# THU-DA-6D-Pose-Group/CATRE

Hardware: AMD Instinct MI355X
Metric: pose-refine iters/sec (B=256, N=1024, K=4) (higher is better)
Workload: dtype f32; 1 GPU; B=256 objects/GPU, N=1024 observed + M=1024 prior points, K=4 refine iterations, forward-only (eval loop of catre_evaluator.py:292-311), fp32 MFMA; objects_per_gpu=256, N=1024, M=1024, K=4, parallelism=batch-sharded x1 (no data-path collective)

## Files before the change

catre_amd/csrc/catre_kernels.hip:

```cpp
#include <algorithm>
#include <cstdlib>
#include <atomic>
#include <mutex>
#include <cstring>
#include <vector>

#include "catre_device.h"

#include "../../include/catre_hip.h"

#define CATRE_VERSION_STR "catre_hip gfx950 r1"
#define PMW 1088

struct TileInfo {
  int obj;
  int cloud;
  int is_obs;
  int p0;
  int valid;
};

__device__ __forceinline__ TileInfo tile_info(int bid, int B, int N, int M) {
  const int TN = (N + TP - 1) / TP, TM = (M + TP - 1) / TP;
  TileInfo ti;
// ... 1281 lines not shown
  } else {
    const int rd = catre_rot_dim(o.rot_type);
    float r[6];
#pragma unroll
    for (int i = 0; i < 6; ++i) r[i] = i < rd ? rotp[i] : 0.f;
    rot_param_to_mat(r, o.rot_type, dR);
  }

  const float* p0 = pose0 + b * 12;
  const float t0[3] = {p0[3], p0[7], p0[11]};
  float d[3] = {dtr[b * 3] * o.delta_t_weight, dtr[b * 3 + 1] * o.delta_t_weight, dtr[b * 3 + 2] * o.delta_t_weight};
  float t[3];
  if (!o.delta_t_space_3d) {
    const float zsrc = t0[2];
    const float ztgt = o.delta_z_deepim ? zsrc / expf(d[2]) : d[2] * zsrc;
    const float fx = o.k_aware ? Ks[b * 9 + 0] : 1.f, fy = o.k_aware ? Ks[b * 9 + 4] : 1.f;
    t[0] = ztgt * (d[0] / fx + t0[0] / zsrc);
    t[1] = ztgt * (d[1] / fy + t0[1] / zsrc);
    t[2] = ztgt;
  } else {
    t[0] = t0[0] + d[0];
    t[1] = t0[1] + d[1];
    t[2] = t0[2] + d[2];
  }
  const float* sb = o.scale_base_mean ? mean_scales + b * 3 : scale0 + b * 3;
  float s[3];
#pragma unroll
  for (int i = 0; i < 3; ++i) s[i] = o.scale_mul ? sb[i] * expf(dsr[b * 3 + i]) : sb[i] + dsr[b * 3 + i];

  if (o.is_allo) {
    const float nrm = sqrtf(t[0] * t[0] + t[1] * t[1] + t[2] * t[2]) + o.allo_eps;
    const float ray[3] = {t[0] / nrm, t[1] / nrm, t[2] / nrm};
    const float angle = acosf(ray[2]);
    float ax[3] = {-ray[1], ray[0], 0.f};
    const float an = sqrtf(ax[0] * ax[0] + ax[1] * ax[1]) + o.allo_eps;
    ax[0] /= an;
    ax[1] /= an;
    const float sh = sinf(angle * 0.5f);
    float q[4] = {cosf(angle * 0.5f), ax[0] * sh, ax[1] * sh, 0.f * sh};
    const float qn = sqrtf(q[0] * q[0] + q[1] * q[1] + q[2] * q[2] + q[3] * q[3]);
#pragma unroll
    for (int i = 0; i < 4; ++i) q[i] /= qn;
    const float X = q[1] * 2.f, Y = q[2] * 2.f, Z = q[3] * 2.f;
    const float wX = q[0] * X, wY = q[0] * Y, wZ = q[0] * Z, xX = q[1] * X, xY = q[1] * Y, xZ = q[1] * Z;
    const float yY = q[2] * Y, yZ = q[2] * Z, zZ = q[3] * Z;
    const float A[9] = {1.f - (yY + zZ), xY - wZ, xZ + wY, xY + wZ, 1.f - (xX + zZ), yZ - wX,
                        xZ - wY,         yZ + wX, 1.f - (xX + yY)};
    float E[9];
#pragma unroll
    for (int i = 0; i < 3; ++i)
#pragma unroll
      for (int j = 0; j < 3; ++j) E[i * 3 + j] = A[i * 3] * dR[j] + A[i * 3 + 1] * dR[3 + j] + A[i * 3 + 2] * dR[6 + j];
#pragma unroll
    for (int i = 0; i < 9; ++i) dR[i] = E[i];
  }
  float* po = pose_out + b * 12;
#pragma unroll
  for (int i = 0; i < 3; ++i) {
#pragma unroll
    for (int j = 0; j < 3; ++j)
      po[i * 4 + j] = dR[i * 3] * p0[j] + dR[i * 3 + 1] * p0[4 + j] + dR[i * 3 + 2] * p0[8 + j];
    po[i * 4 + 3] = t[i];
  }
#pragma unroll
  for (int i = 0; i < 3; ++i) scale_out[b * 3 + i] = o.refine_scale ? s[i] : scale0[b * 3 + i];
}

__global__ void k_pose_update(const float* __restrict__ rot6d, const float* __restrict__ dtr,
                              const float* __restrict__ dsr, const float* __restrict__ pose0,
                              const float* __restrict__ scale0, const float* __restrict__ mean_scales,
                              const float* __restrict__ Ks, catre_opts o, float* __restrict__ pose_out,
                              float* __restrict__ scale_out, int B, float* __restrict__ pose_echo = nullptr,
                              float* __restrict__ scale_echo = nullptr) {
  const int b = blockIdx.x * blockDim.x + threadIdx.x;
  if (b >= B) return;
  pose_update_obj(rot6d + (size_t)b * (o.rot_input_is_matrix ? 9 : catre_rot_dim(o.rot_type)), dtr, dsr, pose0, scale0,
                  mean_scales, Ks, o, pose_out, scale_out, b, pose_echo, scale_echo);
}

__global__ __launch_bounds__(256) void k_colmax(const float* __restrict__ x, float* __restrict__ out, int rows,
                                                int N) {
  const int lane = threadIdx.x & 63;
  const int wpb = blockDim.x >> 6;
  const int nwaves = gridDim.x * wpb;
  for (int row = blockIdx.x * wpb + (threadIdx.x >> 6); row < rows; row += nwaves) {
    const float* r = x + (size_t)row * N;
    float m = -INFINITY;
    if ((N & 3) == 0) {
      const f32x4* r4 = reinterpret_cast<const f32x4*>(r);
      const int n4 = N >> 2;
#pragma unroll 4
      for (int i = lane; i < n4; i += 64) {
        const f32x4 v = __builtin_nontemporal_load(r4 + i);
        m = fmaxf(fmaxf(m, fmaxf(v[0], v[1])), fmaxf(v[2], v[3]));
      }
    } else {
      for (int i = lane; i < N; i += 64) m = fmaxf(m, r[i]);
    }
#pragma unroll
    for (int o = 32; o > 0; o >>= 1) m = fmaxf(m, __shfl_xor(m, o));
    if (lane == 0) out[row] = m;
  }
}

#include "catre_bf16.h"
#include "catre_split.h"
#include "catre_screen.h"

template <bool SPLIT, class OT = OpBf16>
__device__ __forceinline__ void pack_frag_lp_body(const PackJobs& J) {
  static_assert(!SPLIT || !is_f16_op<OT>(), "the split packs are bf16 pairs");
  const int gi = blockIdx.x * blockDim.x + threadIdx.x;
  if (gi >= J.end[J.n - 1]) return;
  int j = 0;
  while (gi >= J.end[j]) ++j;
  const int base = j ? J.end[j - 1] : 0, idx = gi - base, total = J.end[j] - base;
  const int K = J.K[j];
  const int e = idx & 7, lane = (idx >> 3) & 63, rest = idx >> 9;
  const int nkc = K / 16;
  const int kc = rest % nkc, mb = rest / nkc;
  const int row = mb * 32 + (lane & 31), col = kc * 16 + 8 * (e >> 2) + 4 * (lane >> 5) + (e & 3);
  const float w = J.src[j][(size_t)row * J.ld[j] + J.coloff[j] + col];
  unsigned short* dst = reinterpret_cast<unsigned short*>(J.dst[j]);
  const typename OT::T h = (typename OT::T)w;
  dst[idx] = __builtin_bit_cast(unsigned short, h);
  if constexpr (SPLIT) dst[(size_t)total + idx] = __builtin_bit_cast(unsigned short, (__bf16)(w - (float)h));
}
template <bool SPLIT>
__global__ void k_pack_frag_lp_multi(PackJobs J) {
  pack_frag_lp_body<SPLIT>(J);
}
__global__ void k_pack_frag_hf_multi(PackJobs J) { pack_frag_lp_body<false, OpF16>(J); }
#include "catre_gram.h"
#include "catre_small.h"
#include "catre_train.h"
#include "catre_optim.h"
#include "catre_heads.h"
#include "catre_aug.h"
#include "catre_pcl.h"
#include "catre_pclf.h"
#include "catre_loss.h"
#include "catre_eval.h"

namespace {

inline size_t align_up(size_t v, size_t a) { return (v + a - 1) / a * a; }

struct PackLayout {
  size_t stn_c2, stn_c3, fstn_c1, fstn_c2, fstn_c3, c2, c3, c4, rot_l0[2], rot_l1[2], ts_w0t, ts_w1t, sumwp, total;
  size_t bf_stn_c2, bf_stn_c3, bf_fstn_c1, bf_fstn_c2, bf_fstn_c3, bf_c2, bf_c3, bf_c4, bf_rot_l0[2], bf_rot_l1[2];
  size_t sp_stn_c2, sp_stn_c3, sp_fstn_c1, sp_fstn_c2, sp_fstn_c3, sp_c3, sp_c4, sp_rot_l0[2], sp_rot_l1[2];
  size_t f16_stn_c2, f16_stn_c3, f16_fstn_c1, f16_fstn_c2, f16_fstn_c3, f16_c2, f16_c3, f16_c4, f16_rot_l0[2], f16_rot_l1[2];
  size_t scr_c4, scr_nw4, scr_stn_c3, scr_fstn_c3, scr_nw_stn, scr_nw_fstn;
};

PackLayout pack_layout(int ts_in) {
  PackLayout L;
  size_t o = 0;
  auto take = [&](size_t n) {
    size_t r = o;
    o += align_up(n, 64);
    return r;
  };
  L.stn_c2 = take(128 * 64);
  L.stn_c3 = take(1024 * 128);
  L.fstn_c1 = take(64 * 64);
  L.fstn_c2 = take(128 * 64);
  L.fstn_c3 = take(1024 * 128);
  L.c2 = take(128 * 64);
  L.c3 = take(512 * 128);
  L.c4 = take(1024 * 512);
  for (int h = 0; h < 2; ++h) {
    L.rot_l0[h] = take(256 * 64);
    L.rot_l1[h] = take(256 * 256);
  }
  L.sumwp = take(64);
  L.bf_stn_c2 = take(128 * 64 / 2);
  L.bf_stn_c3 = take(1024 * 128 / 2);
  L.bf_fstn_c1 = take(64 * 64 / 2);
  L.bf_fstn_c2 = take(128 * 64 / 2);
  L.bf_fstn_c3 = take(1024 * 128 / 2);
  L.bf_c2 = take(128 * 64 / 2);
  L.bf_c3 = take(512 * 128 / 2);
  L.bf_c4 = take(1024 * 512 / 2);
  for (int h = 0; h < 2; ++h) {
    L.bf_rot_l0[h] = take(256 * 64 / 2);
    L.bf_rot_l1[h] = take(256 * 256 / 2);
  }
  L.sp_stn_c2 = take(128 * 64);
  L.sp_stn_c3 = take(1024 * 128);
  L.sp_fstn_c1 = take(64 * 64);
  L.sp_fstn_c2 = take(128 * 64);
  L.sp_fstn_c3 = take(1024 * 128);
  L.sp_c3 = take(512 * 128);
  L.sp_c4 = take(1024 * 512);
  for (int h = 0; h < 2; ++h) {
    L.sp_rot_l0[h] = take(256 * 64);
    L.sp_rot_l1[h] = take(256 * 256);
  }
  L.f16_stn_c2 = take(128 * 64 / 2);
  L.f16_stn_c3 = take(1024 * 128 / 2);
  L.f16_fstn_c1 = take(64 * 64 / 2);
  L.f16_fstn_c2 = take(128 * 64 / 2);
  L.f16_fstn_c3 = take(1024 * 128 / 2);
  L.f16_c2 = take(128 * 64 / 2);
  L.f16_c3 = take(512 * 128 / 2);
  L.f16_c4 = take(1024 * 512 / 2);
  for (int h = 0; h < 2; ++h) {
    L.f16_rot_l0[h] = take(256 * 64 / 2);
    L.f16_rot_l1[h] = take(256 * 256 / 2);
  }
  L.scr_c4 = take(1024 * 512);
  L.scr_nw4 = take(1024);
  L.scr_stn_c3 = take(1024 * 128);
  L.scr_fstn_c3 = take(1024 * 128);
  L.scr_nw_stn = take(1024);
  L.scr_nw_fstn = take(1024);
  L.ts_w0t = take((size_t)ts_in * 256);
  L.ts_w1t = take(256 * 256);
  L.total = o;
  return L;
}

struct WsLayout {
  size_t tspart, xbuf, kbuf, pm, pool, h1, h2, trans3, trans64, gfeat, pointfeat, dt, ds, rot6d, bias0, gn0, gn1, aff0, gn1stat, y1, rpart,
      bar, frun, total;
};

WsLayout ws_layout(int B, int N, int M) {
  const size_t TN = (N + TP - 1) / TP, TM = (M + TP - 1) / TP, T = TN + TM;
  const size_t b = B, P = (size_t)N + M;
  WsLayout L;
  size_t o = 0;
  auto take = [&](size_t n) {
    size_t r = o;
    o += align_up(n, 64);
    return r;
  };
  L.tspart = take(b * 8 * 256);
  L.xbuf = take(b * N * 3);
  L.kbuf = take(b * M * 3);
  L.pm = take((2 * b <= SMALL_ROWS ? 2 : 1) * b * T * PMW);
  L.pool = take(2 * b * 1024);
  L.h1 = take(2 * b * 512);
  L.h2 = take(2 * b * 256);
  L.trans3 = take(2 * b * 9);
  L.trans64 = take(2 * b * 4096);
  L.gfeat = take(2 * b * PMW);
  L.pointfeat = take(b * P * 64);
  L.dt = take(b * 3);
  L.ds = take(b * 3);
  L.rot6d = take(b * 6);
  L.bias0 = take(2 * 2 * b * 256);
  L.gn0 = take(b * 2 * T * 64);
  L.gn1 = take(b * 2 * T * 64);
  L.aff0 = take(b * 2 * 2 * 2 * 256);
  L.gn1stat = take(b * 2 * 64);
  {
    const size_t y1n = b * 2 * P * 256, mom = b * 2 * (4 * (4096 + 64) + 64);
    const size_t y1t = b * 2 * T * 256 * 32;
    L.y1 = take(std::max(std::max(y1n, mom), y1t));
  }
  L.rpart = take(b * 2 * T * 4);
  L.bar = take(64);
  L.frun = take(b * ((TN + 1) / 2 + (TM + 1) / 2) * 1024);
  L.total = o;
  return L;
}

inline int check_launch() { return hipGetLastError() == hipSuccess ? CATRE_OK : CATRE_ERR_LAUNCH; }

inline bool dims_ok(int B, int N, int M) { return B > 0 && N > 0 && M > 0; }
inline bool dims_ok1(int B, int N, int M) { return B > 0 && N > 0 && M >= 0; }
inline int n_clouds(int B, int M) { return M > 0 ? 2 * B : B; }
#define RS_DISPATCH(rs, L) \
  switch (rs) {            \
    case 4: L(4); break;   \
    case 2: L(2); break;   \
    default: L(1);         \
  }
inline int row_split(int tiles) { return tiles * 4 <= 256 ? 4 : tiles * 2 <= 256 ? 2 : 1; }
#define RS_DISPATCH8(rs, L) \
  switch (rs) {             \
    case 8: L(8); break;    \
    case 4: L(4); break;    \
    case 2: L(2); break;    \
    default: L(1);          \
  }
inline int row_split8(int tiles) { return tiles * 8 <= 256 ? 8 : row_split(tiles); }
inline int gn0_shares(int B) { return B * 8 <= 512 ? 8 : B * 4 <= 512 ? 4 : B * 2 <= 512 ? 2 : 1; }
inline int trunk_h_split(int tiles) { return tiles * 8 <= 256 ? 4 : tiles * 4 <= 256 ? 2 : tiles * 2 <= 256 ? 1 : 0; }

#define REQUIRE(cond) \
  do {                \
    if (!(cond)) return CATRE_ERR_BAD_ARG; \
  } while (0)

inline const f32x4* pk4(const float* packed, size_t off) { return reinterpret_cast<const f32x4*>(packed + off); }
inline const u32x4* pkb(const float* packed, size_t off) { return reinterpret_cast<const u32x4*>(packed + off); }

inline TsHeadArgs ts_head_args(const float* l0part, const float* const* prm, const float* packed, const PackLayout& L,
                               float* dt, float* ds, int B) {
  return TsHeadArgs{l0part, prm[CATRE_P_TS_L0_B], prm[CATRE_P_TS_GN0_W], prm[CATRE_P_TS_GN0_B], packed + L.ts_w1t,
                    prm[CATRE_P_TS_L1_B], prm[CATRE_P_TS_GN1_W], prm[CATRE_P_TS_GN1_B], prm[CATRE_P_TS_FCT_W],
                    prm[CATRE_P_TS_FCT_B], prm[CATRE_P_TS_FCS_W], prm[CATRE_P_TS_FCS_B], dt, ds, B};
}

int stn_fc_tail(const float* pooled, const float* const* prm, int base , float* h1, float* h2,
                float* out, int k, int R, hipStream_t st, const float* pm = nullptr, int B = 0, int N = 0, int M = 0,
                unsigned* bar = nullptr) {
  if (bar) {
    const int nb3 = (k * k + 31) / 32, grid = nb3 > 16 ? nb3 : 16;
    hipLaunchKernelGGL(k_fc_tail, dim3(grid), dim3(64 * LIN_WAVES), 0, st, pooled, pm, B, N, M, prm[base], prm[base + 1],
                       prm[base + 2], prm[base + 3], prm[base + 4], prm[base + 5], h1, h2, out, k, R, bar);
    return check_launch();
  }
  if (pm)
    hipLaunchKernelGGL(k_linear_pm, dim3(1, 512 / 32), dim3(64 * LIN_WAVES), 0, st, pm, B, N, M, prm[base], 1024,
                       prm[base + 1], h1, 512, R, 512, 1, nullptr, nullptr, nullptr);
  else
    hipLaunchKernelGGL(k_linear, dim3((R + 31) / 32, 512 / 32), dim3(64 * LIN_WAVES), 0, st, pooled, 1024, prm[base], 1024,
                       prm[base + 1], h1, 512, R, 512, 1024, 1, 0);
  hipLaunchKernelGGL(k_linear, dim3((R + 31) / 32, 256 / 32), dim3(64 * LIN_WAVES), 0, st, h1, 512, prm[base + 2], 512,
                     prm[base + 3], h2, 256, R, 256, 512, 1, 0);
  hipLaunchKernelGGL(k_linear, dim3((R + 31) / 32, (k * k + 31) / 32), dim3(64 * LIN_WAVES), 0, st, h2, 256, prm[base + 4], 256,
                     prm[base + 5], out, k * k, R, k * k, 256, 0, k);
  return check_launch();
}

struct ProfState {
  int kernel = -1;
  int cap = 0, n = 0;
  hipEvent_t* ev = nullptr;
};
ProfState g_prof;
unsigned long long* g_trunk_trace = nullptr;

static int bf_pair_min() {
  static const int v = [] {
    const char* e = getenv("CATRE_BF_PAIR_MIN");
    return e ? atoi(e) : 512;
  }();
  return v;
}

enum { FORM_TRUNK4 = 1, FORM_STN4 = 2, FORM_STN_PAIR = 4, FORM_ROTW = 8, FORM_FC_TAIL = 16, FORM_SCREEN = 32, FORM_SCREEN_STN = 64,
       FORM_SCREEN_POOL = 128, FORM_SCREEN_RUN = 256 };
#ifndef CATRE_SCREEN_DEFAULT
#define CATRE_SCREEN_DEFAULT true
#endif
#ifndef CATRE_SCREEN_STN_DEFAULT
#define CATRE_SCREEN_STN_DEFAULT true
#endif
#ifndef CATRE_SCREEN_POOL_DEFAULT
#define CATRE_SCREEN_POOL_DEFAULT true
#endif
#ifndef CATRE_SCREEN_RUN_DEFAULT
#define CATRE_SCREEN_RUN_DEFAULT true
#endif
static std::atomic<int> g_forms{-1};
static int forms() {
  int v = g_forms.load(std::memory_order_relaxed);
  if (v < 0) {
    auto on = [](const char* name, bool dflt = true) {
      const char* e = getenv(name);
      return e ? atoi(e) != 0 : dflt;
    };
    v = (on("CATRE_TRUNK4") ? FORM_TRUNK4 : 0) | (on("CATRE_STN4") ? FORM_STN4 : 0) |
        (on("CATRE_STN_PAIR") ? FORM_STN_PAIR : 0) | (on("CATRE_ROTW", false) ? FORM_ROTW : 0) |
        (on("CATRE_FC_TAIL", false) ? FORM_FC_TAIL : 0) | (on("CATRE_SCREEN", CATRE_SCREEN_DEFAULT) ? FORM_SCREEN : 0) |
        (on("CATRE_SCREEN_STN", CATRE_SCREEN_STN_DEFAULT) ? FORM_SCREEN_STN : 0) |
        (on("CATRE_SCREEN_POOL", CATRE_SCREEN_POOL_DEFAULT) ? FORM_SCREEN_POOL : 0) |
        (on("CATRE_SCREEN_RUN", CATRE_SCREEN_RUN_DEFAULT) ? FORM_SCREEN_RUN : 0);
    g_forms.store(v, std::memory_order_relaxed);
  }
  return v;
}
static bool trunk4_on() { return forms() & FORM_TRUNK4; }
inline int stn_pairs(int B, int N, int M) { return B * (((N + TP - 1) / TP + 1) / 2 + ((M + TP - 1) / TP + 1) / 2); }
static bool stn_pair_on() { return forms() & FORM_STN_PAIR; }
static bool stn4_on() { return forms() & FORM_STN4; }
static bool fc_tail_on() { return forms() & FORM_FC_TAIL; }
static bool screen_on() { return forms() & FORM_SCREEN; }
static bool screen_stn_on() { return (forms() & (FORM_SCREEN | FORM_SCREEN_STN)) == (FORM_SCREEN | FORM_SCREEN_STN); }
static bool screen_pool_on() { return forms() & FORM_SCREEN_POOL; }
static bool screen_run_on() { return (forms() & (FORM_SCREEN_POOL | FORM_SCREEN_RUN)) == (FORM_SCREEN_POOL | FORM_SCREEN_RUN); }
static std::atomic<int> g_run_len{0};
static int screen_run_rule(int B, int N, int M, int cus) {
  const int TN = (N + TP - 1) / TP, TM = (M + TP - 1) / TP;
  const long long slots1 = ((long long)B * (TN + TM) + cus - 1) / cus;
  for (int S = 16; S > 1; --S) {
    const long long R = (long long)B * ((TN + S - 1) / S + (TM + S - 1) / S);
    if ((R + cus - 1) / cus * S <= slots1) return S;
  }
  return 1;
}
static int device_cus() {
  static const int n = [] {
    int dev = 0, v = 0;
    if (hipGetDevice(&dev) != hipSuccess || hipDeviceGetAttribute(&v, hipDeviceAttributeMultiprocessorCount, dev) != hipSuccess || v <= 0)
      v = 256;
    return v;
  }();
  return n;
}
static int screen_run_len(int B, int N, int M) {
  const int f = g_run_len.load(std::memory_order_relaxed);
  return f > 0 ? f : screen_run_rule(B, N, M, device_cus());
}
#ifndef CATRE_SCREEN_POOL_STN_DEFAULT
#define CATRE_SCREEN_POOL_STN_DEFAULT true
#endif
static bool screen_pool_stn_on() {
  static const bool stn = [] { const char* e = getenv("CATRE_SCREEN_POOL_STN"); return e ? atoi(e) != 0 : CATRE_SCREEN_POOL_STN_DEFAULT; }();
  return screen_pool_on() && stn;
}
#ifndef CATRE_SCREEN_RUN_STN_DEFAULT
#define CATRE_SCREEN_RUN_STN_DEFAULT true
#endif
static bool screen_run_stn_on() {
  static const bool stn = [] { const char* e = getenv("CATRE_SCREEN_RUN_STN"); return e ? atoi(e) != 0 : CATRE_SCREEN_RUN_STN_DEFAULT; }();
  return screen_run_on() && screen_stn_on() && screen_pool_stn_on() && stn;
}
inline int stn_pair_runs(int B, int N, int M, int SP) {
  return B * ((((N + TP - 1) / TP + 1) / 2 + SP - 1) / SP + (((M + TP - 1) / TP + 1) / 2 + SP - 1) / SP);
}
static bool rotw_on() { return forms() & FORM_ROTW; }

#ifndef CATRE_NO_PROFILING
std::mutex g_prof_mu;
struct ProfScope {
  hipStream_t st;
  int slot = -1;
  ProfScope(int kernel_id, hipStream_t s) : st(s) {
    if (g_prof.kernel != kernel_id) return;
    std::lock_guard<std::mutex> lk(g_prof_mu);
    if (g_prof.kernel == kernel_id && g_prof.n < g_prof.cap) {
      slot = g_prof.n++;
      (void)hipEventRecord(g_prof.ev[2 * slot], st);
    }
  }
  ~ProfScope() {
    if (slot < 0) return;
    std::lock_guard<std::mutex> lk(g_prof_mu);
    if (slot < g_prof.cap) (void)hipEventRecord(g_prof.ev[2 * slot + 1], st);
  }
};
#else
struct ProfScope {
  ProfScope(int, hipStream_t) {}
};
#endif


static bool stn_pair_form(int tiles, int B, int N, int M) {
  return row_split8(tiles) == 1 && stn4_on() && stn_pair_on() && stn_pairs(B, N, M) >= 256;
}

void launch_stn3d(const catre_points* pts, const float* const* prm, const float* packed, float* ws, const WsLayout& W,
                  int B, int N, int M, bool split, hipStream_t st, unsigned* zero_bar = nullptr, float* probe_s = nullptr,
                  float* probe_eps = nullptr, float* probe_rows = nullptr) {
  const PackLayout L = pack_layout(1);
  const int tiles = B * ((N + TP - 1) / TP + (M + TP - 1) / TP);
  ProfScope ps(CATRE_K_STN3D, st);
  if (split) {
#define LAUNCH_(RS)                                                                                            \
  hipLaunchKernelGGL(k_stn3d_split<RS>, dim3(tiles * RS), dim3(256), 0, st, *pts, prm[CATRE_P_STN_CONV1_W],     \
                     prm[CATRE_P_STN_CONV1_B], pkb(packed, L.sp_stn_c2), prm[CATRE_P_STN_CONV2_B],              \
                     pkb(packed, L.sp_stn_c3), prm[CATRE_P_STN_CONV3_B], ws + W.pm, B, N, M)
    RS_DISPATCH(row_split(tiles), LAUNCH_)
#undef LAUNCH_
  } else if (const int S = stn_pair_form(tiles, B, N, M) && screen_run_stn_on() && !probe_s ? screen_run_len(B, N, M) : 1; S > 1) {
    const int SP = S / 2;
    hipLaunchKernelGGL(k_stn3d_pair_sr, dim3(stn_pair_runs(B, N, M, SP)), dim3(256), 0, st,
                       Stn3dRunArgs{*pts, prm[CATRE_P_STN_CONV1_W], prm[CATRE_P_STN_CONV1_B], pk4(packed, L.stn_c2),
                                    prm[CATRE_P_STN_CONV2_B], pk4(packed, L.stn_c3), prm[CATRE_P_STN_CONV3_B], ws + W.pm,
                                    pkb(packed, L.scr_stn_c3), packed + L.scr_nw_stn, B, N, M, SP});
  } else if (stn_pair_form(tiles, B, N, M) && (screen_stn_on() || probe_s)) {
    hipLaunchKernelGGL(screen_pool_stn_on() ? k_stn3d_pair_sp : k_stn3d_pair_s, dim3(stn_pairs(B, N, M)), dim3(256), 0, st, *pts, prm[CATRE_P_STN_CONV1_W],
                       prm[CATRE_P_STN_CONV1_B], pk4(packed, L.stn_c2), prm[CATRE_P_STN_CONV2_B], pk4(packed, L.stn_c3),
                       prm[CATRE_P_STN_CONV3_B], ws + W.pm, B, N, M,
                       ScreenArgs{pkb(packed, L.scr_stn_c3), packed + L.scr_nw_stn, probe_s, probe_eps}, probe_rows);
  } else if (stn_pair_form(tiles, B, N, M)) {
    const int pairs = stn_pairs(B, N, M);
    hipLaunchKernelGGL(k_stn3d_pair<false>, dim3(pairs), dim3(256), 0, st, *pts, prm[CATRE_P_STN_CONV1_W], prm[CATRE_P_STN_CONV1_B],
                       pk4(packed, L.stn_c2), prm[CATRE_P_STN_CONV2_B], pk4(packed, L.stn_c3), prm[CATRE_P_STN_CONV3_B],
                       ws + W.pm, B, N, M);
  } else if (row_split8(tiles) == 1 && stn4_on()) {
    hipLaunchKernelGGL((k_stn3d<1, false, true>), dim3(tiles), dim3(256), 0, st, *pts, prm[CATRE_P_STN_CONV1_W],
                       prm[CATRE_P_STN_CONV1_B], pk4(packed, L.stn_c2), prm[CATRE_P_STN_CONV2_B], pk4(packed, L.stn_c3),
                       prm[CATRE_P_STN_CONV3_B], ws + W.pm, B, N, M, TrainSave{}, zero_bar);
  } else {
#define LAUNCH_(RS)                                                                                      \
  hipLaunchKernelGGL(k_stn3d<RS>, dim3(tiles * RS), dim3(256), 0, st, *pts, prm[CATRE_P_STN_CONV1_W],     \
                     prm[CATRE_P_STN_CONV1_B], pk4(packed, L.stn_c2), prm[CATRE_P_STN_CONV2_B],           \
                     pk4(packed, L.stn_c3), prm[CATRE_P_STN_CONV3_B], ws + W.pm, B, N, M, TrainSave{}, zero_bar)
    RS_DISPATCH8(row_split8(tiles), LAUNCH_)
#undef LAUNCH_
  }
}

void launch_stnkd(const catre_points* pts, const float* trans3, const float* const* prm, const float* packed, float* ws,
                  const WsLayout& W, int B, int N, int M, bool split, hipStream_t st, unsigned* zero_bar = nullptr,
                  float* probe_s = nullptr, float* probe_eps = nullptr, float* probe_rows = nullptr) {
  const PackLayout L = pack_layout(1);
  const int tiles = B * ((N + TP - 1) / TP + (M + TP - 1) / TP);
  ProfScope ps(CATRE_K_STNKD, st);
  if (split) {
#define LAUNCH_(RS)                                                                                                \
  hipLaunchKernelGGL(k_stnkd_split<RS>, dim3(tiles * RS), dim3(256), 0, st, *pts, trans3, prm[CATRE_P_CONV1_W],     \
                     prm[CATRE_P_CONV1_B], pkb(packed, L.sp_fstn_c1), prm[CATRE_P_FSTN_CONV1_B],                    \
                     pkb(packed, L.sp_fstn_c2), prm[CATRE_P_FSTN_CONV2_B], pkb(packed, L.sp_fstn_c3),               \
                     prm[CATRE_P_FSTN_CONV3_B], ws + W.pm, B, N, M)
    RS_DISPATCH(row_split(tiles), LAUNCH_)
#undef LAUNCH_
  } else if (const int S = stn_pair_form(tiles, B, N, M) && screen_run_stn_on() && !probe_s ? screen_run_len(B, N, M) : 1; S > 1) {
    const int SP = S / 2;
    hipLaunchKernelGGL(k_stnkd_pair_sr, dim3(stn_pair_runs(B, N, M, SP)), dim3(256), 0, st,
                       StnkdRunArgs{*pts, trans3, prm[CATRE_P_CONV1_W], prm[CATRE_P_CONV1_B], pk4(packed, L.fstn_c1),
                                    prm[CATRE_P_FSTN_CONV1_B], pk4(packed, L.fstn_c2), prm[CATRE_P_FSTN_CONV2_B],
                                    pk4(packed, L.fstn_c3), prm[CATRE_P_FSTN_CONV3_B], ws + W.pm,
                                    pkb(packed, L.scr_fstn_c3), packed + L.scr_nw_fstn, B, N, M, SP});
  } else if (stn_pair_form(tiles, B, N, M) && (screen_stn_on() || probe_s)) {
    hipLaunchKernelGGL(screen_pool_stn_on() ? k_stnkd_pair_sp : k_stnkd_pair_s, dim3(stn_pairs(B, N, M)), dim3(256), 0, st, *pts, trans3, prm[CATRE_P_CONV1_W],
                       prm[CATRE_P_CONV1_B], pk4(packed, L.fstn_c1), prm[CATRE_P_FSTN_CONV1_B], pk4(packed, L.fstn_c2),
                       prm[CATRE_P_FSTN_CONV2_B], pk4(packed, L.fstn_c3), prm[CATRE_P_FSTN_CONV3_B], ws + W.pm, B, N, M,
                       ScreenArgs{pkb(packed, L.scr_fstn_c3), packed + L.scr_nw_fstn, probe_s, probe_eps}, probe_rows);
  } else if (stn_pair_form(tiles, B, N, M)) {
    const int pairs = stn_pairs(B, N, M);
    hipLaunchKernelGGL(k_stnkd_pair<false>, dim3(pairs), dim3(256), 0, st, *pts, trans3, prm[CATRE_P_CONV1_W], prm[CATRE_P_CONV1_B],
                       pk4(packed, L.fstn_c1), prm[CATRE_P_FSTN_CONV1_B], pk4(packed, L.fstn_c2), prm[CATRE_P_FSTN_CONV2_B],
                       pk4(packed, L.fstn_c3), prm[CATRE_P_FSTN_CONV3_B], ws + W.pm, B, N, M);
  } else if (row_split8(tiles) == 1 && stn4_on()) {
    hipLaunchKernelGGL((k_stnkd<1, false, true>), dim3(tiles), dim3(256), 0, st, *pts, trans3, prm[CATRE_P_CONV1_W],
                       prm[CATRE_P_CONV1_B], pk4(packed, L.fstn_c1), prm[CATRE_P_FSTN_CONV1_B], pk4(packed, L.fstn_c2),
                       prm[CATRE_P_FSTN_CONV2_B], pk4(packed, L.fstn_c3), prm[CATRE_P_FSTN_CONV3_B], ws + W.pm, B, N, M,
                       TrainSave{}, zero_bar);
  } else {
#define LAUNCH_(RS)                                                                                                     \
  hipLaunchKernelGGL(k_stnkd<RS>, dim3(tiles * RS), dim3(256), 0, st, *pts, trans3, prm[CATRE_P_CONV1_W],                \
                     prm[CATRE_P_CONV1_B], pk4(packed, L.fstn_c1), prm[CATRE_P_FSTN_CONV1_B], pk4(packed, L.fstn_c2),    \
                     prm[CATRE_P_FSTN_CONV2_B], pk4(packed, L.fstn_c3), prm[CATRE_P_FSTN_CONV3_B], ws + W.pm, B, N, M,   \
                     TrainSave{}, zero_bar)
    RS_DISPATCH8(row_split8(tiles), LAUNCH_)
#undef LAUNCH_
  }
}

void launch_trunk(const catre_points* pts, const float* trans3, const float* trans64, const float* const* prm,
                  const float* packed, float* pointfeat, float* ws, const WsLayout& W, int B, int N, int M, bool split,
                  hipStream_t st, float* probe_s = nullptr, float* probe_eps = nullptr) {
  const PackLayout L = pack_layout(1);
  const int tiles = B * ((N + TP - 1) / TP + (M + TP - 1) / TP);
  ProfScope ps(CATRE_K_TRUNK, st);
  if (split) {
#define LAUNCH_(RS)                                                                                           \
  hipLaunchKernelGGL(k_trunk_split<RS>, dim3(tiles * RS), dim3(512), 0, st, *pts, trans3, trans64,             \
                     prm[CATRE_P_CONV1_W], prm[CATRE_P_CONV1_B], pk4(packed, L.c2), prm[CATRE_P_CONV2_B],      \
                     pkb(packed, L.sp_c3), prm[CATRE_P_CONV3_B], pkb(packed, L.sp_c4), prm[CATRE_P_CONV4_B],   \
                     ws + W.pm, pointfeat, B, N, M, g_trunk_trace)
    RS_DISPATCH(row_split(tiles), LAUNCH_)
#undef LAUNCH_
  } else if (const int S = row_split8(tiles) == 1 && trunk4_on() && screen_on() && screen_run_on() ? screen_run_len(B, N, M) : 1;
             S > 1) {
    const int runs = B * (((N + TP - 1) / TP + S - 1) / S + ((M + TP - 1) / TP + S - 1) / S);
    hipLaunchKernelGGL(k_trunk4sr, dim3(runs), dim3(256), 0, st,
                       TrunkRunArgs{*pts, trans3, trans64, prm[CATRE_P_CONV1_W], prm[CATRE_P_CONV1_B], pk4(packed, L.c2),
                                    prm[CATRE_P_CONV2_B], pk4(packed, L.c3), prm[CATRE_P_CONV3_B], pk4(packed, L.c4),
                                    prm[CATRE_P_CONV4_B], ws + W.pm, pointfeat, g_trunk_trace,
                                    ScreenArgs{pkb(packed, L.scr_c4), packed + L.scr_nw4, probe_s, probe_eps}, ws + W.frun,
                                    B, N, M, S});
  } else if (row_split8(tiles) == 1 && trunk4_on() && (screen_on() || probe_s)) {
    hipLaunchKernelGGL(screen_pool_on() ? k_trunk4sp : k_trunk4s, dim3(tiles), dim3(256), 0, st, *pts, trans3, trans64,
                       prm[CATRE_P_CONV1_W], prm[CATRE_P_CONV1_B], pk4(packed, L.c2), prm[CATRE_P_CONV2_B], pk4(packed, L.c3),
                       prm[CATRE_P_CONV3_B], pk4(packed, L.c4), prm[CATRE_P_CONV4_B], ws + W.pm, pointfeat, B, N, M,
                       g_trunk_trace, ScreenArgs{pkb(packed, L.scr_c4), packed + L.scr_nw4, probe_s, probe_eps});
  } else if (row_split8(tiles) == 1 && trunk4_on()) {
    hipLaunchKernelGGL(k_trunk4<false>, dim3(tiles), dim3(256), 0, st, *pts, trans3, trans64, prm[CATRE_P_CONV1_W],
                       prm[CATRE_P_CONV1_B], pk4(packed, L.c2), prm[CATRE_P_CONV2_B], pk4(packed, L.c3),
                       prm[CATRE_P_CONV3_B], pk4(packed, L.c4), prm[CATRE_P_CONV4_B], ws + W.pm, pointfeat, B, N, M,
                       g_trunk_trace);
  } else {
#define LAUNCH_(RS)                                                                                             \
  hipLaunchKernelGGL(k_trunk<RS>, dim3(tiles * RS), dim3(512), 0, st, *pts, trans3, trans64, prm[CATRE_P_CONV1_W], \
                     prm[CATRE_P_CONV1_B], pk4(packed, L.c2), prm[CATRE_P_CONV2_B], pk4(packed, L.c3),            \
                     prm[CATRE_P_CONV3_B], pk4(packed, L.c4), prm[CATRE_P_CONV4_B], ws + W.pm, pointfeat, B, N, M, \
                     g_trunk_trace)
    RS_DISPATCH8(row_split8(tiles), LAUNCH_)
#undef LAUNCH_
  }
}

}

extern "C" {

const char* catre_version(void) { return CATRE_VERSION_STR; }

const char* catre_status_string(int s) {
  switch (s) {
    case CATRE_OK: return "ok";
    case CATRE_ERR_BAD_ARG: return "bad argument";
    case CATRE_ERR_WORKSPACE: return "workspace or packed-weight buffer too small";
    case CATRE_ERR_LAUNCH: return "kernel launch failed";
    case CATRE_ERR_UNSUPPORTED: return "unsupported configuration";
    default: return "unknown status";
  }
}

size_t catre_workspace_bytes(int B, int N, int M) {
  if (!dims_ok1(B, N, M)) return 0;
  return ws_layout(B, N, M).total * sizeof(float);
}

size_t catre_packed_floats(int N, int M, int ts_in_dim) {
  if (N <= 0 || M <= 0 || ts_in_dim <= 0) return 0;
  return pack_layout(ts_in_dim).total;
}

int catre_pack_weights(const float* const* prm, int N, int M, int ts_in, float* packed, size_t packed_floats,
                       void* stream) {
  return catre_pack_weights_sel(prm, N, M, ts_in, packed, packed_floats, CATRE_PACK_ALL, stream);
}

int catre_pack_weights_sel(const float* const* prm, int N, int M, int ts_in, float* packed, size_t packed_floats, int sel,
                           void* stream) {
  REQUIRE(prm && packed && N > 0 && M > 0 && ts_in > 0);
  const PackLayout L = pack_layout(ts_in);
  if (packed_floats < L.total) return CATRE_ERR_WORKSPACE;
  hipStream_t st = (hipStream_t)stream;
  const bool enc32 = sel & CATRE_PACK_F32_ENCODER, head32 = sel & CATRE_PACK_F32_HEADS, bf = sel & CATRE_PACK_BF16,
             sp = sel & CATRE_PACK_SPLIT, tails = sel & CATRE_PACK_F32_TAILS, hf = sel & CATRE_PACK_F16;
  PackJobs jobs;
  jobs.n = 0;
  auto flush = [&]() {
    if (jobs.n) hipLaunchKernelGGL(k_pack_frag_multi, dim3((jobs.end[jobs.n - 1] + 255) / 256), dim3(256), 0, st, jobs);
    jobs.n = 0;
  };
  auto frag = [&](const float* src, int ld, int coloff, int rows, int K, size_t off) {
    if (!src) return;
    if (jobs.n == PACK_MAX_JOBS) flush();
    const int j = jobs.n++;
    jobs.src[j] = src;
    jobs.dst[j] = packed + off;
    jobs.ld[j] = ld;
    jobs.coloff[j] = coloff;
    jobs.K[j] = K;
    jobs.end[j] = (j ? jobs.end[j - 1] : 0) + rows * K;
  };
  PackJobs lpjobs;
  lpjobs.n = 0;
  enum { LP_BF16, LP_SPLIT, LP_F16 };
  auto flush_lp = [&](int kind) {
    if (lpjobs.n) {
      const dim3 grid((lpjobs.end[lpjobs.n - 1] + 255) / 256);
      if (kind == LP_SPLIT)
        hipLaunchKernelGGL(k_pack_frag_lp_multi<true>, grid, dim3(256), 0, st, lpjobs);
      else if (kind == LP_F16)
        hipLaunchKernelGGL(k_pack_frag_hf_multi, grid, dim3(256), 0, st, lpjobs);
      else
        hipLaunchKernelGGL(k_pack_frag_lp_multi<false>, grid, dim3(256), 0, st, lpjobs);
    }
    lpjobs.n = 0;
  };
  auto frag_lp = [&](int kind, const float* src, int ld, int coloff, int rows, int K, size_t off) {
    if (!src) return;
    if (lpjobs.n == PACK_MAX_JOBS) flush_lp(kind);
    const int j = lpjobs.n++;
    lpjobs.src[j] = src;
    lpjobs.dst[j] = packed + off;
    lpjobs.ld[j] = ld;
    lpjobs.coloff[j] = coloff;
    lpjobs.K[j] = K;
    lpjobs.end[j] = (j ? lpjobs.end[j - 1] : 0) + rows * K;
  };
  auto frag_bf = [&](const float* src, int ld, int coloff, int rows, int K, size_t off) {
    frag_lp(LP_BF16, src, ld, coloff, rows, K, off);
  };
  if (bf) {
  frag_bf(prm[CATRE_P_STN_CONV2_W], 64, 0, 128, 64, L.bf_stn_c2);
  frag_bf(prm[CATRE_P_STN_CONV3_W], 128, 0, 1024, 128, L.bf_stn_c3);
  frag_bf(prm[CATRE_P_FSTN_CONV1_W], 64, 0, 64, 64, L.bf_fstn_c1);
  frag_bf(prm[CATRE_P_FSTN_CONV2_W], 64, 0, 128, 64, L.bf_fstn_c2);
  frag_bf(prm[CATRE_P_FSTN_CONV3_W], 128, 0, 1024, 128, L.bf_fstn_c3);
  frag_bf(prm[CATRE_P_CONV2_W], 64, 0, 128, 64, L.bf_c2);
  frag_bf(prm[CATRE_P_CONV3_W], 128, 0, 512, 128, L.bf_c3);
  frag_bf(prm[CATRE_P_CONV4_W], 512, 0, 1024, 512, L.bf_c4);
  for (int h = 0; h < 2; ++h) {
    const int base = h ? CATRE_P_ROTY_L0_W : CATRE_P_ROTX_L0_W;
    frag_bf(prm[base], PMW, 1024, 256, 64, L.bf_rot_l0[h]);
    frag_bf(prm[base + 4], 256, 0, 256, 256, L.bf_rot_l1[h]);
  }
  flush_lp(LP_BF16);
  }
  if (hf) {
    auto frag_hf = [&](const float* src, int ld, int coloff, int rows, int K, size_t off) {
      frag_lp(LP_F16, src, ld, coloff, rows, K, off);
    };
    frag_hf(prm[CATRE_P_STN_CONV2_W], 64, 0, 128, 64, L.f16_stn_c2);
    frag_hf(prm[CATRE_P_STN_CONV3_W], 128, 0, 1024, 128, L.f16_stn_c3);
    frag_hf(prm[CATRE_P_FSTN_CONV1_W], 64, 0, 64, 64, L.f16_fstn_c1);
    frag_hf(prm[CATRE_P_FSTN_CONV2_W], 64, 0, 128, 64, L.f16_fstn_c2);
    frag_hf(prm[CATRE_P_FSTN_CONV3_W], 128, 0, 1024, 128, L.f16_fstn_c3);
    frag_hf(prm[CATRE_P_CONV2_W], 64, 0, 128, 64, L.f16_c2);
    frag_hf(prm[CATRE_P_CONV3_W], 128, 0, 512, 128, L.f16_c3);
    frag_hf(prm[CATRE_P_CONV4_W], 512, 0, 1024, 512, L.f16_c4);
    for (int h = 0; h < 2; ++h) {
      const int base = h ? CATRE_P_ROTY_L0_W : CATRE_P_ROTX_L0_W;
      frag_hf(prm[base], PMW, 1024, 256, 64, L.f16_rot_l0[h]);
      frag_hf(prm[base + 4], 256, 0, 256, 256, L.f16_rot_l1[h]);
    }
    flush_lp(LP_F16);
  }
  auto frag_sp = [&](const float* src, int ld, int rows, int K, size_t off, int coloff = 0) {
    frag_lp(LP_SPLIT, src, ld, coloff, rows, K, off);
  };
  if (sp) {
  frag_sp(prm[CATRE_P_STN_CONV2_W], 64, 128, 64, L.sp_stn_c2);
  frag_sp(prm[CATRE_P_STN_CONV3_W], 128, 1024, 128, L.sp_stn_c3);
  frag_sp(prm[CATRE_P_FSTN_CONV1_W], 64, 64, 64, L.sp_fstn_c1);
  frag_sp(prm[CATRE_P_FSTN_CONV2_W], 64, 128, 64, L.sp_fstn_c2);
  frag_sp(prm[CATRE_P_FSTN_CONV3_W], 128, 1024, 128, L.sp_fstn_c3);
  frag_sp(prm[CATRE_P_CONV3_W], 128, 512, 128, L.sp_c3);
  frag_sp(prm[CATRE_P_CONV4_W], 512, 1024, 512, L.sp_c4);
  frag_sp(prm[CATRE_P_ROTX_L0_W], PMW, 256, 64, L.sp_rot_l0[0], 1024);
  frag_sp(prm[CATRE_P_ROTY_L0_W], PMW, 256, 64, L.sp_rot_l0[1], 1024);
  frag_sp(prm[CATRE_P_ROTX_L0_W + 4], 256, 256, 256, L.sp_rot_l1[0]);
  frag_sp(prm[CATRE_P_ROTY_L0_W + 4], 256, 256, 256, L.sp_rot_l1[1]);
  flush_lp(LP_SPLIT);
  }
  if (enc32) {
  frag(prm[CATRE_P_STN_CONV2_W], 64, 0, 128, 64, L.stn_c2);
  frag(prm[CATRE_P_STN_CONV3_W], 128, 0, 1024, 128, L.stn_c3);
  frag(prm[CATRE_P_FSTN_CONV1_W], 64, 0, 64, 64, L.fstn_c1);
  frag(prm[CATRE_P_FSTN_CONV2_W], 64, 0, 128, 64, L.fstn_c2);
  frag(prm[CATRE_P_FSTN_CONV3_W], 128, 0, 1024, 128, L.fstn_c3);
  frag(prm[CATRE_P_CONV2_W], 64, 0, 128, 64, L.c2);
  frag(prm[CATRE_P_CONV3_W], 128, 0, 512, 128, L.c3);
  frag(prm[CATRE_P_CONV4_W], 512, 0, 1024, 512, L.c4);
  if (prm[CATRE_P_CONV4_W]) {
    frag_sp(prm[CATRE_P_CONV4_W], 512, 1024, 512, L.scr_c4);
    flush_lp(LP_SPLIT);
    hipLaunchKernelGGL(k_screen_wnorm, dim3(1024 / 4), dim3(256), 0, st, prm[CATRE_P_CONV4_W], 512, 1024, 512,
                       packed + L.scr_nw4);
  }
  frag_sp(prm[CATRE_P_STN_CONV3_W], 128, 1024, 128, L.scr_stn_c3);
  frag_sp(prm[CATRE_P_FSTN_CONV3_W], 128, 1024, 128, L.scr_fstn_c3);
  flush_lp(LP_SPLIT);
  if (prm[CATRE_P_STN_CONV3_W])
    hipLaunchKernelGGL(k_screen_wnorm, dim3(1024 / 4), dim3(256), 0, st, prm[CATRE_P_STN_CONV3_W], 128, 1024, 128,
                       packed + L.scr_nw_stn);
  if (prm[CATRE_P_FSTN_CONV3_W])
    hipLaunchKernelGGL(k_screen_wnorm, dim3(1024 / 4), dim3(256), 0, st, prm[CATRE_P_FSTN_CONV3_W], 128, 1024, 128,
                       packed + L.scr_nw_fstn);
  }
  for (int h = 0; h < 2 && head32; ++h) {
    const int base = h ? CATRE_P_ROTY_L0_W : CATRE_P_ROTX_L0_W;
    frag(prm[base], PMW, 1024, 256, 64, L.rot_l0[h]);
    frag(prm[base + 4], 256, 0, 256, 256, L.rot_l1[h]);
    if (prm[base + 10] && tails)
      hipLaunchKernelGGL(k_sum, dim3(1), dim3(256), 0, st, prm[base + 10], N + M, packed + L.sumwp + h);
  }
  flush();
  if (head32 && tails && prm[CATRE_P_TS_L0_W] && prm[CATRE_P_TS_L1_W]) {
    int n = ts_in * 256;
    hipLaunchKernelGGL(k_pack_transpose, dim3((n + 255) / 256), dim3(256), 0, st, prm[CATRE_P_TS_L0_W], 256, ts_in,
                       packed + L.ts_w0t);
    n = 256 * 256;
    hipLaunchKernelGGL(k_pack_transpose, dim3((n + 255) / 256), dim3(256), 0, st, prm[CATRE_P_TS_L1_W], 256, 256,
                       packed + L.ts_w1t);
  }
  return check_launch();
}

int catre_pose_apply(const float* pcl, const float* kps, const float* pose, const float* scale, float* x_out,
                     float* kps_out, int B, int N, int M, int zero_center, void* stream) {
  REQUIRE(pcl && kps && pose && scale && x_out && kps_out && dims_ok(B, N, M));
  const int total = B * (N + M);
  hipLaunchKernelGGL(k_pose_apply, dim3((total + 255) / 256), dim3(256), 0, (hipStream_t)stream, pcl, kps, pose, scale,
                     x_out, kps_out, B, N, M, zero_center);
  return check_launch();
}

int catre_stn3d_pool(const catre_points* pts, const float* const* prm, const float* packed, float* pooled,
                     void* workspace, size_t ws_bytes, int B, int N, int M, void* stream) {
  REQUIRE(pts && prm && packed && pooled && workspace && dims_ok1(B, N, M));
  const WsLayout W = ws_layout(B, N, M);
  if (ws_bytes < W.total * sizeof(float)) return CATRE_ERR_WORKSPACE;
  float* ws = (float*)workspace;
  hipStream_t st = (hipStream_t)stream;
  launch_stn3d(pts, prm, packed, ws, W, B, N, M, false, st);
  hipLaunchKernelGGL(k_reduce_pm, dim3(n_clouds(B, M), (1024 + 255) / 256), dim3(256), 0, st, ws + W.pm, pooled, 1024, 1024, B, N, M);
  return check_launch();
}

int catre_linear(const float* x, int ldx, const float* Wt, int ldw, const float* bias, float* y, int ldy, int R, int J,
                 int K, int relu, int add_identity_k, void* stream) {
  REQUIRE(x && Wt && y && R > 0 && J > 0 && K > 0 && (K % 8) == 0 && (ldx % 4) == 0 && (ldw % 4) == 0);
  hipLaunchKernelGGL(k_linear, dim3((R + 31) / 32, (J + 31) / 32), dim3(64 * LIN_WAVES), 0, (hipStream_t)stream, x, ldx, Wt, ldw,
                     bias, y, ldy, R, J, K, relu, add_identity_k);
  return check_launch();
}

int catre_linear_t(const float* x, int ldx, const float* xmask, const float* W, int ldw, float* y, int ldy, int R, int J,
                   int K, void* stream) {
  REQUIRE(x && W && y && R > 0 && J > 0 && K > 0 && (K % 8) == 0 && (ldx % 4) == 0 && ldw >= J);
  hipLaunchKernelGGL(k_linear_t, dim3((R + 31) / 32, (J + 31) / 32), dim3(64 * LIN_WAVES), 0, (hipStream_t)stream, x, ldx, W,
                     ldw, y, ldy, R, J, K, xmask);
  return check_launch();
}

int catre_stnkd_pool(const catre_points* pts, const float* trans3, const float* const* prm, const float* packed,
                     float* pooled, void* workspace, size_t ws_bytes, int B, int N, int M, void* stream) {
  REQUIRE(pts && trans3 && prm && packed && pooled && workspace && dims_ok1(B, N, M));
  const WsLayout W = ws_layout(B, N, M);
  if (ws_bytes < W.total * sizeof(float)) return CATRE_ERR_WORKSPACE;
  float* ws = (float*)workspace;
  hipStream_t st = (hipStream_t)stream;
  launch_stnkd(pts, trans3, prm, packed, ws, W, B, N, M, false, st);
  hipLaunchKernelGGL(k_reduce_pm, dim3(n_clouds(B, M), (1024 + 255) / 256), dim3(256), 0, st, ws + W.pm, pooled, 1024, 1024, B, N, M);
  return check_launch();
}

int catre_trunk(const catre_points* pts, const float* trans3, const float* trans64, const float* const* prm,
                const float* packed, float* gfeat, float* pointfeat, void* workspace, size_t ws_bytes, int B, int N,
                int M, void* stream) {
  REQUIRE(pts && trans3 && prm && packed && gfeat && pointfeat && workspace && dims_ok1(B, N, M));
  const WsLayout W = ws_layout(B, N, M);
  if (ws_bytes < W.total * sizeof(float)) return CATRE_ERR_WORKSPACE;
  float* ws = (float*)workspace;
  hipStream_t st = (hipStream_t)stream;
  launch_trunk(pts, trans3, trans64, prm, packed, pointfeat, ws, W, B, N, M, false, st);
  hipLaunchKernelGGL(k_reduce_pm, dim3(n_clouds(B, M), (PMW + 255) / 256), dim3(256), 0, st, ws + W.pm, gfeat, PMW, PMW, B, N, M);
  return check_launch();
}

static bool out_dim_ok(int d) { return d == 64 || d == 128 || d == 256 || d == 512 || d == 1024; }

size_t catre_packed_floats_w(int out_dim) {
  if (!out_dim_ok(out_dim)) return 0;
  return pack_layout(1).total + (size_t)out_dim * 512;
}

int catre_pack_encoder_w(const float* const* prm, int out_dim, float* packed, size_t packed_floats, void* stream) {
  REQUIRE(prm && packed);
  if (!out_dim_ok(out_dim)) return CATRE_ERR_UNSUPPORTED;
  REQUIRE(prm[CATRE_P_CONV4_W]);
  const size_t base = pack_layout(1).total;
  if (packed_floats < base + (size_t)out_dim * 512) return CATRE_ERR_WORKSPACE;
  const float* enc[CATRE_P_COUNT];
  for (int i = 0; i < CATRE_P_COUNT; ++i) enc[i] = prm[i];
  enc[CATRE_P_CONV4_W] = nullptr;
  const int s = catre_pack_weights_sel(enc, 1, 1, 1, packed, packed_floats, CATRE_PACK_F32_ENCODER, stream);
  if (s != CATRE_OK) return s;
  const int n = out_dim * 512;
  hipLaunchKernelGGL(k_pack_frag, dim3((n + 255) / 256), dim3(256), 0, (hipStream_t)stream, prm[CATRE_P_CONV4_W], 512, 0,
                     out_dim, 512, packed + base);
  return check_launch();
}

int catre_trunk_w(const catre_points* pts, const float* trans3, const float* trans64, const float* const* prm,
                  const float* packed, int out_dim, float* gfeat, float* pointfeat, void* workspace, size_t ws_bytes, int B,
                  int N, int M, void* stream) {
  REQUIRE(pts && trans3 && prm && packed && gfeat && pointfeat && workspace && dims_ok1(B, N, M));
  if (!out_dim_ok(out_dim)) return CATRE_ERR_UNSUPPORTED;
  const WsLayout W = ws_layout(B, N, M);
  if (ws_bytes < W.total * sizeof(float)) return CATRE_ERR_WORKSPACE;
  float* ws = (float*)workspace;
  hipStream_t st = (hipStream_t)stream;
  const PackLayout L = pack_layout(1);
  const int tiles = B * ((N + TP - 1) / TP + (M + TP - 1) / TP);
#define LAUNCH_(MB, NB)                                                                                                \
  hipLaunchKernelGGL((k_trunkw<MB, NB>), dim3(tiles), dim3(512), 0, st, *pts, trans3, trans64, prm[CATRE_P_CONV1_W],   \
                     prm[CATRE_P_CONV1_B], pk4(packed, L.c2), prm[CATRE_P_CONV2_B], pk4(packed, L.c3),                 \
                     prm[CATRE_P_CONV3_B], pk4(packed, L.total), prm[CATRE_P_CONV4_B], out_dim / 32, ws + W.pm,        \
                     pointfeat, B, N, M)
  switch (out_dim) {
    case 1024: LAUNCH_(4, 2); break;
    case 512: LAUNCH_(2, 2); break;
    case 256: LAUNCH_(1, 2); break;
    default: LAUNCH_(1, 1);
  }
#undef LAUNCH_
  hipLaunchKernelGGL(k_reduce_pm_w, dim3(n_clouds(B, M), (out_dim + 64 + 255) / 256), dim3(256), 0, st, ws + W.pm, gfeat,
                     out_dim, B, N, M);
  return check_launch();
}

int catre_trunk_screen_probe(const catre_points* pts, const float* trans3, const float* trans64, const float* const* prm,
                             const float* packed, float* screen, float* eps, float* gfeat, float* pointfeat, void* workspace,
                             size_t ws_bytes, int B, int N, int M, void* stream) {
  REQUIRE(pts && trans3 && prm && packed && screen && eps && gfeat && pointfeat && workspace && dims_ok1(B, N, M));
  const WsLayout W = ws_layout(B, N, M);
  if (ws_bytes < W.total * sizeof(float)) return CATRE_ERR_WORKSPACE;
  const int tiles = B * ((N + TP - 1) / TP + (M + TP - 1) / TP);
  if (row_split8(tiles) != 1 || !trunk4_on()) return CATRE_ERR_UNSUPPORTED;
  float* ws = (float*)workspace;
  hipStream_t st = (hipStream_t)stream;
  launch_trunk(pts, trans3, trans64, prm, packed, pointfeat, ws, W, B, N, M, false, st, screen, eps);
  hipLaunchKernelGGL(k_reduce_pm, dim3(n_clouds(B, M), (PMW + 255) / 256), dim3(256), 0, st, ws + W.pm, gfeat, PMW, PMW, B, N, M);
  return check_launch();
}

int catre_stn_screen_probe(int which, const catre_points* pts, const float* trans3, const float* const* prm,
                           const float* packed, float* screen, float* eps, float* rows, float* pooled, void* workspace,
                           size_t ws_bytes, int B, int N, int M, void* stream) {
  REQUIRE((which == 0 || which == 1) && pts && (which == 0 || trans3) && prm && packed && screen && eps && rows && pooled &&
// ... 346 lines not shown
    A.s1c = s1c;
    A.shc = shc;
    A.pose = init_pose;
    A.scale = init_scale;
    A.W0T = packed + L.ts_w0t;
    A.tspart = ws + W.tspart;
    A.in_dim = o->ts_in_dim;
    A.with_kps = o->with_kps_feature;
    A.with_scale = o->with_init_scale;
    A.with_trans = o->with_init_trans;
    A.w0x = prm[CATRE_P_ROTX_L0_W];
    A.b0x = prm[CATRE_P_ROTX_L0_W + 1];
    A.w0y = prm[CATRE_P_ROTY_L0_W];
    A.b0y = prm[CATRE_P_ROTY_L0_W + 1];
    A.bias0 = bias0;
    A.pm = fold ? ws + W.pm : nullptr;
    A.gfeat = ws + W.gfeat;
    A.B = B;
    A.N = N;
    A.M = M;
    A.rpt = rsh ? 2 : 1;
    A.n_mom = R * PF_NG;
    A.n_ts = groups * TS_KS;
    ProfScope ps(CATRE_K_ROT_L0_STATS, st);
    hipLaunchKernelGGL(k_heads_a, dim3(A.n_mom + A.n_ts + 2 * 8), dim3(64 * LIN_WAVES), 0, st, A);
    hipLaunchKernelGGL(k_gn0_from_moments, dim3(B, gn0_shares(B)), dim3(256), 0, st, Gc, s1c, shc, prm[CATRE_P_ROTX_L0_W],
                       prm[CATRE_P_ROTY_L0_W], PMW, 1024, bias0, prm[CATRE_P_ROTX_GN0_W], prm[CATRE_P_ROTX_GN0_B],
                       prm[CATRE_P_ROTY_GN0_W], prm[CATRE_P_ROTY_GN0_B], ws + W.aff0, B, N, M);
  }
  {
    ProfScope ps(CATRE_K_ROT_L1, st);
    if (split)
      hipLaunchKernelGGL(k_rot_l1_split<false>, dim3(B * T), dim3(256), 0, st, ws + W.pointfeat, pkb(packed, L.sp_rot_l0[0]),
                         pkb(packed, L.sp_rot_l0[1]), ws + W.aff0, pkb(packed, L.sp_rot_l1[0]), pkb(packed, L.sp_rot_l1[1]),
                         prm[CATRE_P_ROTX_L1_B], prm[CATRE_P_ROTY_L1_B], ws + W.y1, ws + W.gn1, B, N, M,
                         g_trunk_trace ? g_trunk_trace + ((size_t)1 << 24) : nullptr);
    else {
#define LAUNCH_ROT_L1(RS)                                                                                               \
  hipLaunchKernelGGL(k_rot_l1<RS>, dim3(B * T * RS), dim3(256), 0, st, ws + W.pointfeat, pk4(packed, L.rot_l0[0]),        \
                     pk4(packed, L.rot_l0[1]), ws + W.aff0, pk4(packed, L.rot_l1[0]), pk4(packed, L.rot_l1[1]),         \
                     prm[CATRE_P_ROTX_L1_B], prm[CATRE_P_ROTY_L1_B], ws + W.y1, ws + W.gn1, B, N, M,                     \
                     g_trunk_trace ? g_trunk_trace + ((size_t)1 << 24) : nullptr)
      RS_DISPATCH(row_split(B * T), LAUNCH_ROT_L1)
#undef LAUNCH_ROT_L1
    }
  }
  {
    HeadsDArgs D;
    D.y1 = ws + W.y1;
    D.gn1 = ws + W.gn1;
    D.gam1x = prm[CATRE_P_ROTX_GN1_W];
    D.bet1x = prm[CATRE_P_ROTX_GN1_B];
    D.gam1y = prm[CATRE_P_ROTY_GN1_W];
    D.bet1y = prm[CATRE_P_ROTY_GN1_B];
    D.neckx = prm[CATRE_P_ROTX_NECK_W];
    D.necky = prm[CATRE_P_ROTY_NECK_W];
    D.wpx = prm[CATRE_P_ROTX_CONVP_W];
    D.wpy = prm[CATRE_P_ROTY_CONVP_W];
    D.rpart = ws + W.rpart;
    D.B = B;
    D.N = N;
    D.M = M;
    D.rd = rd;
    D.n_rot = B * T * 2;
    D.ts = ts_head_args(ws + W.tspart, prm, packed, L, ws + W.dt, ws + W.ds, B);
    ProfScope ps(CATRE_K_ROT_OUT, st);
    hipLaunchKernelGGL(k_heads_d, dim3(D.n_rot + groups), dim3(1024), smem_d, st, D);
  }
  hipLaunchKernelGGL(k_finish_update, dim3((B + 7) / 8), dim3(64), 0, st, ws + W.rpart, prm[CATRE_P_ROTX_NECK_B],
                     prm[CATRE_P_ROTY_NECK_B], packed + L.sumwp, prm[CATRE_P_ROTX_CONVP_B], prm[CATRE_P_ROTY_CONVP_B], T, rd,
                     ws + W.dt, ws + W.ds, init_pose, init_scale, mean_scales, Ks, *o, pose_out, scale_out, B, pose_echo,
                     scale_echo);
  return check_launch();
}

int catre_refine_iter(const catre_points* pts, const float* init_pose, const float* init_scale,
                      const float* mean_scales, const float* Ks, const float* const* prm, const float* packed,
                      const catre_opts* o, float* pose_out, float* scale_out, void* workspace, size_t ws_bytes, int B,
                      int N, int M, void* stream) {
  return refine_iter_impl(pts, init_pose, init_scale, mean_scales, Ks, prm, packed, o, pose_out, scale_out, workspace,
                          ws_bytes, B, N, M, stream, nullptr, nullptr);
}

static int refine_k_impl(const float* pcl, const float* kps, const float* init_pose, const float* init_scale,
                         const float* mean_scales, const float* Ks, const float* const* prm, const float* packed,
                         const catre_opts* o, float* poses, float* scales, void* workspace, size_t ws_bytes, int B, int N,
                         int M, int n_iter, void* stream) {
  REQUIRE(pcl && kps && prm && packed && o && poses && scales && workspace && dims_ok(B, N, M) && n_iter >= 0);
  REQUIRE((init_pose == nullptr) == (init_scale == nullptr));
  const WsLayout W = ws_layout(B, N, M);
  if (ws_bytes < W.total * sizeof(float)) return CATRE_ERR_WORKSPACE;
  float* ws = (float*)workspace;
#ifndef CATRE_OTF_POINTS
#define CATRE_OTF_POINTS (64 * 1024)
#endif
  const bool on_the_fly = (size_t)B * (N + M) <= (size_t)CATRE_OTF_POINTS;
  catre_points pts;
  pts.obs = on_the_fly ? pcl : ws + W.xbuf;
  pts.obs_sb = (int64_t)N * 3;
  pts.obs_sn = 3;
  pts.obs_sc = 1;
  pts.kps = on_the_fly ? kps : ws + W.kbuf;
  pts.kps_sb = (int64_t)M * 3;
  pts.kps_sn = 3;
  pts.kps_sc = 1;
  pts.apply_pose = on_the_fly ? 1 : 0;
  pts.zero_center = o->zero_center;
  pts.pose = pts.scale = nullptr;
  if (init_pose && n_iter == 0) {
    if (hipMemcpyAsync(poses, init_pose, (size_t)B * 12 * sizeof(float), hipMemcpyDeviceToDevice, (hipStream_t)stream) !=
            hipSuccess ||
        hipMemcpyAsync(scales, init_scale, (size_t)B * 3 * sizeof(float), hipMemcpyDeviceToDevice, (hipStream_t)stream) !=
            hipSuccess)
      return CATRE_ERR_LAUNCH;
  }
  for (int i = 1; i <= n_iter; ++i) {
    const bool first = init_pose && i == 1;
    const float* pose_in = first ? init_pose : poses + (size_t)(i - 1) * B * 12;
    const float* scale_in = first ? init_scale : scales + (size_t)(o->refine_scale ? i - 1 : 0) * B * 3;
    if (on_the_fly) {
      pts.pose = pose_in;
      pts.scale = scale_in;
    } else {
      const int rc0 =
          catre_pose_apply(pcl, kps, pose_in, scale_in, ws + W.xbuf, ws + W.kbuf, B, N, M, o->zero_center, stream);
      if (rc0) return rc0;
    }
    const int rc = refine_iter_impl(&pts, pose_in, scale_in, mean_scales, Ks, prm, packed, o, poses + (size_t)i * B * 12,
                                    scales + (size_t)i * B * 3, workspace, ws_bytes, B, N, M, stream,
                                    first ? poses : nullptr, first ? scales : nullptr);
    if (rc) return rc;
  }
  return CATRE_OK;
}

int catre_refine_k(const float* pcl, const float* kps, const float* mean_scales, const float* Ks,
                   const float* const* prm, const float* packed, const catre_opts* o, float* poses, float* scales,
                   void* workspace, size_t ws_bytes, int B, int N, int M, int n_iter, void* stream) {
  return refine_k_impl(pcl, kps, nullptr, nullptr, mean_scales, Ks, prm, packed, o, poses, scales, workspace, ws_bytes, B, N,
                       M, n_iter, stream);
}

int catre_refine_k_from(const float* pcl, const float* kps, const float* init_pose, const float* init_scale,
                        const float* mean_scales, const float* Ks, const float* const* prm, const float* packed,
                        const catre_opts* o, float* poses, float* scales, void* workspace, size_t ws_bytes, int B, int N,
                        int M, int n_iter, void* stream) {
  REQUIRE(init_pose && init_scale);
  return refine_k_impl(pcl, kps, init_pose, init_scale, mean_scales, Ks, prm, packed, o, poses, scales, workspace, ws_bytes,
                       B, N, M, n_iter, stream);
}


int catre_form_switch(int id, int value) {
  if (id < 0 || id > 8) return -1;
  const int bit = 1 << id;
  const int cur = forms();
  if (value >= 0) g_forms.store(value ? (cur | bit) : (cur & ~bit), std::memory_order_relaxed);
  return (cur & bit) ? 1 : 0;
}

int catre_screen_run_len(int value) {
  const int prev = g_run_len.load(std::memory_order_relaxed);
  if (value >= 0) g_run_len.store(value > 16 ? 16 : value, std::memory_order_relaxed);
  return prev;
}

int catre_screen_run_rule(int B, int N, int M, int cus) {
  if (B <= 0 || N <= 0 || M < 0 || cus <= 0) return -1;
  return screen_run_rule(B, N, M, cus);
}

int catre_debug_knob(int id, int value) {
#ifdef CATRE_DEBUG_TRACE
  if (id == 0) return hipMemcpyToSymbol(HIP_SYMBOL(g_dephase_cycles), &value, sizeof(int)) == hipSuccess ? CATRE_OK : CATRE_ERR_LAUNCH;
  if (id == 1) return hipMemcpyToSymbol(HIP_SYMBOL(g_ablate), &value, sizeof(int)) == hipSuccess ? CATRE_OK : CATRE_ERR_LAUNCH;
  if (id == 2) return hipMemcpyToSymbol(HIP_SYMBOL(g_screen_count_on), &value, sizeof(int)) == hipSuccess ? CATRE_OK : CATRE_ERR_LAUNCH;
  return CATRE_ERR_BAD_ARG;
#else
  (void)id;
  (void)value;
  return CATRE_ERR_UNSUPPORTED;
#endif
}

int catre_stream_capture_id(void* stream, unsigned long long* id_out) {
  REQUIRE(id_out);
  hipStreamCaptureStatus status = hipStreamCaptureStatusNone;
  unsigned long long id = 0;
  if (hipStreamGetCaptureInfo((hipStream_t)stream, &status, &id) != hipSuccess) return CATRE_ERR_LAUNCH;
  *id_out = status == hipStreamCaptureStatusActive ? id : 0ull;
  return CATRE_OK;
}

int catre_debug_screen_counts(unsigned long long* out192, int reset) {
#ifdef CATRE_DEBUG_TRACE
  REQUIRE(out192);
  if (hipMemcpyFromSymbol(out192, HIP_SYMBOL(g_screen_cnt), 3 * 64 * sizeof(unsigned long long)) != hipSuccess) return CATRE_ERR_LAUNCH;
  if (reset) {
    const unsigned long long z[3 * 64] = {};
    if (hipMemcpyToSymbol(HIP_SYMBOL(g_screen_cnt), z, sizeof(z)) != hipSuccess) return CATRE_ERR_LAUNCH;
  }
  return CATRE_OK;
#else
  (void)out192;
  (void)reset;
  return CATRE_ERR_UNSUPPORTED;
#endif
}

int catre_debug_trunk_trace(void* device_buffer) {
#ifdef CATRE_DEBUG_TRACE
  g_trunk_trace = (unsigned long long*)device_buffer;
  return CATRE_OK;
#else
  (void)device_buffer;
  return CATRE_ERR_UNSUPPORTED;
#endif
}

#ifdef CATRE_NO_PROFILING
int catre_profile_enable(int, int) { return CATRE_ERR_UNSUPPORTED; }
int catre_profile_collect(float*, int, int*) { return CATRE_ERR_UNSUPPORTED; }
#else
int catre_profile_enable(int kernel_id, int max_records) {
  std::lock_guard<std::mutex> lk(g_prof_mu);
  for (int i = 0; i < 2 * g_prof.cap; ++i) (void)hipEventDestroy(g_prof.ev[i]);
  delete[] g_prof.ev;
  g_prof = ProfState();
  if (kernel_id < 0 || max_records <= 0) return CATRE_OK;
  if (kernel_id >= CATRE_K_COUNT) return CATRE_ERR_BAD_ARG;
  g_prof.ev = new hipEvent_t[2 * max_records];
  for (int i = 0; i < 2 * max_records; ++i)
    if (hipEventCreate(&g_prof.ev[i]) != hipSuccess) return CATRE_ERR_LAUNCH;
  g_prof.kernel = kernel_id;
  g_prof.cap = max_records;
  return CATRE_OK;
}

int catre_profile_collect(float* ms_out, int max_out, int* n_out) {
  REQUIRE(n_out && (ms_out || max_out == 0));
  std::lock_guard<std::mutex> lk(g_prof_mu);
  int n = g_prof.n < max_out ? g_prof.n : max_out;
  for (int i = 0; i < n; ++i) {
    if (hipEventSynchronize(g_prof.ev[2 * i + 1]) != hipSuccess) return CATRE_ERR_LAUNCH;
    if (hipEventElapsedTime(&ms_out[i], g_prof.ev[2 * i], g_prof.ev[2 * i + 1]) != hipSuccess) return CATRE_ERR_LAUNCH;
  }
  *n_out = n;
  g_prof.n = 0;
  return CATRE_OK;
}
#endif

int catre_colmax(const float* x, float* out, int B, int C, int N, void* stream) {
  REQUIRE(x && out && B > 0 && C > 0 && N > 0);
  const int rows = B * C;
  const int grid = rows / 4 < 8192 ? (rows + 3) / 4 : 8192;
  {
    ProfScope ps(CATRE_K_COLMAX, (hipStream_t)stream);
    hipLaunchKernelGGL(k_colmax, dim3(grid), dim3(256), 0, (hipStream_t)stream, x, out, rows, N);
  }
  return check_launch();
}

#include "catre_train_api.inc"
#include "catre_heads_api.inc"

int catre_aug_points(const float* pcl, const float* pose, const float* scale, const int32_t* sym_flags,
                     const float* bbox_ratios, const float* delta_r, const float* delta_t, float* pcl_out,
                     float* pose_out, float* scale_out, int B, int N, void* stream) {
  REQUIRE(pcl && pose && scale && pcl_out && pose_out && scale_out && B > 0 && N > 0);
  REQUIRE((delta_r == nullptr) == (delta_t == nullptr));
  AugParams prm;
  prm.do_bbox = bbox_ratios != nullptr;
  prm.do_rt = delta_r != nullptr;
  for (int i = 0; i < 3; ++i) prm.ratios[i] = prm.do_bbox ? bbox_ratios[i] : 1.f;
  for (int i = 0; i < 9; ++i) prm.delta_r[i] = prm.do_rt ? delta_r[i] : (i % 4 == 0 ? 1.f : 0.f);
  for (int i = 0; i < 3; ++i) prm.delta_t[i] = prm.do_rt ? delta_t[i] : 0.f;
  const int total = B * N;
  hipLaunchKernelGGL(k_aug_points, dim3((total + 255) / 256), dim3(256), 0, (hipStream_t)stream, pcl, pose, scale,
                     sym_flags, prm, pcl_out, pose_out, scale_out, B, N);
  return check_launch();
}

namespace {
struct PclWs {
  size_t bins, choose, offsets, total, cand, total_ints;
  int nchunks;
};
inline bool pcl_frame_ok(int H, int W) { return H > 0 && W > 0 && (size_t)H * (size_t)W < ((size_t)1 << 30); }
PclWs pcl_ws(int I, int H, int W) {
  PclWs L;
  const size_t HW = (size_t)H * (size_t)W;
  L.nchunks = (int)((HW + PCL_CHUNK - 1) / PCL_CHUNK);
  size_t o = 0;
  auto take = [&](size_t n) {
    size_t r = o;
    o += align_up(n, 64);
    return r;
  };
  L.bins = take((size_t)I * L.nchunks * 12);
  L.choose = take(I);
  L.offsets = take((size_t)I * L.nchunks);
  L.total = take(I);
  L.cand = take((size_t)I * HW);
  L.total_ints = o;
  return L;
}
// ... 254 lines not shown
```

catre_amd/csrc/catre_screen.h:

```cpp
#pragma once

template <int K>
struct ScreenBound {
  static constexpr float gamma = 3.f * 0x1p-18f + 4.f * K * 0x1p-23f;
  static constexpr float delta = K * 0x1p-122f;
  static constexpr float infl = 1.f + 0x1p-22f / gamma + 0x1p-20f;
};
template <int K>
__device__ __forceinline__ void screen_eps_coef(float nw, float& e1, float& e0) {
  e1 = fmaf(ScreenBound<K>::gamma, nw, ScreenBound<K>::delta) * ScreenBound<K>::infl;
  e0 = ScreenBound<K>::delta * (nw + 1.f) * ScreenBound<K>::infl;
}

__global__ __launch_bounds__(256) void k_screen_wnorm(const float* __restrict__ W, int ld, int rows, int K,
                                                      float* __restrict__ nw) {
  const int row = blockIdx.x * 4 + (threadIdx.x >> 6), lane = threadIdx.x & 63;
  if (row >= rows) return;
  double s = 0.0;
  for (int k = lane; k < K; k += 64) {
    const double w = W[(size_t)row * ld + k];
    s += w * w;
  }
#pragma unroll
  for (int o = 32; o > 0; o >>= 1) s += __shfl_xor(s, o);
  if (lane == 0) nw[row] = (float)sqrt(s) * (1.f + 0x1p-21f);
}

struct ScreenArgs {
  const u32x4* wps;
  const float* nw;
  float* probe_s;
  float* probe_eps;
};

#ifdef CATRE_DEBUG_TRACE
__device__ unsigned long long g_screen_cnt[3][64];
__device__ int g_screen_count_on = 1;
#define SCREEN_COUNT(layer, bin, v)                                        \
  do {                                                                     \
    if (g_screen_count_on) atomicAdd(&g_screen_cnt[layer][bin], (unsigned long long)(v)); \
  } while (0)
#endif

#define SCREEN_CMAX 4

template <class T>
__device__ __forceinline__ T lane_get(T v, int src_lane) {
  return __builtin_bit_cast(T, __builtin_amdgcn_ds_bpermute(src_lane << 2, __builtin_bit_cast(int, v)));
}

template <int C, int NT, int ROWS = 64, bool SWZ = true>
__device__ __forceinline__ void screen_row_norms(const float* __restrict__ img, float* __restrict__ na, int tid, int ld = C) {
  constexpr int PER = NT / ROWS, CH = C / 4 / PER;
  static_assert(CH % 16 == 0, "a thread's chunks are whole swizzle groups");
  const int row = tid / PER, part = tid % PER;
  const float* r = img + row * ld + part * CH * 4;
  const int key = SWZ ? row & 15 : 0;
  float s = 0.f;
#pragma unroll 8
  for (int j = 0; j < CH; ++j) {
    const f32x4 v = *reinterpret_cast<const f32x4*>(r + ((j ^ key) << 2));
    s = fmaf(v[0], v[0], s);
    s = fmaf(v[1], v[1], s);
    s = fmaf(v[2], v[2], s);
    s = fmaf(v[3], v[3], s);
  }
#pragma unroll
  for (int o = 1; o < PER; o <<= 1) s += lane_get(s, tid ^ o);
  if (part == 0) na[row] = fmaf(sqrtf(s), 1.f + 0x1p-12f, 0x1p-58f);
}

template <int PFD, int NKC_ = 32, bool SWZ = true, int LD = 512>
struct ScreenPipe8 {
  static constexpr int NKC = NKC_, NT = 2 * NKC, RA = PFD + 1, LO = 1024 * (16 * NKC) / 8;
  u32x4 ah[RA][4], al[RA][4];
  const u32x4* wp;

  __device__ __forceinline__ void issue_a(int t) {
    const int kc = t >> 1, half = t & 1;
#pragma unroll
    for (int m = 0; m < 4; ++m) {
      ah[t % RA][m] = wp[((half * 4 + m) * NKC + kc) * 64];
      al[t % RA][m] = wp[LO + ((half * 4 + m) * NKC + kc) * 64];
    }
  }
  __device__ __forceinline__ void prefetch(const u32x4* __restrict__ wp_) {
    wp = wp_;
#pragma unroll
    for (int d = 0; d < PFD - 1; ++d) issue_a(d);
    __builtin_amdgcn_sched_barrier(0);
  }
  __device__ __forceinline__ void run(f32x16 (&acc)[8][2], const float* x, int lane) {
    const int n = lane & 31, h = lane >> 5, sw = lane & 15;
    const float* xrow = x + n * LD;
    const float* xlow[4][2];
#pragma unroll
    for (int q = 0; q < 4; ++q)
#pragma unroll
      for (int j = 0; j < 2; ++j) xlow[q][j] = SWZ ? xrow + (((4 * q + 2 * j + h) ^ sw) << 2) : xrow + ((2 * j + h) << 2);
    f32x4 braw[2][2];
    u32x4 bh[2][2], bl[2][2];
    auto issue_b = [&](int kc) {
#pragma unroll
      for (int nb = 0; nb < 2; ++nb)
#pragma unroll
        for (int j = 0; j < 2; ++j)
          braw[nb][j] = *reinterpret_cast<const f32x4*>((SWZ ? xlow[kc & 3][j] + (kc >> 2) * 64 : xlow[0][j] + kc * 16) +
                                                        nb * 32 * LD);
    };
    auto split_b = [&](int kc) {
#pragma unroll
      for (int nb = 0; nb < 2; ++nb) {
        const float v[8] = {braw[nb][0][0], braw[nb][0][1], braw[nb][0][2], braw[nb][0][3],
                            braw[nb][1][0], braw[nb][1][1], braw[nb][1][2], braw[nb][1][3]};
        split_bf8(v, bh[kc & 1][nb], bl[kc & 1][nb]);
      }
    };
    issue_a(PFD - 1);
    issue_b(0);
    split_b(0);
    issue_b(1);
#pragma unroll
    for (int kc = 0; kc < NKC; ++kc) {
#pragma unroll
      for (int half = 0; half < 2; ++half) {
        const int t = 2 * kc + half;
        if (t + PFD < NT) issue_a(t + PFD);
        __builtin_amdgcn_sched_barrier(0);
        if (half == 1 && kc + 1 < NKC) split_b(kc + 1);
#pragma unroll
        for (int m = 0; m < 4; ++m)
#pragma unroll
          for (int nb = 0; nb < 2; ++nb) {
            f32x16& c = acc[half * 4 + m][nb];
            c = mfma_bf(bh[kc & 1][nb], al[t % RA][m], c);
            c = mfma_bf(bl[kc & 1][nb], ah[t % RA][m], c);
            c = mfma_bf(bh[kc & 1][nb], ah[t % RA][m], c);
          }
        if (half == 1 && kc + 1 < NKC) {
#pragma unroll
          for (int g = 0; g < 24; ++g) {
            __builtin_amdgcn_sched_group_barrier(0x008, 1, 0);
            __builtin_amdgcn_sched_group_barrier(0x002, 3, 0);
          }
        }
        __builtin_amdgcn_sched_barrier(0);
        if (half == 1 && kc + 2 < NKC) issue_b(kc + 2);
      }
    }
  }
};

__device__ __forceinline__ void screen_load_w(f32x4 (&wb)[16], const f32x4* __restrict__ w) {
#pragma unroll
  for (int kc = 0; kc < 8; ++kc) {
    wb[2 * kc] = w[kc * 64];
    wb[2 * kc + 1] = w[kc * 64 + 32];
  }
}

template <int T, int NKC8, bool SWZ = true>
__device__ __forceinline__ float screen_replay(const f32x4* __restrict__ w, const f32x4* __restrict__ wnext,
                                               f32x4 (&wb)[2][16], const float* x, int ld, const int (&p)[SCREEN_CMAX]) {
  static_assert(NKC8 % 2 == 0 && (T == 1 || T == 2 || T == 4), "two blocks of 8 chunks per trip");
  constexpr int SB = 4 / T, NS = 8 / SB;
  float y[T];
  const float* row[T];
  int key[T];
#pragma unroll
  for (int j = 0; j < T; ++j) {
    y[j] = 0.f;
    row[j] = x + p[j] * ld;
    key[j] = SWZ ? p[j] & 15 : 0;
  }
  f32x4 ab[2][SB][T][2];
  auto load_stage = [&](int buf, int b8, int st) {
#pragma unroll
    for (int i = 0; i < SB; ++i)
#pragma unroll
      for (int j = 0; j < T; ++j)
#pragma unroll
        for (int e = 0; e < 2; ++e)
          ab[buf][i][j][e] =
              *reinterpret_cast<const f32x4*>(row[j] + b8 * 64 + (((2 * (SB * st + i) + e) ^ key[j]) << 2));
  };
  auto block = [&](const f32x4 (&wv)[16], int b8, int b8next) {
#pragma unroll
    for (int st = 0; st < NS; ++st) {
      if (st + 1 < NS)
        load_stage((st + 1) & 1, b8, st + 1);
      else
        load_stage(0, b8next, 0);
      __builtin_amdgcn_sched_barrier(0);
#pragma unroll
      for (int i = 0; i < SB; ++i)
#pragma unroll
        for (int j = 0; j < T; ++j)
#pragma unroll
          for (int s = 0; s < 4; ++s) {
            y[j] = fmaf(wv[2 * (SB * st + i)][s], ab[st & 1][i][j][0][s], y[j]);
            y[j] = fmaf(wv[2 * (SB * st + i) + 1][s], ab[st & 1][i][j][1][s], y[j]);
          }
      __builtin_amdgcn_sched_barrier(0);
    }
  };
  load_stage(0, 0, 0);
#pragma unroll 1
  for (int it = 0; it < NKC8 / 2; ++it) {
    screen_load_w(wb[1], w + (2 * it + 1) * 8 * 64);
    __builtin_amdgcn_sched_barrier(0);
    block(wb[0], 2 * it, 2 * it + 1);
    screen_load_w(wb[0], it + 1 < NKC8 / 2 ? w + (2 * it + 2) * 8 * 64 : wnext);
    __builtin_amdgcn_sched_barrier(0);
    block(wb[1], 2 * it + 1, (2 * it + 2) % NKC8);
  }
  float m = y[0];
#pragma unroll
  for (int j = 1; j < T; ++j) m = fmaxf(m, y[j]);
  return m;
}

#define SCREEN_POOL_CAP 512
static_assert(SCREEN_POOL_CAP >= 64 && SCREEN_POOL_CAP * 4 + 256 * 8 <= 8 * 64 * 8, "a channel's 64 candidates fit; list + sets fit the wave's 4 KiB");

template <int T, int K, bool SWZ>
__device__ __forceinline__ void screen_replay_pool(const f32x4* __restrict__ wbase, const float* x, int ld, unsigned* list,
                                                   int e0, int total, int lane) {
  constexpr int WB = 2, RING = 4, WL = K >= 512 ? 3 : 2, AL = K >= 512 ? 2 : 1, NKC8 = K / 64;
  static_assert(WB * RING == 8, "one trip of the loop is one group of 8 chunks (64 floats of a row)");
  float y[T];
  const f32x4* w[T];
  const float* row[T];
  int key[T];
  bool live[T];
#pragma unroll
  for (int j = 0; j < T; ++j) {
    const int idx = e0 + 64 * j + lane;
    live[j] = idx < total;
    const unsigned ent = list[live[j] ? idx : e0];
    const int cw = ent >> 8, p = ent & 63;
    y[j] = 0.f;
    w[j] = wbase + (size_t)(cw >> 5) * (K / 8) * 64 + (cw & 31);
    row[j] = x + p * ld;
    key[j] = SWZ ? p & 15 : 0;
  }
  f32x4 wv[RING][WB][T][2], ab[RING][WB][T][2];
  auto load_w = [&](int slot, int g8, int b) {
#pragma unroll
    for (int i = 0; i < WB; ++i)
#pragma unroll
      for (int j = 0; j < T; ++j)
#pragma unroll
        for (int e = 0; e < 2; ++e) wv[slot][i][j][e] = w[j][(g8 * 8 + WB * b + i) * 64 + 32 * e];
  };
  auto load_a = [&](int slot, int g8, int b) {
#pragma unroll
    for (int i = 0; i < WB; ++i)
#pragma unroll
      for (int j = 0; j < T; ++j)
#pragma unroll
        for (int e = 0; e < 2; ++e)
          ab[slot][i][j][e] = *reinterpret_cast<const f32x4*>(row[j] + g8 * 64 + (((2 * (WB * b + i) + e) ^ key[j]) << 2));
  };
#pragma unroll
  for (int b = 0; b < WL; ++b) load_w(b, 0, b);
#pragma unroll
  for (int b = 0; b < AL; ++b) load_a(b, 0, b);
  __builtin_amdgcn_sched_barrier(0);
#pragma unroll 1
  for (int g8 = 0; g8 < NKC8; ++g8) {
    const int gn = g8 + 1 < NKC8 ? g8 + 1 : 0;
#pragma unroll
    for (int b = 0; b < RING; ++b) {
      load_w((b + WL) % RING, b + WL < RING ? g8 : gn, (b + WL) % RING);
      load_a((b + AL) % RING, b + AL < RING ? g8 : gn, (b + AL) % RING);
      __builtin_amdgcn_sched_barrier(0);
#pragma unroll
      for (int i = 0; i < WB; ++i)
#pragma unroll
        for (int j = 0; j < T; ++j)
#pragma unroll
          for (int s = 0; s < 4; ++s) {
            y[j] = fmaf(wv[b][i][j][0][s], ab[b][i][j][0][s], y[j]);
            y[j] = fmaf(wv[b][i][j][1][s], ab[b][i][j][1][s], y[j]);
          }
      __builtin_amdgcn_sched_barrier(0);
    }
  }
#pragma unroll
  for (int j = 0; j < T; ++j)
    if (live[j]) list[e0 + 64 * j + lane] = __float_as_uint(y[j]);
}

template <int K, bool SWZ, int LAYER, bool RUN = false>
__device__ __forceinline__ void screen_pool_store(const f32x4* __restrict__ wbase, const float* x, int ld,
                                                  unsigned long long* sets, float* __restrict__ out,
                                                  const float* __restrict__ bias, int ch0, bool relu, int lane,
                                                  float* frun = nullptr, bool first = true) {
  unsigned* list = reinterpret_cast<unsigned*>(sets + 256);
  float best[4] = {-INFINITY, -INFINITY, -INFINITY, -INFINITY};
  if constexpr (RUN) {
    if (!first) {
      const f32x4 f = *reinterpret_cast<const f32x4*>(frun + ch0 + 4 * lane);
#pragma unroll
      for (int j = 0; j < 4; ++j) best[j] = f[j];
    }
  }
#ifdef CATRE_DEBUG_TRACE
  int entries = 0, rounds = 0, batches = 0;
#endif
  int start = 0;
#pragma unroll 1
  while (start < 256) {
    int c[4], off[4], s = 0;
#pragma unroll
    for (int j = 0; j < 4; ++j) {
      c[j] = 4 * lane + j >= start ? __popcll(sets[4 * lane + j]) : 0;
      s += c[j];
    }
    int incl = s;
#pragma unroll
    for (int o = 1; o < 64; o <<= 1) {
      const int t = lane_get(incl, lane - o);
      if (lane >= o) incl += t;
    }
    int run = incl - s, end = 0, last[4];
#pragma unroll
    for (int j = 0; j < 4; ++j) {
      off[j] = run;
      run += c[j];
      last[j] = run;
      end += __popcll(__ballot(run <= SCREEN_POOL_CAP));
    }
    const int sel = (end - 1) & 3;
    const int total = lane_get(sel == 0 ? last[0] : sel == 1 ? last[1] : sel == 2 ? last[2] : last[3], (end - 1) >> 2);
#pragma unroll
    for (int j = 0; j < 4; ++j) {
      const int cw = 4 * lane + j;
      if (cw >= start && cw < end) {
        unsigned long long m = sets[cw];
        int o = off[j];
        while (m) {
          const int bit = __builtin_ctzll(m);
          m &= m - 1;
          const int p = ((bit >> 4) & 1) * 32 + (bit & 3) + 8 * ((bit & 15) >> 2) + 4 * (bit >> 5);
          list[o++] = (unsigned)(cw << 8 | p);
        }
      }
    }
    __builtin_amdgcn_fence(__ATOMIC_ACQ_REL, "wavefront");
    __builtin_amdgcn_wave_barrier();
#pragma unroll 1
    for (int e0 = 0; e0 < total; e0 += 128) {
      if (total - e0 > 64)
        screen_replay_pool<2, K, SWZ>(wbase, x, ld, list, e0, total, lane);
      else
        screen_replay_pool<1, K, SWZ>(wbase, x, ld, list, e0, total, lane);
    }
    __builtin_amdgcn_fence(__ATOMIC_ACQ_REL, "wavefront");
    __builtin_amdgcn_wave_barrier();
#pragma unroll
    for (int j = 0; j < 4; ++j) {
      const int cw = 4 * lane + j;
      if (cw >= start && cw < end)
        for (int i = 0; i < c[j]; ++i) best[j] = fmaxf(best[j], __uint_as_float(list[off[j] + i]));
    }
    __builtin_amdgcn_fence(__ATOMIC_ACQ_REL, "wavefront");
    __builtin_amdgcn_wave_barrier();
#ifdef CATRE_DEBUG_TRACE
    entries += total;
    rounds += (total + 63) >> 6;
    ++batches;
#endif
    start = end;
  }
  if constexpr (RUN) {
    *reinterpret_cast<f32x4*>(frun + ch0 + 4 * lane) = f32x4{best[0], best[1], best[2], best[3]};
    __builtin_amdgcn_fence(__ATOMIC_RELEASE, "workgroup");
  }
  const f32x4 b = *reinterpret_cast<const f32x4*>(bias + ch0 + 4 * lane);
  f32x4 v;
#pragma unroll
  for (int j = 0; j < 4; ++j) {
    v[j] = best[j] + b[j];
    if (relu) v[j] = fmaxf(v[j], 0.f);
  }
  *reinterpret_cast<f32x4*>(out + ch0 + 4 * lane) = v;
#ifdef CATRE_DEBUG_TRACE
  if (lane == 0) {
    SCREEN_COUNT(LAYER, 32 + (rounds < 15 ? rounds : 15), 1ull);
    if (batches > 1) SCREEN_COUNT(LAYER, 48, 1ull);
    SCREEN_COUNT(LAYER, 49, 1ull);
    SCREEN_COUNT(LAYER, 50, entries);
    SCREEN_COUNT(LAYER, 51, rounds);
    if (entries == 0) SCREEN_COUNT(LAYER, 52, 1ull);
  }
#endif
}

template <int MB, int K, bool SWZ = true, int LAYER = 0, bool POOL = false, bool RUN = false>
__device__ __forceinline__ void screen_select_store(const f32x16 (&acc)[MB][2], const f32x4* __restrict__ wf,
                                                    const float* __restrict__ nw, const float* na, const float* x,
                                                    unsigned long long* sets, float* __restrict__ out,
                                                    const float* __restrict__ bias, int ch0, bool relu, int valid, int tile,
                                                    const ScreenArgs& sc, int lane, int ld = K, float* frun = nullptr,
                                                    bool first = true) {
  static_assert(POOL || !RUN, "the run form refines the pooled replay");
  constexpr int NKC8 = K / 64;
  const int n = lane & 31, h = lane >> 5;
  const int partner = (lane ^ 32) << 2;
  auto swap32 = [&](auto v) { return __builtin_bit_cast(decltype(v), __builtin_amdgcn_ds_bpermute(partner, __builtin_bit_cast(int, v))); };
  f32x4 wb[2][16];
  if constexpr (!POOL) screen_load_w(wb[0], wf);
  {
    f32x4 na4[2][4];
#pragma unroll
    for (int nb = 0; nb < 2; ++nb)
#pragma unroll
      for (int g = 0; g < 4; ++g) na4[nb][g] = *reinterpret_cast<const f32x4*>(na + nb * 32 + 8 * g + 4 * h);
    unsigned vmask = 0xffffffffu;
    if (valid < TP) {
      vmask = 0;
#pragma unroll
      for (int i = 0; i < 32; ++i)
        if ((i >> 4) * 32 + (i & 3) + 8 * ((i & 15) >> 2) + 4 * h < valid) vmask |= 1u << i;
    }
    float fc[RUN ? MB : 1];
    if constexpr (RUN) {
      __builtin_amdgcn_fence(__ATOMIC_ACQUIRE, "workgroup");
#pragma unroll
      for (int mb = 0; mb < MB; ++mb) fc[mb] = -INFINITY;
      if (!first) {
#pragma unroll
        for (int mb = 0; mb < MB; ++mb) fc[mb] = frun[ch0 + mb * 32 + n];
      }
    }
#pragma unroll
    for (int mb = 0; mb < MB; ++mb) {
      float e1, e0;
      screen_eps_coef<K>(nw[ch0 + mb * 32 + n], e1, e0);
      float L = -INFINITY;
      if constexpr (RUN) L = fc[mb];
#pragma unroll
      for (int nb = 0; nb < 2; ++nb)
#pragma unroll
        for (int r = 0; r < 16; ++r) L = fmaxf(L, acc[mb][nb][r] - fmaf(e1, na4[nb][r >> 2][r & 3], e0));
      L = fmaxf(L, swap32(L));
      unsigned own = 0;
#pragma unroll
      for (int nb = 0; nb < 2; ++nb)
#pragma unroll
        for (int r = 0; r < 16; ++r)
          own |= (acc[mb][nb][r] + fmaf(e1, na4[nb][r >> 2][r & 3], e0) >= L) ? 1u << (nb * 16 + r) : 0u;
      own &= vmask;
      if (sc.probe_s) {
#pragma unroll
        for (int nb = 0; nb < 2; ++nb)
#pragma unroll
          for (int r = 0; r < 16; ++r) {
            const size_t o = ((size_t)tile * 1024 + ch0 + mb * 32 + n) * TP + nb * 32 + (r & 3) + 8 * (r >> 2) + 4 * h;
            sc.probe_s[o] = acc[mb][nb][r];
            sc.probe_eps[o] = fmaf(e1, na4[nb][r >> 2][r & 3], e0);
          }
      }
      const unsigned other = swap32(own);
      unsigned long long m64 = h ? ((unsigned long long)own << 32) | other : ((unsigned long long)other << 32) | own;
      if (m64 == 0 && (!RUN || L == -INFINITY)) m64 = 1;
      if constexpr (POOL) {
#ifdef CATRE_DEBUG_TRACE
        const int c = __popcll(m64);
        if (h == 0) SCREEN_COUNT(LAYER, c < 31 ? c : 31, 1ull);
#endif
        sets[mb * 32 + n] = m64;
      } else {
        sets[mb * 64 + lane] = m64;
      }
    }
  }
  if constexpr (POOL) {
    static_assert(MB == 8, "lane l owns channels 4 l .. 4 l + 3 of the wave's 256");
    __builtin_amdgcn_fence(__ATOMIC_ACQ_REL, "wavefront");
    __builtin_amdgcn_wave_barrier();
    screen_pool_store<K, SWZ, LAYER, RUN>(wf - n, x, ld, sets, out, bias, ch0, relu, lane, frun, first);
    return;
  }
#ifdef CATRE_DEBUG_TRACE
  int tmax = 0;
#endif
#pragma unroll 1
  for (int mb = 0; mb < MB; ++mb) {
    const unsigned long long m64 = sets[mb * 64 + lane];
    const float b = bias[ch0 + mb * 32 + n];
    int c = __popcll(m64);
#ifdef CATRE_DEBUG_TRACE
    if (h == 0) SCREEN_COUNT(LAYER, c < 31 ? c : 31, 1ull);
#endif
    int trips = 1;
    while (trips < TP / 2 && __ballot(c > 2 * trips)) ++trips;
#ifdef CATRE_DEBUG_TRACE
    if (lane == 0) SCREEN_COUNT(LAYER, 32 + (trips < 15 ? trips : 15), 1ull);
    tmax = trips > tmax ? trips : tmax;
#endif
    const int pad = __builtin_ctzll(m64);
    unsigned long long m = m64;
    if (h) m &= m - 1;
    const f32x4* w = wf + (size_t)mb * (K / 8) * 64;
    const f32x4* wn = mb + 1 < MB ? w + (K / 8) * 64 : w;
    float best = -INFINITY;
#pragma unroll 1
    for (int done = 0; done < trips; done += SCREEN_CMAX) {
      int p[SCREEN_CMAX];
#pragma unroll
      for (int j = 0; j < SCREEN_CMAX; ++j) {
        const int bit = m ? __builtin_ctzll(m) : pad;
        m &= m - 1;
        m &= m - 1;
        p[j] = ((bit >> 4) & 1) * 32 + (bit & 3) + 8 * ((bit & 15) >> 2) + 4 * (bit >> 5);
      }
      const int rem = trips - done;
      const f32x4* nxt = rem > SCREEN_CMAX ? w : wn;
      float v;
      if (rem == 1)
        v = screen_replay<1, NKC8, SWZ>(w, nxt, wb, x, ld, p);
      else if (rem == 2)
        v = screen_replay<2, NKC8, SWZ>(w, nxt, wb, x, ld, p);
      else
        v = screen_replay<SCREEN_CMAX, NKC8, SWZ>(w, nxt, wb, x, ld, p);
      best = fmaxf(best, v);
    }
    best = fmaxf(best, swap32(best));
    if (lane < 32) {
      const float v = best + b;
      out[ch0 + mb * 32 + lane] = relu ? fmaxf(v, 0.f) : v;
    }
  }
#ifdef CATRE_DEBUG_TRACE
  if (lane == 0) {
    if (tmax > SCREEN_CMAX) SCREEN_COUNT(LAYER, 48, 1ull);
    SCREEN_COUNT(LAYER, 49, 1ull);
  }
#endif
}

template <bool POOL, bool RUN = false>
struct Trunk4ScreenT {
  ScreenArgs sc;
  float* frun;
  bool first;
  const f32x4* wf;
  const float* b4;
  ScreenPipe8<2> g4;
  f32x16 acc4[8][2];
  __device__ __forceinline__ void prefetch(const f32x4* __restrict__ wp4, const float* __restrict__ b4_, int mb0, int lane) {
    wf = wp4 + ((size_t)mb0 * 64) * 64 + (lane & 31);
    b4 = b4_;
    g4.prefetch(sc.wps + ((size_t)mb0 * 32) * 64 + lane);
  }
  __device__ __forceinline__ void sweep(const float* a3, float* a2, int tid, int lane) {
    screen_row_norms<512, 256>(a3, a2, tid);
    __syncthreads();
#pragma unroll
    for (int mb = 0; mb < 8; ++mb) acc4[mb][0] = acc4[mb][1] = zero16();
    g4.run(acc4, a3, lane);
  }
  __device__ __forceinline__ void store(const float* a3, float* a2, float* __restrict__ pm, int tile, int mb0, int valid, int,
                                        const TrainSave&, int lane) {
    unsigned long long* sets = reinterpret_cast<unsigned long long*>(a2 + 64) + (mb0 >> 3) * 8 * 64;
    asm volatile("v_mbcnt_lo_u32_b32 %0, -1, 0\n\tv_mbcnt_hi_u32_b32 %0, -1, %0" : "=v"(lane));
    screen_select_store<8, 512, true, 0, POOL, RUN>(acc4, wf, sc.nw, a2, a3, sets, pm + (size_t)tile * PMW, b4, mb0 * 32,
                                                    false, valid, tile, sc, lane, 512, frun, first);
  }
};
typedef Trunk4ScreenT<false> Trunk4Screen;

__global__ __launch_bounds__(256) void k_trunk4s(catre_points P, const float* __restrict__ trans3,
                                                 const float* __restrict__ trans64, const float* __restrict__ Wc1,
                                                 const float* __restrict__ bc1, const f32x4* __restrict__ wp2,
                                                 const float* __restrict__ b2, const f32x4* __restrict__ wp3,
                                                 const float* __restrict__ b3, const f32x4* __restrict__ wp4,
                                                 const float* __restrict__ b4, float* __restrict__ pm,
                                                 float* __restrict__ pointfeat, int B, int N, int M,
                                                 unsigned long long* __restrict__ trace, ScreenArgs sc) {
  __shared__ __attribute__((aligned(16))) float smem[TRUNK_SMEM];
  Trunk4Screen tl;
  tl.sc = sc;
  trunk4_body<false>(smem, P, trans3, trans64, Wc1, bc1, wp2, b2, wp3, b3, wp4, b4, pm, pointfeat, B, N, M, trace,
                     TrainSave{}, tl, blockIdx.x, threadIdx.x);
}

__global__ __launch_bounds__(256) void k_trunk4sp(catre_points P, const float* __restrict__ trans3,
                                                  const float* __restrict__ trans64, const float* __restrict__ Wc1,
                                                  const float* __restrict__ bc1, const f32x4* __restrict__ wp2,
                                                  const float* __restrict__ b2, const f32x4* __restrict__ wp3,
                                                  const float* __restrict__ b3, const f32x4* __restrict__ wp4,
                                                  const float* __restrict__ b4, float* __restrict__ pm,
                                                  float* __restrict__ pointfeat, int B, int N, int M,
                                                  unsigned long long* __restrict__ trace, ScreenArgs sc) {
  __shared__ __attribute__((aligned(16))) float smem[TRUNK_SMEM];
  Trunk4ScreenT<true> tl;
  tl.sc = sc;
  trunk4_body<false>(smem, P, trans3, trans64, Wc1, bc1, wp2, b2, wp3, b3, wp4, b4, pm, pointfeat, B, N, M, trace,
                     TrainSave{}, tl, blockIdx.x, threadIdx.x);
}

__device__ __forceinline__ void run_info(int rid, int B, int N, int M, int S, int& tile0, int& nt) {
  const int TN = (N + TP - 1) / TP, TM = (M + TP - 1) / TP;
  const int RN = (TN + S - 1) / S, RM = (TM + S - 1) / S;
  if (rid < B * RN) {
    const int k = rid % RN;
    tile0 = (rid / RN) * TN + k * S;
    nt = min(S, TN - k * S);
  } else {
    const int r = rid - B * RN, k = r % RM;
    tile0 = B * TN + (r / RM) * TM + k * S;
    nt = min(S, TM - k * S);
  }
}

struct TrunkRunArgs {
  catre_points P;
  const float *trans3, *trans64, *Wc1, *bc1;
  const f32x4* wp2;
  const float* b2;
  const f32x4* wp3;
  const float* b3;
  const f32x4* wp4;
  const float* b4;
  float *pm, *pointfeat;
  unsigned long long* trace;
  ScreenArgs sc;
  float* frun;
  int B, N, M, S;
};

__global__ __launch_bounds__(256) void k_trunk4sr(TrunkRunArgs args) {
  __shared__ __attribute__((aligned(16))) float smem[TRUNK_SMEM];
  typedef const __attribute__((address_space(4))) TrunkRunArgs* ArgPtr;
  ArgPtr ap = (ArgPtr)__builtin_amdgcn_kernarg_segment_ptr();
  (void)args;
  const int wave = __builtin_amdgcn_readfirstlane(threadIdx.x >> 6);
  int tile0, nt;
  run_info(blockIdx.x, ap->B, ap->N, ap->M, ap->S, tile0, nt);
#pragma unroll 1
  for (int t = 0; t < nt; ++t) {
    int lane;
    asm volatile("v_mbcnt_lo_u32_b32 %0, -1, 0\n\tv_mbcnt_hi_u32_b32 %0, -1, %0" : "=v"(lane));
    asm volatile("" : "+s"(ap));
    const TrunkRunArgs a = *(const TrunkRunArgs*)ap;
    Trunk4ScreenT<true, true> tl;
    tl.sc = a.sc;
    tl.frun = a.frun + (size_t)blockIdx.x * 1024;
    tl.first = t == 0;
    trunk4_body<false>(smem, a.P, a.trans3, a.trans64, a.Wc1, a.bc1, a.wp2, a.b2, a.wp3, a.b3, a.wp4, a.b4, a.pm, a.pointfeat,
                       a.B, a.N, a.M, a.trace, TrainSave{}, tl, tile0 + t, wave * 64 + lane);
    __syncthreads();
  }
}

typedef ScreenPipe8<2, 8, false, LD128> StnScreenPipe;

template <int LAYER, bool POOL, bool RUN = false>
__device__ __forceinline__ void stn_conv3_screened(const float* img, float* scratch, StnScreenPipe& g,
                                                   const f32x4* __restrict__ wp3, const float* __restrict__ b3,
                                                   float* __restrict__ pm, int tile0, int valid2, const ScreenArgs& sc,
                                                   float* __restrict__ probe_rows, int wave, int tid, int lane,
                                                   float* frun = nullptr, bool first_pair = true) {
  const int nt = valid2 > TP ? 2 : 1, mb0 = wave * 8;
  screen_row_norms<128, 256, 2 * TP, false>(img, scratch, tid, LD128);
  if (probe_rows) {
    for (int i = tid; i < nt * TP * 32; i += 256)
      *reinterpret_cast<f32x4*>(probe_rows + ((size_t)tile0 * TP + (i >> 5)) * 128 + (i & 31) * 4) =
          *reinterpret_cast<const f32x4*>(img + (i >> 5) * LD128 + (i & 31) * 4);
  }
  __syncthreads();
  unsigned long long* sets = reinterpret_cast<unsigned long long*>(scratch + 2 * TP) + wave * 8 * 64;
  auto tile = [&](int t, int ln) {
    f32x16 acc[8][2];
#pragma unroll
    for (int mb = 0; mb < 8; ++mb) acc[mb][0] = acc[mb][1] = zero16();
    const float* x = img + t * TP * LD128;
    g.run(acc, x, ln);
    asm volatile("v_mbcnt_lo_u32_b32 %0, -1, 0\n\tv_mbcnt_hi_u32_b32 %0, -1, %0" : "=v"(ln));
    const f32x4* wf = wp3 + ((size_t)mb0 * 16) * 64 + (ln & 31);
    screen_select_store<8, 128, false, LAYER, POOL, RUN>(acc, wf, sc.nw, scratch + t * TP, x, sets,
                                                         pm + (size_t)(tile0 + t) * PMW, b3, mb0 * 32, true,
                                                         min(valid2 - t * TP, TP), tile0 + t, sc, ln, LD128, frun,
                                                         first_pair && t == 0);
  };
  tile(0, lane);
  if (nt == 2) {
    asm volatile("v_mbcnt_lo_u32_b32 %0, -1, 0\n\tv_mbcnt_hi_u32_b32 %0, -1, %0" : "=v"(lane));
    g.prefetch(sc.wps + ((size_t)mb0 * 8) * 64 + lane);
    tile(1, lane);
  }
}

template <bool POOL, bool RUN = false>
__device__ __forceinline__ void stn3d_pair_s_body(catre_points P, const float* __restrict__ W1,
                                                  const float* __restrict__ b1, const f32x4* __restrict__ wp2,
                                                  const float* __restrict__ b2, const f32x4* __restrict__ wp3,
                                                  const float* __restrict__ b3, float* __restrict__ pm, int B, int N,
                                                  int M, const ScreenArgs& sc, float* __restrict__ probe_rows,
                                                  const int bid, const int tid, float* frun = nullptr,
                                                  bool first_pair = true) {
  __shared__ __attribute__((aligned(16))) float smem[2 * TP * LD64 + 2 * TP * LD128];
  float* a1 = smem;
  float* a2 = smem + 2 * TP * LD64;
  const int lane = tid & 63;
  const int wave = __builtin_amdgcn_readfirstlane(tid >> 6);
  TileInfo ti;
  int tile0;
  pair_info32(bid, B, N, M, ti, tile0);

  GemmPipe<1, 4, false, false, 8, 3> g2;
  g2.prefetch(wp2 + (wave * 8) * 64 + lane, 0);
  f32x4 bv2[1][4];
  load_bias_quads<1>(bv2, b2, wave * 32, lane);
  {
    const int p = (wave & 1) * TP + lane;
    float x, y, z;
    load_point(P, ti, p, x, y, z);
    conv3_relu_row<32>(x, y, z, W1, b1, (wave >> 1) * 32, a1 + p * LD64);
  }
  __syncthreads();
  StnScreenPipe g3;
  g3.prefetch(sc.wps + ((size_t)wave * 8 * 8) * 64 + lane);
  {
    f32x16 acc[1][4] = {{zero16(), zero16(), zero16(), zero16()}};
    g2.run(acc, a1, LD64, lane);
    store_tile_lds_pre<1, 4, true, false>(acc, a2, LD128, wave * 32, bv2, lane);
  }
  __syncthreads();
  stn_conv3_screened<1, POOL, RUN>(a2, a1, g3, wp3, b3, pm, tile0, ti.valid, sc, probe_rows, wave, tid, lane, frun, first_pair);
}
#define STN3D_PAIR_S_(NAME, POOL)                                                                                          \
  __global__ __launch_bounds__(256) void NAME(catre_points P, const float* __restrict__ W1, const float* __restrict__ b1, \
                                              const f32x4* __restrict__ wp2, const float* __restrict__ b2,                \
                                              const f32x4* __restrict__ wp3, const float* __restrict__ b3,                \
                                              float* __restrict__ pm, int B, int N, int M, ScreenArgs sc,                 \
                                              float* __restrict__ probe_rows) {                                           \
    stn3d_pair_s_body<POOL>(P, W1, b1, wp2, b2, wp3, b3, pm, B, N, M, sc, probe_rows, blockIdx.x, threadIdx.x);          \
  }
STN3D_PAIR_S_(k_stn3d_pair_s, false)
STN3D_PAIR_S_(k_stn3d_pair_sp, true)
#undef STN3D_PAIR_S_

template <bool POOL, bool RUN = false>
__device__ __forceinline__ void stnkd_pair_s_body(catre_points P, const float* __restrict__ trans3,
                                                  const float* __restrict__ Wc1, const float* __restrict__ bc1,
                                                  const f32x4* __restrict__ wpf1, const float* __restrict__ bf1,
                                                  const f32x4* __restrict__ wpf2, const float* __restrict__ bf2,
                                                  const f32x4* __restrict__ wpf3, const float* __restrict__ bf3,
                                                  float* __restrict__ pm, int B, int N, int M, const ScreenArgs& sc,
                                                  float* __restrict__ probe_rows, const int bid, const int tid,
                                                  float* frun = nullptr, bool first_pair = true) {
  __shared__ __attribute__((aligned(16))) float smem[4 * TP * LD64 + 2 * TP * LD128];
  float* h1 = smem;
  float* f1 = smem + 2 * TP * LD64;
  float* f2 = smem + 4 * TP * LD64;
  const int lane = tid & 63;
  const int wave = __builtin_amdgcn_readfirstlane(tid >> 6);
  TileInfo ti;
  int tile0;
  pair_info32(bid, B, N, M, ti, tile0);

  const int mblk1 = wave >> 1, half1 = wave & 1;
  GemmPipe<1, 2, false, false, 8, 4> g1;
  g1.prefetch(wpf1 + (mblk1 * 8) * 64 + lane, 0);
  f32x4 bv1[1][4];
  load_bias_quads<1>(bv1, bf1, mblk1 * 32, lane);
  {
    const int p = (wave & 1) * TP + lane;
    float x, y, z;
    load_point(P, ti, p, x, y, z);
    apply_t3(trans3 + ti.cloud * 9, x, y, z);
    conv3_relu_row<32>(x, y, z, Wc1, bc1, (wave >> 1) * 32, h1 + p * LD64);
  }
  __syncthreads();
  GemmPipe<1, 4, false, false, 8, 3> g2;
  g2.prefetch(wpf2 + (wave * 8) * 64 + lane, 0);
  f32x4 bv2[1][4];
  load_bias_quads<1>(bv2, bf2, wave * 32, lane);
  __builtin_amdgcn_sched_barrier(0);
  {
    f32x16 acc[1][2] = {{zero16(), zero16()}};
    g1.run(acc, h1 + half1 * TP * LD64, LD64, lane);
    store_tile_lds_pre<1, 2, true, false>(acc, f1 + half1 * TP * LD64, LD64, mblk1 * 32, bv1, lane);
  }
  __syncthreads();
  StnScreenPipe g3;
  g3.prefetch(sc.wps + ((size_t)wave * 8 * 8) * 64 + lane);
  {
    f32x16 acc[1][4] = {{zero16(), zero16(), zero16(), zero16()}};
    g2.run(acc, f1, LD64, lane);
    store_tile_lds_pre<1, 4, true, false>(acc, f2, LD128, wave * 32, bv2, lane);
  }
  __syncthreads();
  stn_conv3_screened<2, POOL, RUN>(f2, h1, g3, wpf3, bf3, pm, tile0, ti.valid, sc, probe_rows, wave, tid, lane, frun, first_pair);
}
#define STNKD_PAIR_S_(NAME, POOL)                                                                                      \
  __global__ __launch_bounds__(256) void NAME(                                                                        \
      catre_points P, const float* __restrict__ trans3, const float* __restrict__ Wc1, const float* __restrict__ bc1, \
      const f32x4* __restrict__ wpf1, const float* __restrict__ bf1, const f32x4* __restrict__ wpf2,                  \
      const float* __restrict__ bf2, const f32x4* __restrict__ wpf3, const float* __restrict__ bf3,                   \
      float* __restrict__ pm, int B, int N, int M, ScreenArgs sc, float* __restrict__ probe_rows) {                   \
    stnkd_pair_s_body<POOL>(P, trans3, Wc1, bc1, wpf1, bf1, wpf2, bf2, wpf3, bf3, pm, B, N, M, sc, probe_rows,       \
                            blockIdx.x, threadIdx.x);                                                                  \
  }
STNKD_PAIR_S_(k_stnkd_pair_s, false)
STNKD_PAIR_S_(k_stnkd_pair_sp, true)
#undef STNKD_PAIR_S_

__device__ __forceinline__ void pair_run_info(int rid, int B, int N, int M, int SP, int& pair0, int& np) {
  const int PN = ((N + TP - 1) / TP + 1) / 2, PM_ = ((M + TP - 1) / TP + 1) / 2;
  const int RN = (PN + SP - 1) / SP, RM = (PM_ + SP - 1) / SP;
  if (rid < B * RN) {
    const int k = rid % RN;
    pair0 = (rid / RN) * PN + k * SP;
    np = min(SP, PN - k * SP);
  } else {
    const int r = rid - B * RN, k = r % RM;
    pair0 = B * PN + (r / RM) * PM_ + k * SP;
    np = min(SP, PM_ - k * SP);
  }
}

struct Stn3dRunArgs {
  catre_points P;
  const float *W1, *b1;
  const f32x4* wp2;
  const float* b2;
  const f32x4* wp3;
  const float* b3;
  float* pm;
  const u32x4* wps;
  const float* nw;
  int B, N, M, SP;
};

__global__ __launch_bounds__(256) void k_stn3d_pair_sr(Stn3dRunArgs args) {
  __shared__ __attribute__((aligned(16))) float frun[1024];
  typedef const __attribute__((address_space(4))) Stn3dRunArgs* ArgPtr;
  ArgPtr ap = (ArgPtr)__builtin_amdgcn_kernarg_segment_ptr();
  (void)args;
  const int wave = __builtin_amdgcn_readfirstlane(threadIdx.x >> 6);
  int pair0, np;
  pair_run_info(blockIdx.x, ap->B, ap->N, ap->M, ap->SP, pair0, np);
  *reinterpret_cast<f32x4*>(frun + 4 * threadIdx.x) = f32x4{-INFINITY, -INFINITY, -INFINITY, -INFINITY};
  __syncthreads();
#pragma unroll 1
  for (int bid = pair0, end = pair0 + np; bid < end; ++bid) {
    int lane;
    asm volatile("v_mbcnt_lo_u32_b32 %0, -1, 0\n\tv_mbcnt_hi_u32_b32 %0, -1, %0" : "=v"(lane));
    asm volatile("" : "+s"(ap));
    const Stn3dRunArgs a = *(const Stn3dRunArgs*)ap;
    stn3d_pair_s_body<true, true>(a.P, a.W1, a.b1, a.wp2, a.b2, a.wp3, a.b3, a.pm, a.B, a.N, a.M,
                                  ScreenArgs{a.wps, a.nw, nullptr, nullptr}, nullptr, bid, wave * 64 + lane, frun, false);
    __syncthreads();
  }
}

struct StnkdRunArgs {
  catre_points P;
  const float *trans3, *Wc1, *bc1;
  const f32x4* wpf1;
  const float* bf1;
  const f32x4* wpf2;
  const float* bf2;
  const f32x4* wpf3;
  const float* bf3;
  float* pm;
  const u32x4* wps;
  const float* nw;
  int B, N, M, SP;
};

__global__ __launch_bounds__(256) void k_stnkd_pair_sr(StnkdRunArgs args) {
  __shared__ __attribute__((aligned(16))) float frun[1024];
  typedef const __attribute__((address_space(4))) StnkdRunArgs* ArgPtr;
  ArgPtr ap = (ArgPtr)__builtin_amdgcn_kernarg_segment_ptr();
  (void)args;
  const int wave = __builtin_amdgcn_readfirstlane(threadIdx.x >> 6);
  int pair0, np;
  pair_run_info(blockIdx.x, ap->B, ap->N, ap->M, ap->SP, pair0, np);
  *reinterpret_cast<f32x4*>(frun + 4 * threadIdx.x) = f32x4{-INFINITY, -INFINITY, -INFINITY, -INFINITY};
  __syncthreads();
#pragma unroll 1
  for (int bid = pair0, end = pair0 + np; bid < end; ++bid) {
    int lane;
    asm volatile("v_mbcnt_lo_u32_b32 %0, -1, 0\n\tv_mbcnt_hi_u32_b32 %0, -1, %0" : "=v"(lane));
    asm volatile("" : "+s"(ap));
    const StnkdRunArgs a = *(const StnkdRunArgs*)ap;
    stnkd_pair_s_body<true, true>(a.P, a.trans3, a.Wc1, a.bc1, a.wpf1, a.bf1, a.wpf2, a.bf2, a.wpf3, a.bf3, a.pm, a.B, a.N, a.M,
                                  ScreenArgs{a.wps, a.nw, nullptr, nullptr}, nullptr, bid, wave * 64 + lane, frun, false);
    __syncthreads();
  }
}
```

catre_amd/hip.py:

```python
import ctypes
import os

import torch

_HERE = os.path.dirname(os.path.abspath(__file__))
LIB_PATH = os.environ.get("CATRE_HIP_LIB") or os.path.join(_HERE, "csrc", "libcatre_hip.so")

PARAM_KEYS = (
    [f"pcl_net.stn.{l}.{p}" for l in ("conv1", "conv2", "conv3", "fc1", "fc2", "fc3") for p in ("weight", "bias")]
    + [f"pcl_net.{l}.{p}" for l in ("conv1", "conv2", "conv3", "conv4") for p in ("weight", "bias")]
    + [f"pcl_net.fstn.{l}.{p}" for l in ("conv1", "conv2", "conv3", "fc1", "fc2", "fc3") for p in ("weight", "bias")]
    + [
        f"rot_head.rot_head_{a}.{l}.{p}"
        for a in ("x", "y")
        for l in ("layers.0", "layers.1", "layers.3", "layers.4", "neck.0", "conv_p")
        for p in ("weight", "bias")
    ]
    + [
        f"ts_head.{l}.{p}"
        for l in ("linears.0", "linears.1", "linears.3", "linears.4", "fc_t", "fc_s")
        for p in ("weight", "bias")
    ]
)
CATRE_P_COUNT = len(PARAM_KEYS)
# ... 87 lines not shown
    "catre_op_gemm_rows_nr": (_I, [_P, _I, _P, _I, _P, _P, _P, _I, _P, _P, _I, _I, _I, _I, _I, _P, _I, _P]),
    "catre_op_gemm_tn_bias_nr": (_I, [_P, _I, _P, _I, _P, _I, _P, _P, _P, _I, _I, _I, _I, _P, _SZ, _P, _I, _P]),
    "catre_train_stn3d_fwd": (_I, [_P, _P, _P, _P, _P, _P, _P, _P, _SZ, _I, _I, _I, _I, _P]),
    "catre_train_stnkd_fwd": (_I, [_P, _P, _P, _P, _P, _P, _P, _P, _P, _SZ, _I, _I, _I, _I, _P]),
    "catre_train_trunk_fwd": (_I, [_P] * 12 + [_P, _SZ, _I, _I, _I, _I, _P]),
    "catre_pose_apply": (_I, [_P, _P, _P, _P, _P, _P, _I, _I, _I, _I, _P]),
    "catre_stn3d_pool": (_I, [_P, _P, _P, _P, _P, _SZ, _I, _I, _I, _P]),
    "catre_linear": (_I, [_P, _I, _P, _I, _P, _P, _I, _I, _I, _I, _I, _I, _P]),
    "catre_linear_t": (_I, [_P, _I, _P, _P, _I, _P, _I, _I, _I, _I, _P]),
    "catre_stnkd_pool": (_I, [_P, _P, _P, _P, _P, _P, _SZ, _I, _I, _I, _P]),
    "catre_trunk": (_I, [_P, _P, _P, _P, _P, _P, _P, _P, _SZ, _I, _I, _I, _P]),
    "catre_packed_floats_w": (_SZ, [_I]),
    "catre_pack_encoder_w": (_I, [_P, _I, _P, _SZ, _P]),
    "catre_trunk_w": (_I, [_P, _P, _P, _P, _P, _I, _P, _P, _P, _SZ, _I, _I, _I, _P]),
    "catre_trunk_screen_probe": (_I, [_P, _P, _P, _P, _P, _P, _P, _P, _P, _P, _SZ, _I, _I, _I, _P]),
    "catre_ts_head": (_I, [_P, _P, _P, _P, _P, _P, _P, _P, _P, _SZ, _I, _P]),
    "catre_rot_head": (_I, [_P, _P, _P, _P, _P, _P, _SZ, _I, _I, _I, _P]),
    "catre_rot_head_dim": (_I, [_P, _P, _P, _P, _P, _P, _SZ, _I, _I, _I, _I, _P]),
    "catre_rot_to_mat": (_I, [_P, _I, _P, _I, _P]),
    "catre_rot_to_mat_bwd": (_I, [_P, _I, _P, _P, _I, _P]),
    "catre_pose_update": (_I, [_P, _P, _P, _P, _P, _P, _P, _P, _P, _P, _I, _P]),
    "catre_refine_iter": (_I, [_P, _P, _P, _P, _P, _P, _P, _P, _P, _P, _P, _SZ, _I, _I, _I, _P]),
    "catre_refine_k": (_I, [_P, _P, _P, _P, _P, _P, _P, _P, _P, _P, _SZ, _I, _I, _I, _I, _P]),
    "catre_stn_screen_probe": (_I, [_I, _P, _P, _P, _P, _P, _P, _P, _P, _P, _SZ, _I, _I, _I, _P]),
    "catre_form_switch": (_I, [_I, _I]),
    "catre_screen_run_len": (_I, [_I]),
    "catre_screen_run_rule": (_I, [_I, _I, _I, _I]),
    "catre_refine_k_from": (_I, [_P, _P, _P, _P, _P, _P, _P, _P, _P, _P, _P, _P, _SZ, _I, _I, _I, _I, _P]),
    "catre_colmax": (_I, [_P, _P, _I, _I, _I, _P]),
    "catre_op_pack": (_I, [_P, _I, _I, _I, _I, _P, _P]),
    "catre_op_gemm_rows": (_I, [_P, _I, _P, _P, _P, _I, _P, _I, _I, _I, _I, _I, _P]),
    "catre_op_linear_maxpool_ws_bytes": (_SZ, [_I, _I]),
    "catre_op_linear_maxpool": (_I, [_P, _I, _P, _P, _P, _P, _I, _I, _I, _I, _I, _P, _SZ, _P]),
    "catre_op_pack_bf16": (_I, [_P, _I, _I, _I, _I, _P, _P]),
    "catre_op_gemm_rows_bf16": (_I, [_P, _I, _P, _I, _P, _P, _P, _I, _P, _I, _I, _I, _I, _I, _P]),
    "catre_op_linear_maxpool_bf16": (_I, [_P, _I, _P, _P, _P, _P, _I, _I, _I, _I, _I, _P, _SZ, _P]),
    "catre_op_gemm_rows_cloudbias": (_I, [_P, _I, _P, _P, _P, _I, _I, _I, _I, _I, _I, _I, _P]),
    "catre_op_gemm_rows_gn": (_I, [_P, _I, _P, _P, _I, _P, _I, _I, _I, _I, _I, _I, _P, _I, _P]),
    "catre_op_gnp_gelu_fwd_pre": (_I, [_P, _P, _P, _P, _P, _P, _I, _I, _P]),
    "catre_op_pack_split": (_I, [_P, _I, _I, _I, _I, _P, _P]),
    "catre_op_gemm_rows_split": (_I, [_P, _I, _P, _I, _P, _P, _P, _I, _P, _I, _I, _I, _I, _I, _P]),
    "catre_op_linear_maxpool_split": (_I, [_P, _I, _P, _P, _P, _P, _I, _I, _I, _I, _I, _P, _SZ, _P]),
    "catre_op_gemm_tn_ws_bytes": (_SZ, [_I, _I, _I]),
    "catre_op_gemm_tn": (_I, [_P, _I, _P, _I, _P, _I, _I, _I, _I, _P, _SZ, _P]),
    "catre_op_gemm_rows_m": (_I, [_P, _I, _P, _I, _P, _P, _P, _I, _P, _I, _I, _I, _I, _I, _P]),
    "catre_op_gemm_tn_bias_m": (_I, [_P, _I, _P, _I, _P, _I, _P, _P, _I, _I, _I, _I, _P, _SZ, _P]),
    "catre_op_gemm_tn_bias_lp": (_I, [_P, _I, _P, _I, _P, _I, _P, _P, _I, _I, _I, _I, _P, _SZ, _I, _P]),
    "catre_op_gemm_tn_bias_ws_bytes": (_SZ, [_I, _I, _I]),
    "catre_op_fc_bwd": (_I, [_P, _I, _P, _P, _I, _P, _I, _P, _P, _P, _I, _I, _I, _I, _I, _P]),
    "catre_op_skinny_bwd": (_I, [_P, _I, _P, _I, _P, _I, _P, _I, _P, _I, _I, _P, _P, _P, _I, _I, _I, _P, _SZ, _P]),
    "catre_op_gemm_tn_bias": (_I, [_P, _I, _P, _I, _P, _P, _I, _I, _I, _I, _P, _SZ, _P]),
    "catre_op_colsum": (_I, [_P, _I, _I, _I, _P, _I, _P, _SZ, _P]),
    "catre_op_reduce_splits": (_I, [_P, _P, _I, _I, _I, _P]),
    "catre_op_rowbias_add": (_I, [_P, _I, _P, _I, _I, _I, _I, _P]),
    "catre_op_rowbias_bwd": (_I, [_P, _I, _P, _I, _I, _I, _I, _P]),
    "catre_op_maxpool_fwd": (_I, [_P, _I, _P, _P, _I, _I, _I, _I, _P]),
    "catre_op_maxpool_scatter": (_I, [_P, _P, _P, _I, _I, _I, _P]),
    "catre_op_maxlin_bwd_w": (_I, [_P, _P, _P, _I, _P, _P, _I, _I, _I, _P]),
    "catre_op_maxlin_bwd_w_h": (_I, [_P, _P, _P, _I, _P, _P, _I, _I, _I, _P]),
    "catre_op_maxlin_bwd_x": (_I, [_P, _P, _P, _I, _P, _I, _I, _I, _I, _P]),
    "catre_op_maxlin_bwd_x_rows": (_I, [_P, _P, _P, _I, _P, _I, _I, _I, _I, _I, _I, _P]),
    "catre_op_cloud_matmul": (_I, [_P, _I, _P, _P, _I, _I, _I, _I, _I, _I, _P]),
    "catre_op_cloud_matmul_bwd_t": (_I, [_P, _I, _P, _I, _P, _I, _I, _I, _I, _P]),
    "catre_op_relu_bwd": (_I, [_P, _P, _P, _SZ, _P]),
    "catre_op_sum_rows": (_I, [_P, _P, _P, _I, _P, _I, _I, _I, _P]),
    "catre_op_gnp_gelu_fwd": (_I, [_P, _P, _P, _P, _P, _I, _I, _P]),
    "catre_op_gnp_gelu_neck_fwd": (_I, [_P, _P, _P, _P, _P, _P, _P, _P, _I, _I, _P]),
    "catre_op_gnp_gelu_neck_bwd_ws_bytes": (_SZ, [_I, _I]),
    "catre_op_gnp_gelu_neck_bwd": (_I, [_P, _P, _P, _P, _P, _P, _P, _P, _I, _P, _SZ, _I, _I, _P]),
    "catre_op_rot_l0_bwd_ws_bytes": (_SZ, [_I, _I, _I]),
    "catre_op_rot_l0_bwd": (_I, [_P, _P, _P, _P, _P, _P, _I, _P, _P, _I, _P, _P, _P, _P, _I, _P, _SZ, _I, _I, _I, _P]),
    "catre_op_rot_l0_bwd_lp": (_I, [_P, _P, _P, _P, _P, _P, _I, _P, _P, _I, _P, _P, _P, _P, _I, _P, _SZ, _I, _I, _I, _P]),
    "catre_op_rot_l0_bwd_sp": (_I, [_P, _P, _P, _P, _P, _P, _I, _P, _P, _I, _P, _P, _P, _P, _I, _P, _SZ, _I, _I, _I, _P]),
    "catre_op_gnp_gelu_neck_fwd_s": (_I, [_P] * 10 + [_I, _I, _P]),
    "catre_op_rot_l1_bwd_s": (_I, [_P] * 14 + [_SZ, _I, _I, _P]),
    "catre_op_rot_l1_bwd_lp": (_I, [_P] * 14 + [_SZ, _I, _I, _P]),
    "catre_op_rot_l1_bwd_sp": (_I, [_P] * 14 + [_SZ, _I, _I, _P]),
    "catre_op_rot_l1_bwd_h": (_I, [_P] * 14 + [_SZ, _I, _I, _P]),
    "catre_op_rot_l0_bwd_h": (_I, [_P, _P, _P, _P, _P, _P, _I, _P, _P, _I, _P, _P, _P, _P, _I, _P, _SZ, _I, _I, _I, _P]),
    "catre_op_gemm_rows_gn_h": (_I, [_P, _I, _P, _P, _I, _P, _I, _I, _I, _I, _I, _I, _P, _I, _P]),
    "catre_op_gnp_gelu_fwd_pre_h": (_I, [_P, _P, _P, _P, _P, _P, _I, _I, _P]),
    "catre_op_gnp_gelu_neck_fwd_s_h": (_I, [_P] * 10 + [_I, _I, _P]),
    "catre_op_gn_gelu_gemm_rows_h": (_I, [_P] * 10 + [_I, _I, _I, _P]),
    "catre_op_gnp_gelu_neck_bwd_s": (_I, [_P] * 11 + [_SZ, _I, _I, _P]),
    "catre_op_pad_cols": (_I, [_P, ctypes.c_long, ctypes.c_long, _I, _I, _P, _I, _P]),
    "catre_op_rot_l1_bwd_ws_bytes": (_SZ, [_I, _I]),
    "catre_op_rot_l1_bwd": (_I, [_P, _P, _P, _P, _P, _P, _P, _P, _P, _P, _P, _P, _SZ, _I, _I, _P]),
    "catre_op_gnp_gelu_bwd": (_I, [_P, _P, _P, _P, _P, _P, _P, _P, _I, _P, _SZ, _I, _I, _P]),
    "catre_op_gnr_gelu_fwd": (_I, [_P, _P, _P, _P, _I, _P]),
    "catre_op_gnr_gelu_bwd": (_I, [_P, _P, _P, _P, _P, _P, _P, _I, _P, _SZ, _I, _P]),
    "catre_op_gnp_act_fwd": (_I, [_P] * 5 + [_I] * 6 + [_P]),
    "catre_op_gnp_act_bwd_ws_bytes": (_SZ, [_I, _I, _I, _I]),
    "catre_op_gnp_act_bwd": (_I, [_P] * 8 + [_I, _P, _SZ] + [_I] * 6 + [_P]),
    "catre_op_gnr_act_fwd": (_I, [_P] * 4 + [_I] * 5 + [_P]),
    "catre_op_gnr_act_bwd_ws_bytes": (_SZ, [_I, _I]),
    "catre_op_gnr_act_bwd": (_I, [_P] * 7 + [_I, _P, _SZ] + [_I] * 5 + [_P]),
    "catre_op_gnp_act_neck_wsum_ws_bytes": (_SZ, [_I, _I, _I]),
    "catre_op_gnp_act_neck_wsum": (_I, [_P] * 9 + [_SZ] + [_I] * 7 + [_P]),
    "catre_op_wsum_fwd": (_I, [_P, _P, _P, _P, _I, _I, _P]),
    "catre_op_wsum_bwd": (_I, [_P, _P, _P, _P, _P, _P, _I, _P, _SZ, _I, _I, _P]),
    "catre_op_wsum_bwd_n": (_I, [_P, _P, _P, _P, _P, _P, _P, _I, _P, _SZ, _I, _I, _P]),
    "catre_op_pose_update_bwd": (_I, [_P] * 13 + [_I, _P]),
    "catre_train_rot_fwd_ws_bytes": (_SZ, [_I]),
    "catre_train_rot_fwd": (_I, [_P] * 10 + [_SZ, _I, _I, _I, _I, _P]),
    "catre_op_ranger_step": (_I, [_P, _I, _P, _I, _P, _I, _P, ctypes.c_double, ctypes.c_double, ctypes.c_float,
                                  ctypes.c_float, _I, ctypes.c_float, _P]),
    "catre_op_optim_step": (_I, [_I, _P, _I, _P, _I, _P, _I, _I, _P, _SZ, _I, ctypes.c_float, _P]),
    "catre_aug_points": (_I, [_P] * 10 + [_I, _I, _P]),
    "catre_init_noise": (_I, [_P, _P, _P, ctypes.c_float, ctypes.c_float, _P, _P, _P, ctypes.c_float, ctypes.c_float, _P, _I,
                              _P]),
    "catre_pcl_workspace_bytes": (_SZ, [_I, _I, _I]),
    "catre_pcl_candidates": (_I, [_P, _P, _P, _P, _P, ctypes.c_float, _I, _I, _I, _I, _P, _SZ, _P, _P]),
    "catre_pcl_sample": (_I, [_P, _P, _P, _SZ, _P, ctypes.c_uint64, _I, _I, _I, _I, _P, _P, _P]),
    "catre_pcl_fps": (_I, [_P, _P, _P, _SZ, _I, _I, _I, _I, _P, _I, _P, _P]),
    "catre_pclf_workspace_bytes": (_SZ, [_I, _I, _I, _I]),
    "catre_pclf_candidates": (_I, [_P, _P, _P, _P, _P, _I, _P, _P, _P, ctypes.c_float, _I, _I, _I, _I, _I, _P, _SZ, _P, _P]),
    "catre_pclf_sample": (_I, [_P, _P, _P, _P, _P, _SZ, _P, _P, _I, _I, _I, _I, _I, _P, _P, _P]),
    "catre_pclf_fps": (_I, [_P, _P, _P, _P, _SZ, _I, _I, _I, _I, _I, _P, _I, _P, _P]),
    "catre_depth_augment": (_I, [_P, _I, ctypes.c_float, _P, _I, _P, _P, _P, ctypes.c_uint64, _P, _I, _I, _I, _P]),
    "catre_loss_fwd": (_I, [_P] * 15 + [_I, _I, _I, _P]),
    "catre_loss_bwd": (_I, [_P] * 14 + [_I, _I, _I, _P]),
    "catre_loss_fwd_sums": (_I, [_P] * 16 + [_I, _P, _I, _I, _I, _P]),
    "catre_loss_bwd_sums": (_I, [_P] * 13 + [_I, _P, _P, _P, _I, _I, _I, _P]),
    "catre_loss_fwd2": (_I, [_P] * 16 + [_I, _P, _I, _I, _I, _P]),
    "catre_loss_bwd2": (_I, [_P] * 13 + [_I, _P, _P, _P, _I, _I, _I, _P]),
    "catre_loss_fwd3": (_I, [_P] * 16 + [_I, _P, _I, _I, _I, _P, _P]),
    "catre_loss_bwd3": (_I, [_P] * 13 + [_I, _P, _P, _P, _I, _I, _I, _P, _P]),
    "catre_eval_overlaps": (_I, [_P] * 14 + [_I] * 6 + [_P]),
    "catre_eval_match_iou": (_I, [_P] * 7 + [_I] * 6 + [_P]),
    "catre_eval_match_pose": (_I, [_P] * 6 + [_I, _I] + [_P] * 4 + [_I] * 7 + [_P]),
    "catre_profile_enable": (_I, [_I, _I]),
    "catre_profile_collect": (_I, [_P, _I, _P]),
    "catre_debug_trunk_trace": (_I, [_P]),
    "catre_debug_knob": (_I, [_I, _I]),
    "catre_debug_screen_counts": (_I, [_P, _I]),
    "catre_stream_capture_id": (_I, [_P, _P]),
    "catre_status_string": (ctypes.c_char_p, [_I]),
    "catre_version": (ctypes.c_char_p, []),
}
EXPORTED_SYMBOLS = tuple(_SIGS)

KERNEL_IDS = {"stn3d": 0, "stnkd": 1, "trunk": 2, "ts_head": 3, "rot_l0_stats": 4, "rot_l1": 5, "rot_out": 6, "colmax": 7}

_lib = None

_param_epoch = [0]


def bump_param_epoch():
    _param_epoch[0] += 1


FORM_IDS = {"trunk4": 0, "stn4": 1, "stn_pair": 2, "rotw": 3, "fc_tail": 4, "screen": 5, "screen_stn": 6, "screen_pool": 7,
            "screen_run": 8}


def form_switch(name, value=None):
    r = load().catre_form_switch(FORM_IDS[name], -1 if value is None else int(bool(value)))
    if r < 0:
        raise CatreHipError(f"unknown kernel-form switch {name!r}")
    return bool(r)


def screen_run_len(value=None):
    return load().catre_screen_run_len(-1 if value is None else int(value))


def screen_run_rule(B, N, M, cus=256):
    return load().catre_screen_run_rule(B, N, M, cus)


def capture_id(device):
    out = ctypes.c_ulonglong(0)
    check(load().catre_stream_capture_id(stream_ptr(device), ctypes.byref(out)), "catre_stream_capture_id")
    return int(out.value)


def param_epoch():
    return _param_epoch[0]


class CatreHipError(RuntimeError):
    pass


def load():
    global _lib
    if _lib is not None:
        return _lib
    if not os.path.exists(LIB_PATH):
        raise CatreHipError(
            f"{LIB_PATH} not found - build it with `make -C catre_amd/csrc` (or `python -c "
            "'import __graft_entry__ as g; g.build()'`).  catre_amd has no CPU or PyTorch fallback."
        )
    lib = ctypes.CDLL(LIB_PATH)
    for name, (res, args) in _SIGS.items():
        fn = getattr(lib, name)
        fn.restype = res
        fn.argtypes = args
    _lib = lib
    return lib


def check(status, what):
    if status != 0:
        msg = load().catre_status_string(status).decode()
        raise CatreHipError(f"{what} failed: {msg} (status {status})")


_raw_stream = getattr(torch._C, "_cuda_getCurrentRawStream", None)


def stream_ptr(device=None):
    if _raw_stream is not None:
        if device is None:
            idx = torch.cuda.current_device()
        elif isinstance(device, int):
            idx = device
        else:
            if isinstance(device, str):
                device = torch.device(device)
            idx = device.index if device.index is not None else torch.cuda.current_device()
        return ctypes.c_void_p(_raw_stream(idx))
    return ctypes.c_void_p(torch.cuda.current_stream(device).cuda_stream)


def ptr(t):
    return ctypes.c_void_p(t.data_ptr()) if t is not None else ctypes.c_void_p(0)


def require_dev_f32(t, name, shape=None, contiguous=True):
    if not isinstance(t, torch.Tensor):
        raise TypeError(f"{name}: expected a torch.Tensor, got {type(t).__name__}")
    if not t.is_cuda:
        raise CatreHipError(
            f"{name} is on {t.device}; catre_amd runs on HIP devices only (no CPU fallback - the CPU "
            "restatement lives in oracle/ and is test infrastructure)"
        )
    if t.dtype != torch.float32:
        raise TypeError(f"{name}: expected float32, got {t.dtype}")
    if shape is not None:
        if t.dim() != len(shape) or any(e is not None and int(a) != int(e) for a, e in zip(t.shape, shape)):
            raise ValueError(f"{name}: expected shape {tuple(shape)}, got {tuple(t.shape)}")
    if contiguous and not t.is_contiguous():
        raise ValueError(f"{name}: must be contiguous")
    return t


def points_desc(x, tfd_kps):
    require_dev_f32(x, "x", (None, 3, None), contiguous=False)
    require_dev_f32(tfd_kps, "tfd_kps", (x.shape[0], 3, None), contiguous=False)
    d = CatrePoints()
    d.obs, d.obs_sb, d.obs_sc, d.obs_sn = x.data_ptr(), x.stride(0), x.stride(1), x.stride(2)
    d.kps, d.kps_sb, d.kps_sc, d.kps_sn = tfd_kps.data_ptr(), tfd_kps.stride(0), tfd_kps.stride(1), tfd_kps.stride(2)
    return d


def param_array(tensors):
    arr = (ctypes.c_void_p * CATRE_P_COUNT)()
    for i, t in enumerate(tensors):
        if t is None:
            arr[i] = None
        else:
            require_dev_f32(t, PARAM_KEYS[i])
            arr[i] = t.data_ptr()
    return arr


def profile_kernel(name, max_records):
    check(load().catre_profile_enable(-1 if name is None else KERNEL_IDS[name], int(max_records)), "catre_profile_enable")


def profile_collect(max_records):
    buf = (ctypes.c_float * max_records)()
    n = ctypes.c_int(0)
    check(load().catre_profile_collect(buf, max_records, ctypes.byref(n)), "catre_profile_collect")
    return [buf[i] for i in range(n.value)]
```

profiles/screen_candidates.py:

```python
import ctypes
import os
import sys

import torch

sys.path.insert(0, os.path.dirname(os.path.dirname(os.path.abspath(__file__))))
from catre_amd import hip, synth
from catre_amd.CATRE_disR_shared import build_model_optimizer, expected_state_shapes
from catre_amd.config import default_cfg

B, N, M, K = 256, 1024, 1024, 4
cfg = default_cfg(num_pcl=N, num_kps=M, n_iter=K, device="cuda:0")
model, _ = build_model_optimizer(cfg, is_test=True)
sd = synth.recipe_state_dict(expected_state_shapes(cfg))
model.load_state_dict({k: v.cuda() for k, v in sd.items()}, strict=True)
model.eval()
batch = {k: v.cuda() for k, v in synth.make_inputs(B, N, M, seed=1000).items()}
lib = hip.load()
hip.form_switch("screen", True)
hip.form_switch("screen_stn", True)
model.refine(batch, n_iter=K)
torch.cuda.synchronize()
cnt = (ctypes.c_ulonglong * (3 * 64))()
hip.check(lib.catre_debug_screen_counts(cnt, 1), "catre_debug_screen_counts (needs the TRACE=1 library)")
model.refine(batch, n_iter=K)
torch.cuda.synchronize()
hip.check(lib.catre_debug_screen_counts(cnt, 1), "catre_debug_screen_counts")
pool = hip.form_switch("screen_pool")
run = pool and hip.form_switch("screen_run")
run_stn = run and os.environ.get("CATRE_SCREEN_RUN_STN", "1") != "0"
S = (hip.screen_run_len() or hip.screen_run_rule(B, N, M, torch.cuda.get_device_properties(0).multi_processor_count)) if run else 1
lines = [f"B={B} N=M={N} K={K} refine, make_inputs(seed=1000), recipe weights; screen_pool {'on' if pool else 'off'}; "
         f"screen_run {'on, run length ' + str(S) + (' (STN kernels: ' + ('on' if run_stn else 'off') + ')') if run and S > 1 else 'off'}; "
         "per-channel replay: chains a lane carries at once: 4"]
for row, name in enumerate(("trunk conv4 (k_trunk4s)", "stn.conv3 (k_stn3d_pair_s)", "fstn.conv3 (k_stnkd_pair_s)")):
    c = list(cnt)[64 * row:64 * row + 64]
    pooled = c[51] > 0
    if pooled:
        name = name.replace("_s)", "_sp)").replace("k_trunk4s", "k_trunk4sp")
        if run and S > 1 and (row == 0 or run_stn):
            name = name.replace("sp)", "sr)")
    lines.append(f"screened {name}")
    tot = sum(c[:32])
    mean = sum(i * v for i, v in enumerate(c[:32])) / max(tot, 1)
    lines.append(f"candidates per (tile, channel): {tot} pairs, mean {mean:.4f} (bin 31 = 31 and more)")
    for i, v in enumerate(c[:32]):
        if v:
            lines.append(f"  {i:2d}: {v:10d}  {v / tot:.6f}")
    if pooled:
        lines.append(f"list entries per (wave, tile): mean {c[50] / max(c[49], 1):.2f}; rounds of 64 entries: mean "
                     f"{c[51] / max(c[49], 1):.4f} over {c[49]} units (bin 15 = 15 and more)")
        for i, v in enumerate(c[32:48]):
            if v:
                lines.append(f"  {i:2d}: {v:10d}  {v / max(c[49], 1):.6f}")
        lines.append(f"(wave, tile) units whose list filled up (replayed in more than one batch): {c[48]} of {c[49]}")
        lines.append(f"(wave, tile) units with an empty list: {c[52]} of {c[49]}")
        continue
    tt = sum(c[32:48])
    tmean = sum(i * v for i, v in enumerate(c[32:48])) / max(tt, 1)
    lines.append(f"replay trips per (wave, tile, 32-channel block): {tt} blocks, mean {tmean:.4f} (bin 15 = 15 and more)")
    for i, v in enumerate(c[32:48]):
        if v:
            lines.append(f"  {i:2d}: {v:10d}  {v / tt:.6f}")
    lines.append(f"(wave, tile) units with a block of more than 4 trips (a further replay round): {c[48]} of {c[49]} = "
                 f"{c[48] / max(c[49], 1):.5f}")
text = "\n".join(lines) + "\n"
print(text, end="")
if len(sys.argv) > 1:
    open(sys.argv[1], "w").write(text)
```

Baseline: 47250 object-iterations/s.

## Run max-pool screening pass in fp16 MFMA with rigorous per-row error bounds

Adds an fp16 variant of the screening GEMM for trunk conv4 and the STN conv3 layers. Weights are pre-scaled per row by a power of two and packed to fp16, and each row's residual norm is computed so the screen's error bound stays valid. Activation tiles are scaled the same way at runtime. Doing the candidate-screening matmul at half precision is meant to cut its MFMA and bandwidth cost, in exchange for looser bounds that may let more candidates through to exact fp32 replay, plus extra packing kernels and workspace.

```diff
diff --git a/catre_amd/csrc/catre_kernels.hip b/catre_amd/csrc/catre_kernels.hip
--- a/catre_amd/csrc/catre_kernels.hip
+++ b/catre_amd/csrc/catre_kernels.hip
@@ -1457,6 +1457,7 @@
   size_t sp_stn_c2, sp_stn_c3, sp_fstn_c1, sp_fstn_c2, sp_fstn_c3, sp_c3, sp_c4, sp_rot_l0[2], sp_rot_l1[2];
   size_t f16_stn_c2, f16_stn_c3, f16_fstn_c1, f16_fstn_c2, f16_fstn_c3, f16_c2, f16_c3, f16_c4, f16_rot_l0[2], f16_rot_l1[2];
   size_t scr_c4, scr_nw4, scr_stn_c3, scr_fstn_c3, scr_nw_stn, scr_nw_fstn;
+  size_t s16_c4, s16_stn_c3, s16_fstn_c3, s16_uw4, s16_uw_stn, s16_uw_fstn;
 };
 
 PackLayout pack_layout(int ts_in) {
@@ -1521,6 +1522,12 @@
   L.scr_fstn_c3 = take(1024 * 128);
   L.scr_nw_stn = take(1024);
   L.scr_nw_fstn = take(1024);
+  L.s16_c4 = take(1024 * 512 / 2);
+  L.s16_stn_c3 = take(1024 * 128 / 2);
+  L.s16_fstn_c3 = take(1024 * 128 / 2);
+  L.s16_uw4 = take(2 * 1024);
+  L.s16_uw_stn = take(2 * 1024);
+  L.s16_uw_fstn = take(2 * 1024);
   L.ts_w0t = take((size_t)ts_in * 256);
   L.ts_w1t = take(256 * 256);
   L.total = o;
@@ -1650,7 +1657,7 @@
 }
 
 enum { FORM_TRUNK4 = 1, FORM_STN4 = 2, FORM_STN_PAIR = 4, FORM_ROTW = 8, FORM_FC_TAIL = 16, FORM_SCREEN = 32, FORM_SCREEN_STN = 64,
-       FORM_SCREEN_POOL = 128, FORM_SCREEN_RUN = 256 };
+       FORM_SCREEN_POOL = 128, FORM_SCREEN_RUN = 256, FORM_SCREEN_F16 = 512 };
 #ifndef CATRE_SCREEN_DEFAULT
 #define CATRE_SCREEN_DEFAULT true
 #endif
@@ -1662,6 +1669,9 @@
 #endif
 #ifndef CATRE_SCREEN_RUN_DEFAULT
 #define CATRE_SCREEN_RUN_DEFAULT true
+#endif
+#ifndef CATRE_SCREEN_F16_DEFAULT
+#define CATRE_SCREEN_F16_DEFAULT true
 #endif
 static std::atomic<int> g_forms{-1};
 static int forms() {
@@ -1676,7 +1686,8 @@
         (on("CATRE_FC_TAIL", false) ? FORM_FC_TAIL : 0) | (on("CATRE_SCREEN", CATRE_SCREEN_DEFAULT) ? FORM_SCREEN : 0) |
         (on("CATRE_SCREEN_STN", CATRE_SCREEN_STN_DEFAULT) ? FORM_SCREEN_STN : 0) |
         (on("CATRE_SCREEN_POOL", CATRE_SCREEN_POOL_DEFAULT) ? FORM_SCREEN_POOL : 0) |
-        (on("CATRE_SCREEN_RUN", CATRE_SCREEN_RUN_DEFAULT) ? FORM_SCREEN_RUN : 0);
+        (on("CATRE_SCREEN_RUN", CATRE_SCREEN_RUN_DEFAULT) ? FORM_SCREEN_RUN : 0) |
+        (on("CATRE_SCREEN_F16", CATRE_SCREEN_F16_DEFAULT) ? FORM_SCREEN_F16 : 0);
     g_forms.store(v, std::memory_order_relaxed);
   }
   return v;
@@ -1727,6 +1738,14 @@
   static const bool stn = [] { const char* e = getenv("CATRE_SCREEN_RUN_STN"); return e ? atoi(e) != 0 : CATRE_SCREEN_RUN_STN_DEFAULT; }();
   return screen_run_on() && screen_stn_on() && screen_pool_stn_on() && stn;
 }
+static bool screen_f16_on() { return (forms() & (FORM_SCREEN_POOL | FORM_SCREEN_F16)) == (FORM_SCREEN_POOL | FORM_SCREEN_F16); }
+#ifndef CATRE_SCREEN_F16_STN_DEFAULT
+#define CATRE_SCREEN_F16_STN_DEFAULT true
+#endif
+static bool screen_f16_stn_on() {
+  static const bool stn = [] { const char* e = getenv("CATRE_SCREEN_F16_STN"); return e ? atoi(e) != 0 : CATRE_SCREEN_F16_STN_DEFAULT; }();
+  return screen_f16_on() && screen_pool_stn_on() && stn;
+}
 inline int stn_pair_runs(int B, int N, int M, int SP) {
   return B * ((((N + TP - 1) / TP + 1) / 2 + SP - 1) / SP + (((M + TP - 1) / TP + 1) / 2 + SP - 1) / SP);
 }
@@ -1777,15 +1796,20 @@
 #undef LAUNCH_
   } else if (const int S = stn_pair_form(tiles, B, N, M) && screen_run_stn_on() && !probe_s ? screen_run_len(B, N, M) : 1; S > 1) {
     const int SP = S / 2;
-    hipLaunchKernelGGL(k_stn3d_pair_sr, dim3(stn_pair_runs(B, N, M, SP)), dim3(256), 0, st,
+    const bool f16 = screen_f16_stn_on();
+    hipLaunchKernelGGL(f16 ? k_stn3d_pair_sr16 : k_stn3d_pair_sr, dim3(stn_pair_runs(B, N, M, SP)), dim3(256), 0, st,
                        Stn3dRunArgs{*pts, prm[CATRE_P_STN_CONV1_W], prm[CATRE_P_STN_CONV1_B], pk4(packed, L.stn_c2),
                                     prm[CATRE_P_STN_CONV2_B], pk4(packed, L.stn_c3), prm[CATRE_P_STN_CONV3_B], ws + W.pm,
-                                    pkb(packed, L.scr_stn_c3), packed + L.scr_nw_stn, B, N, M, SP});
+                                    pkb(packed, f16 ? L.s16_stn_c3 : L.scr_stn_c3), packed + L.scr_nw_stn, B, N, M, SP,
+                                    packed + L.s16_uw_stn});
   } else if (stn_pair_form(tiles, B, N, M) && (screen_stn_on() || probe_s)) {
-    hipLaunchKernelGGL(screen_pool_stn_on() ? k_stn3d_pair_sp : k_stn3d_pair_s, dim3(stn_pairs(B, N, M)), dim3(256), 0, st, *pts, prm[CATRE_P_STN_CONV1_W],
+    const bool f16 = screen_f16_stn_on();
+    hipLaunchKernelGGL(f16 ? k_stn3d_pair_sp16 : screen_pool_stn_on() ? k_stn3d_pair_sp : k_stn3d_pair_s, dim3(stn_pairs(B, N, M)), dim3(256), 0, st, *pts, prm[CATRE_P_STN_CONV1_W],
                        prm[CATRE_P_STN_CONV1_B], pk4(packed, L.stn_c2), prm[CATRE_P_STN_CONV2_B], pk4(packed, L.stn_c3),
                        prm[CATRE_P_STN_CONV3_B], ws + W.pm, B, N, M,
-                       ScreenArgs{pkb(packed, L.scr_stn_c3), packed + L.scr_nw_stn, probe_s, probe_eps}, probe_rows);
+                       ScreenArgs{pkb(packed, f16 ? L.s16_stn_c3 : L.scr_stn_c3), packed + L.scr_nw_stn, probe_s, probe_eps,
+                                  packed + L.s16_uw_stn},
+                       probe_rows);
   } else if (stn_pair_form(tiles, B, N, M)) {
     const int pairs = stn_pairs(B, N, M);
     hipLaunchKernelGGL(k_stn3d_pair<false>, dim3(pairs), dim3(256), 0, st, *pts, prm[CATRE_P_STN_CONV1_W], prm[CATRE_P_STN_CONV1_B],
@@ -1821,16 +1845,21 @@
 #undef LAUNCH_
   } else if (const int S = stn_pair_form(tiles, B, N, M) && screen_run_stn_on() && !probe_s ? screen_run_len(B, N, M) : 1; S > 1) {
     const int SP = S / 2;
-    hipLaunchKernelGGL(k_stnkd_pair_sr, dim3(stn_pair_runs(B, N, M, SP)), dim3(256), 0, st,
+    const bool f16 = screen_f16_stn_on();
+    hipLaunchKernelGGL(f16 ? k_stnkd_pair_sr16 : k_stnkd_pair_sr, dim3(stn_pair_runs(B, N, M, SP)), dim3(256), 0, st,
                        StnkdRunArgs{*pts, trans3, prm[CATRE_P_CONV1_W], prm[CATRE_P_CONV1_B], pk4(packed, L.fstn_c1),
                                     prm[CATRE_P_FSTN_CONV1_B], pk4(packed, L.fstn_c2), prm[CATRE_P_FSTN_CONV2_B],
                                     pk4(packed, L.fstn_c3), prm[CATRE_P_FSTN_CONV3_B], ws + W.pm,
-                                    pkb(packed, L.scr_fstn_c3), packed + L.scr_nw_fstn, B, N, M, SP});
+                                    pkb(packed, f16 ? L.s16_fstn_c3 : L.scr_fstn_c3), packed + L.scr_nw_fstn, B, N, M, SP,
+                                    packed + L.s16_uw_fstn});
   } else if (stn_pair_form(tiles, B, N, M) && (screen_stn_on() || probe_s)) {
-    hipLaunchKernelGGL(screen_pool_stn_on() ? k_stnkd_pair_sp : k_stnkd_pair_s, dim3(stn_pairs(B, N, M)), dim3(256), 0, st, *pts, trans3, prm[CATRE_P_CONV1_W],
+    const bool f16 = screen_f16_stn_on();
+    hipLaunchKernelGGL(f16 ? k_stnkd_pair_sp16 : screen_pool_stn_on() ? k_stnkd_pair_sp : k_stnkd_pair_s, dim3(stn_pairs(B, N, M)), dim3(256), 0, st, *pts, trans3, prm[CATRE_P_CONV1_W],
                        prm[CATRE_P_CONV1_B], pk4(packed, L.fstn_c1), prm[CATRE_P_FSTN_CONV1_B], pk4(packed, L.fstn_c2),
                        prm[CATRE_P_FSTN_CONV2_B], pk4(packed, L.fstn_c3), prm[CATRE_P_FSTN_CONV3_B], ws + W.pm, B, N, M,
-                       ScreenArgs{pkb(packed, L.scr_fstn_c3), packed + L.scr_nw_fstn, probe_s, probe_eps}, probe_rows);
+                       ScreenArgs{pkb(packed, f16 ? L.s16_fstn_c3 : L.scr_fstn_c3), packed + L.scr_nw_fstn, probe_s, probe_eps,
+                                  packed + L.s16_uw_fstn},
+                       probe_rows);
   } else if (stn_pair_form(tiles, B, N, M)) {
     const int pairs = stn_pairs(B, N, M);
     hipLaunchKernelGGL(k_stnkd_pair<false>, dim3(pairs), dim3(256), 0, st, *pts, trans3, prm[CATRE_P_CONV1_W], prm[CATRE_P_CONV1_B],
@@ -1869,17 +1898,21 @@
   } else if (const int S = row_split8(tiles) == 1 && trunk4_on() && screen_on() && screen_run_on() ? screen_run_len(B, N, M) : 1;
              S > 1) {
     const int runs = B * (((N + TP - 1) / TP + S - 1) / S + ((M + TP - 1) / TP + S - 1) / S);
-    hipLaunchKernelGGL(k_trunk4sr, dim3(runs), dim3(256), 0, st,
+    const bool f16 = screen_f16_on();
+    hipLaunchKernelGGL(f16 ? k_trunk4sr16 : k_trunk4sr, dim3(runs), dim3(256), 0, st,
                        TrunkRunArgs{*pts, trans3, trans64, prm[CATRE_P_CONV1_W], prm[CATRE_P_CONV1_B], pk4(packed, L.c2),
                                     prm[CATRE_P_CONV2_B], pk4(packed, L.c3), prm[CATRE_P_CONV3_B], pk4(packed, L.c4),
                                     prm[CATRE_P_CONV4_B], ws + W.pm, pointfeat, g_trunk_trace,
-                                    ScreenArgs{pkb(packed, L.scr_c4), packed + L.scr_nw4, probe_s, probe_eps}, ws + W.frun,
-                                    B, N, M, S});
+                                    ScreenArgs{pkb(packed, f16 ? L.s16_c4 : L.scr_c4), packed + L.scr_nw4, probe_s, probe_eps,
+                                               packed + L.s16_uw4},
+                                    ws + W.frun, B, N, M, S});
   } else if (row_split8(tiles) == 1 && trunk4_on() && (screen_on() || probe_s)) {
-    hipLaunchKernelGGL(screen_pool_on() ? k_trunk4sp : k_trunk4s, dim3(tiles), dim3(256), 0, st, *pts, trans3, trans64,
+    const bool f16 = screen_f16_on();
+    hipLaunchKernelGGL(f16 ? k_trunk4sp16 : screen_pool_on() ? k_trunk4sp : k_trunk4s, dim3(tiles), dim3(256), 0, st, *pts, trans3, trans64,
                        prm[CATRE_P_CONV1_W], prm[CATRE_P_CONV1_B], pk4(packed, L.c2), prm[CATRE_P_CONV2_B], pk4(packed, L.c3),
                        prm[CATRE_P_CONV3_B], pk4(packed, L.c4), prm[CATRE_P_CONV4_B], ws + W.pm, pointfeat, B, N, M,
-                       g_trunk_trace, ScreenArgs{pkb(packed, L.scr_c4), packed + L.scr_nw4, probe_s, probe_eps});
+                       g_trunk_trace,
+                       ScreenArgs{pkb(packed, f16 ? L.s16_c4 : L.scr_c4), packed + L.scr_nw4, probe_s, probe_eps, packed + L.s16_uw4});
   } else if (row_split8(tiles) == 1 && trunk4_on()) {
     hipLaunchKernelGGL(k_trunk4<false>, dim3(tiles), dim3(256), 0, st, *pts, trans3, trans64, prm[CATRE_P_CONV1_W],
                        prm[CATRE_P_CONV1_B], pk4(packed, L.c2), prm[CATRE_P_CONV2_B], pk4(packed, L.c3),
@@ -2048,16 +2081,31 @@
     flush_lp(LP_SPLIT);
     hipLaunchKernelGGL(k_screen_wnorm, dim3(1024 / 4), dim3(256), 0, st, prm[CATRE_P_CONV4_W], 512, 1024, 512,
                        packed + L.scr_nw4);
+    hipLaunchKernelGGL(k_pack_screen_f16, dim3(1024 * 512 / 256), dim3(256), 0, st, prm[CATRE_P_CONV4_W], 512, 1024, 512,
+                       packed + L.scr_nw4, reinterpret_cast<unsigned short*>(packed + L.s16_c4), packed + L.s16_uw4);
+    hipLaunchKernelGGL(k_screen_f16_dw, dim3(1024 / 4), dim3(256), 0, st, prm[CATRE_P_CONV4_W], 512, 1024, 512,
+                       packed + L.scr_nw4, packed + L.s16_uw4 + 1024);
   }
   frag_sp(prm[CATRE_P_STN_CONV3_W], 128, 1024, 128, L.scr_stn_c3);
   frag_sp(prm[CATRE_P_FSTN_CONV3_W], 128, 1024, 128, L.scr_fstn_c3);
   flush_lp(LP_SPLIT);
-  if (prm[CATRE_P_STN_CONV3_W])
+  if (prm[CATRE_P_STN_CONV3_W]) {
     hipLaunchKernelGGL(k_screen_wnorm, dim3(1024 / 4), dim3(256), 0, st, prm[CATRE_P_STN_CONV3_W], 128, 1024, 128,
                        packed + L.scr_nw_stn);
-  if (prm[CATRE_P_FSTN_CONV3_W])
+    hipLaunchKernelGGL(k_pack_screen_f16, dim3(1024 * 128 / 256), dim3(256), 0, st, prm[CATRE_P_STN_CONV3_W], 128, 1024, 128,
+                       packed + L.scr_nw_stn, reinterpret_cast<unsigned short*>(packed + L.s16_stn_c3), packed + L.s16_uw_stn);
+    hipLaunchKernelGGL(k_screen_f16_dw, dim3(1024 / 4), dim3(256), 0, st, prm[CATRE_P_STN_CONV3_W], 128, 1024, 128,
+                       packed + L.scr_nw_stn, packed + L.s16_uw_stn + 1024);
+  }
+  if (prm[CATRE_P_FSTN_CONV3_W]) {
     hipLaunchKernelGGL(k_screen_wnorm, dim3(1024 / 4), dim3(256), 0, st, prm[CATRE_P_FSTN_CONV3_W], 128, 1024, 128,
                        packed + L.scr_nw_fstn);
+    hipLaunchKernelGGL(k_pack_screen_f16, dim3(1024 * 128 / 256), dim3(256), 0, st, prm[CATRE_P_FSTN_CONV3_W], 128, 1024, 128,
+                       packed + L.scr_nw_fstn, reinterpret_cast<unsigned short*>(packed + L.s16_fstn_c3),
+                       packed + L.s16_uw_fstn);
+    hipLaunchKernelGGL(k_screen_f16_dw, dim3(1024 / 4), dim3(256), 0, st, prm[CATRE_P_FSTN_CONV3_W], 128, 1024, 128,
+                       packed + L.scr_nw_fstn, packed + L.s16_uw_fstn + 1024);
+  }
   }
   for (int h = 0; h < 2 && head32; ++h) {
     const int base = h ? CATRE_P_ROTY_L0_W : CATRE_P_ROTX_L0_W;
@@ -2710,7 +2758,7 @@
 
 
 int catre_form_switch(int id, int value) {
-  if (id < 0 || id > 8) return -1;
+  if (id < 0 || id > 9) return -1;
   const int bit = 1 << id;
   const int cur = forms();
   if (value >= 0) g_forms.store(value ? (cur | bit) : (cur & ~bit), std::memory_order_relaxed);
diff --git a/catre_amd/csrc/catre_screen.h b/catre_amd/csrc/catre_screen.h
--- a/catre_amd/csrc/catre_screen.h
+++ b/catre_amd/csrc/catre_screen.h
@@ -12,6 +12,25 @@
   e0 = ScreenBound<K>::delta * (nw + 1.f) * ScreenBound<K>::infl;
 }
 
+template <int K>
+struct ScreenBoundF16 {
+  static_assert(K == 128 || K == 512, "rk is tabulated");
+  static constexpr float gamma = 0x1p-11f + 0x1p-21f + 2.f * K * 0x1p-23f;
+  static constexpr float rk = (K == 128 ? 11.32f : 22.63f) * 0x1p-12f;
+  static constexpr float infl = 1.f + 0x1p-22f / gamma + 0x1p-19f;
+};
+template <int K>
+__device__ __forceinline__ void screen_eps_coef_f16(float nw, float uw, float dw, float ua, float& e1, float& e0) {
+  typedef ScreenBoundF16<K> SB;
+  e1 = fmaf(SB::gamma, nw, fmaf(1.f + 0x1p-10f, dw, SB::rk * uw)) * SB::infl;
+  e0 = fmaf(SB::rk * nw, ua, fmaf(K * 0x1p-24f * uw, ua, K * 0x1p-122f)) * SB::infl;
+}
+__device__ __forceinline__ int screen_f16_exp(float n) {
+  const int s = 14 - ((int)((__float_as_uint(n) >> 23) & 0xff) - 127);
+  return s > 60 ? 60 : s;
+}
+__device__ __forceinline__ float screen_pow2(int e) { return __uint_as_float((unsigned)(127 + e) << 23); }
+
 __global__ __launch_bounds__(256) void k_screen_wnorm(const float* __restrict__ W, int ld, int rows, int K,
                                                       float* __restrict__ nw) {
   const int row = blockIdx.x * 4 + (threadIdx.x >> 6), lane = threadIdx.x & 63;
@@ -26,11 +45,47 @@
   if (lane == 0) nw[row] = (float)sqrt(s) * (1.f + 0x1p-21f);
 }
 
+__global__ __launch_bounds__(256) void k_pack_screen_f16(const float* __restrict__ W, int ld, int rows, int K,
+                                                         const float* __restrict__ nw, unsigned short* __restrict__ dst,
+                                                         float* __restrict__ uw) {
+  const int idx = blockIdx.x * blockDim.x + threadIdx.x;
+  if (idx >= rows * K) return;
+  const int e = idx & 7, lane = (idx >> 3) & 63, rest = idx >> 9;
+  const int nkc = K / 16;
+  const int kc = rest % nkc, mb = rest / nkc;
+  const int row = mb * 32 + (lane & 31), col = kc * 16 + 8 * (e >> 2) + 4 * (lane >> 5) + (e & 3);
+  const int sw = screen_f16_exp(nw[row]);
+  const bool bad = sw < -60;
+  const float w = bad ? 0.f : W[(size_t)row * ld + col] * screen_pow2(sw);
+  dst[idx] = __builtin_bit_cast(unsigned short, (_Float16)w);
+  if (col == 0) uw[row] = bad ? INFINITY : screen_pow2(-sw);
+}
+
+__global__ __launch_bounds__(256) void k_screen_f16_dw(const float* __restrict__ W, int ld, int rows, int K,
+                                                       const float* __restrict__ nw, float* __restrict__ dw) {
+  const int row = blockIdx.x * 4 + (threadIdx.x >> 6), lane = threadIdx.x & 63;
+  if (row >= rows) return;
+  const int sw = screen_f16_exp(nw[row]);
+  double s = 0.0;
+  if (sw >= -60) {
+    const float f = screen_pow2(sw);
+    for (int k = lane; k < K; k += 64) {
+      const float w = W[(size_t)row * ld + k] * f;
+      const double r = (double)w - (double)(float)(_Float16)w;
+      s += r * r;
+    }
+  }
+#pragma unroll
+  for (int o = 32; o > 0; o >>= 1) s += __shfl_xor(s, o);
+  if (lane == 0) dw[row] = sw >= -60 ? (float)(sqrt(s) * (double)screen_pow2(-sw)) * (1.f + 0x1p-21f) : 0.f;
+}
+
 struct ScreenArgs {
   const u32x4* wps;
   const float* nw;
   float* probe_s;
   float* probe_eps;
+  const float* uw;
 };
 
 #ifdef CATRE_DEBUG_TRACE
@@ -151,6 +206,93 @@
   }
 };
 
+__device__ __forceinline__ int screen_tile_scale(const float* na, int lane) {
+  float m = na[lane & 63];
+#pragma unroll
+  for (int o = 1; o < 64; o <<= 1) m = fmaxf(m, lane_get(m, lane ^ o));
+  const int s = screen_f16_exp(m);
+  return __builtin_amdgcn_readfirstlane(s < -61 ? -61 : s);
+}
+
+template <int PFD, int PRE, int NKC_ = 32, bool SWZ = true, int LD = 512>
+struct ScreenPipeF16 {
+  static constexpr int NKC = NKC_, NT = 2 * NKC, RA = PFD + 1;
+  static_assert(PRE <= PFD && PFD < NT, "ring");
+  u32x4 ah[RA][4];
+  const u32x4* wp;
+
+  __device__ __forceinline__ void issue_a(int t) {
+    const int kc = t >> 1, half = t & 1;
+#pragma unroll
+    for (int m = 0; m < 4; ++m) ah[t % RA][m] = wp[((half * 4 + m) * NKC + kc) * 64];
+  }
+  __device__ __forceinline__ void prefetch(const u32x4* __restrict__ wp_) {
+    wp = wp_;
+#pragma unroll
+    for (int d = 0; d < PRE; ++d) issue_a(d);
+    __builtin_amdgcn_sched_barrier(0);
+  }
+  __device__ __forceinline__ void run(f32x16 (&acc)[8][2], const float* x, int lane, int sa) {
+    const int n = lane & 31, h = lane >> 5, sw = lane & 15;
+    const float fs = screen_pow2(sa < -60 ? -60 : sa);
+    const float* xrow = x + n * LD;
+    const float* xlow[4][2];
+#pragma unroll
+    for (int q = 0; q < 4; ++q)
+#pragma unroll
+      for (int j = 0; j < 2; ++j) xlow[q][j] = SWZ ? xrow + (((4 * q + 2 * j + h) ^ sw) << 2) : xrow + ((2 * j + h) << 2);
+    f32x4 braw[2][2];
+    u32x4 bh[2][2];
+    auto issue_b = [&](int kc) {
+#pragma unroll
+      for (int nb = 0; nb < 2; ++nb)
+#pragma unroll
+        for (int j = 0; j < 2; ++j)
+          braw[nb][j] = *reinterpret_cast<const f32x4*>((SWZ ? xlow[kc & 3][j] + (kc >> 2) * 64 : xlow[0][j] + kc * 16) +
+                                                        nb * 32 * LD);
+    };
+    auto cvt_b = [&](int kc) {
+#pragma unroll
+      for (int nb = 0; nb < 2; ++nb) {
+        const float v[8] = {braw[nb][0][0] * fs, braw[nb][0][1] * fs, braw[nb][0][2] * fs, braw[nb][0][3] * fs,
+                            braw[nb][1][0] * fs, braw[nb][1][1] * fs, braw[nb][1][2] * fs, braw[nb][1][3] * fs};
+        bh[kc & 1][nb] = pack8<OpF16>(v);
+      }
+    };
+#pragma unroll
+    for (int d = PRE; d < PFD; ++d) issue_a(d);
+    issue_b(0);
+    cvt_b(0);
+    issue_b(1);
+#pragma unroll
+    for (int kc = 0; kc < NKC; ++kc) {
+#pragma unroll
+      for (int half = 0; half < 2; ++half) {
+        const int t = 2 * kc + half;
+        if (t + PFD < NT) issue_a(t + PFD);
+        __builtin_amdgcn_sched_barrier(0);
+        if (half == 1 && kc + 1 < NKC) cvt_b(kc + 1);
+#pragma unroll
+        for (int m = 0; m < 4; ++m)
+#pragma unroll
+          for (int nb = 0; nb < 2; ++nb) {
+            f32x16& c = acc[half * 4 + m][nb];
+            c = OpF16::mfma(bh[kc & 1][nb], ah[t % RA][m], c);
+          }
+        if (half == 1 && kc + 1 < NKC) {
+#pragma unroll
+          for (int g = 0; g < 8; ++g) {
+            __builtin_amdgcn_sched_group_barrier(0x008, 1, 0);
+            __builtin_amdgcn_sched_group_barrier(0x002, 3, 0);
+          }
+        }
+        __builtin_amdgcn_sched_barrier(0);
+        if (half == 1 && kc + 2 < NKC) issue_b(kc + 2);
+      }
+    }
+  }
+};
+
 __device__ __forceinline__ void screen_load_w(f32x4 (&wb)[16], const f32x4* __restrict__ w) {
 #pragma unroll
   for (int kc = 0; kc < 8; ++kc) {
@@ -398,14 +540,15 @@
 #endif
 }
 
-template <int MB, int K, bool SWZ = true, int LAYER = 0, bool POOL = false, bool RUN = false>
+template <int MB, int K, bool SWZ = true, int LAYER = 0, bool POOL = false, bool RUN = false, bool F16 = false>
 __device__ __forceinline__ void screen_select_store(const f32x16 (&acc)[MB][2], const f32x4* __restrict__ wf,
                                                     const float* __restrict__ nw, const float* na, const float* x,
                                                     unsigned long long* sets, float* __restrict__ out,
                                                     const float* __restrict__ bias, int ch0, bool relu, int valid, int tile,
                                                     const ScreenArgs& sc, int lane, int ld = K, float* frun = nullptr,
-                                                    bool first = true) {
+                                                    bool first = true, int sa = 0) {
   static_assert(POOL || !RUN, "the run form refines the pooled replay");
+  static_assert(POOL || !F16, "the fp16 screen exists for the pooled forms");
   constexpr int NKC8 = K / 64;
   const int n = lane & 31, h = lane >> 5;
   const int partner = (lane ^ 32) << 2;
@@ -437,21 +580,35 @@
     }
 #pragma unroll
     for (int mb = 0; mb < MB; ++mb) {
-      float e1, e0;
-      screen_eps_coef<K>(nw[ch0 + mb * 32 + n], e1, e0);
+      float e1, e0, u = 1.f;
+      bool all = false;
+      if constexpr (F16) {
+        const float uw = sc.uw[ch0 + mb * 32 + n], ua = screen_pow2(sa < -60 ? 60 : -sa);
+        all = sa < -60 || !(uw <= 0x1p60f);
+        screen_eps_coef_f16<K>(nw[ch0 + mb * 32 + n], uw, sc.uw[1024 + ch0 + mb * 32 + n], ua, e1, e0);
+        u = uw * ua;
+      } else {
+        screen_eps_coef<K>(nw[ch0 + mb * 32 + n], e1, e0);
+      }
       float L = -INFINITY;
       if constexpr (RUN) L = fc[mb];
 #pragma unroll
       for (int nb = 0; nb < 2; ++nb)
 #pragma unroll
-        for (int r = 0; r < 16; ++r) L = fmaxf(L, acc[mb][nb][r] - fmaf(e1, na4[nb][r >> 2][r & 3], e0));
+        for (int r = 0; r < 16; ++r) {
+          const float eps = fmaf(e1, na4[nb][r >> 2][r & 3], e0);
+          L = fmaxf(L, F16 ? fmaf(acc[mb][nb][r], u, -eps) : acc[mb][nb][r] - eps);
+        }
       L = fmaxf(L, swap32(L));
       unsigned own = 0;
 #pragma unroll
       for (int nb = 0; nb < 2; ++nb)
 #pragma unroll
-        for (int r = 0; r < 16; ++r)
-          own |= (acc[mb][nb][r] + fmaf(e1, na4[nb][r >> 2][r & 3], e0) >= L) ? 1u << (nb * 16 + r) : 0u;
+        for (int r = 0; r < 16; ++r) {
+          const float eps = fmaf(e1, na4[nb][r >> 2][r & 3], e0);
+          own |= ((F16 ? fmaf(acc[mb][nb][r], u, eps) : acc[mb][nb][r] + eps) >= L) ? 1u << (nb * 16 + r) : 0u;
+        }
+      if (F16 && all) own = 0xffffffffu;
       own &= vmask;
       if (sc.probe_s) {
 #pragma unroll
@@ -459,7 +616,7 @@
 #pragma unroll
           for (int r = 0; r < 16; ++r) {
             const size_t o = ((size_t)tile * 1024 + ch0 + mb * 32 + n) * TP + nb * 32 + (r & 3) + 8 * (r >> 2) + 4 * h;
-            sc.probe_s[o] = acc[mb][nb][r];
+            sc.probe_s[o] = F16 ? acc[mb][nb][r] * u : acc[mb][nb][r];
             sc.probe_eps[o] = fmaf(e1, na4[nb][r >> 2][r & 3], e0);
           }
       }
@@ -542,14 +699,20 @@
 #endif
 }
 
-template <bool POOL, bool RUN = false>
+template <bool C, class A, class B>
+struct ScreenPipeSel { typedef A type; };
+template <class A, class B>
+struct ScreenPipeSel<false, A, B> { typedef B type; };
+
+template <bool POOL, bool RUN = false, bool F16 = false>
 struct Trunk4ScreenT {
   ScreenArgs sc;
   float* frun;
   bool first;
   const f32x4* wf;
   const float* b4;
-  ScreenPipe8<2> g4;
+  typename ScreenPipeSel<F16, ScreenPipeF16<5, 2>, ScreenPipe8<2>>::type g4;
+  int sa;
   f32x16 acc4[8][2];
   __device__ __forceinline__ void prefetch(const f32x4* __restrict__ wp4, const float* __restrict__ b4_, int mb0, int lane) {
     wf = wp4 + ((size_t)mb0 * 64) * 64 + (lane & 31);
@@ -561,14 +724,19 @@
     __syncthreads();
 #pragma unroll
     for (int mb = 0; mb < 8; ++mb) acc4[mb][0] = acc4[mb][1] = zero16();
-    g4.run(acc4, a3, lane);
+    if constexpr (F16) {
+      sa = screen_tile_scale(a2, lane);
+      g4.run(acc4, a3, lane, sa);
+    } else {
+      g4.run(acc4, a3, lane);
+    }
   }
   __device__ __forceinline__ void store(const float* a3, float* a2, float* __restrict__ pm, int tile, int mb0, int valid, int,
                                         const TrainSave&, int lane) {
     unsigned long long* sets = reinterpret_cast<unsigned long long*>(a2 + 64) + (mb0 >> 3) * 8 * 64;
     asm volatile("v_mbcnt_lo_u32_b32 %0, -1, 0\n\tv_mbcnt_hi_u32_b32 %0, -1, %0" : "=v"(lane));
-    screen_select_store<8, 512, true, 0, POOL, RUN>(acc4, wf, sc.nw, a2, a3, sets, pm + (size_t)tile * PMW, b4, mb0 * 32,
-                                                    false, valid, tile, sc, lane, 512, frun, first);
+    screen_select_store<8, 512, true, 0, POOL, RUN, F16>(acc4, wf, sc.nw, a2, a3, sets, pm + (size_t)tile * PMW, b4, mb0 * 32,
+                                                         false, valid, tile, sc, lane, 512, frun, first, F16 ? sa : 0);
   }
 };
 typedef Trunk4ScreenT<false> Trunk4Screen;
@@ -588,20 +756,22 @@
                      TrainSave{}, tl, blockIdx.x, threadIdx.x);
 }
 
-__global__ __launch_bounds__(256) void k_trunk4sp(catre_points P, const float* __restrict__ trans3,
-                                                  const float* __restrict__ trans64, const float* __restrict__ Wc1,
-                                                  const float* __restrict__ bc1, const f32x4* __restrict__ wp2,
-                                                  const float* __restrict__ b2, const f32x4* __restrict__ wp3,
-                                                  const float* __restrict__ b3, const f32x4* __restrict__ wp4,
-                                                  const float* __restrict__ b4, float* __restrict__ pm,
-                                                  float* __restrict__ pointfeat, int B, int N, int M,
-                                                  unsigned long long* __restrict__ trace, ScreenArgs sc) {
-  __shared__ __attribute__((aligned(16))) float smem[TRUNK_SMEM];
-  Trunk4ScreenT<true> tl;
-  tl.sc = sc;
-  trunk4_body<false>(smem, P, trans3, trans64, Wc1, bc1, wp2, b2, wp3, b3, wp4, b4, pm, pointfeat, B, N, M, trace,
-                     TrainSave{}, tl, blockIdx.x, threadIdx.x);
-}
+#define TRUNK4SP_(NAME, F16)                                                                                              \
+  __global__ __launch_bounds__(256) void NAME(                                                                            \
+      catre_points P, const float* __restrict__ trans3, const float* __restrict__ trans64, const float* __restrict__ Wc1, \
+      const float* __restrict__ bc1, const f32x4* __restrict__ wp2, const float* __restrict__ b2,                         \
+      const f32x4* __restrict__ wp3, const float* __restrict__ b3, const f32x4* __restrict__ wp4,                         \
+      const float* __restrict__ b4, float* __restrict__ pm, float* __restrict__ pointfeat, int B, int N, int M,           \
+      unsigned long long* __restrict__ trace, ScreenArgs sc) {                                                            \
+    __shared__ __attribute__((aligned(16))) float smem[TRUNK_SMEM];                                                       \
+    Trunk4ScreenT<true, false, F16> tl;                                                                                   \
+    tl.sc = sc;                                                                                                           \
+    trunk4_body<false>(smem, P, trans3, trans64, Wc1, bc1, wp2, b2, wp3, b3, wp4, b4, pm, pointfeat, B, N, M, trace,      \
+                       TrainSave{}, tl, blockIdx.x, threadIdx.x);                                                         \
+  }
+TRUNK4SP_(k_trunk4sp, false)
+TRUNK4SP_(k_trunk4sp16, true)
+#undef TRUNK4SP_
 
 __device__ __forceinline__ void run_info(int rid, int B, int N, int M, int S, int& tile0, int& nt) {
   const int TN = (N + TP - 1) / TP, TM = (M + TP - 1) / TP;
@@ -633,11 +803,11 @@
   int B, N, M, S;
 };
 
-__global__ __launch_bounds__(256) void k_trunk4sr(TrunkRunArgs args) {
+template <bool F16>
+__device__ __forceinline__ void trunk4sr_body() {
   __shared__ __attribute__((aligned(16))) float smem[TRUNK_SMEM];
   typedef const __attribute__((address_space(4))) TrunkRunArgs* ArgPtr;
   ArgPtr ap = (ArgPtr)__builtin_amdgcn_kernarg_segment_ptr();
-  (void)args;
   const int wave = __builtin_amdgcn_readfirstlane(threadIdx.x >> 6);
   int tile0, nt;
   run_info(blockIdx.x, ap->B, ap->N, ap->M, ap->S, tile0, nt);
@@ -647,7 +817,7 @@
     asm volatile("v_mbcnt_lo_u32_b32 %0, -1, 0\n\tv_mbcnt_hi_u32_b32 %0, -1, %0" : "=v"(lane));
     asm volatile("" : "+s"(ap));
     const TrunkRunArgs a = *(const TrunkRunArgs*)ap;
-    Trunk4ScreenT<true, true> tl;
+    Trunk4ScreenT<true, true, F16> tl;
     tl.sc = a.sc;
     tl.frun = a.frun + (size_t)blockIdx.x * 1024;
     tl.first = t == 0;
@@ -656,11 +826,22 @@
     __syncthreads();
   }
 }
+__global__ __launch_bounds__(256) void k_trunk4sr(TrunkRunArgs args) {
+  (void)args;
+  trunk4sr_body<false>();
+}
+__global__ __launch_bounds__(256) void k_trunk4sr16(TrunkRunArgs args) {
+  (void)args;
+  trunk4sr_body<true>();
+}
 
 typedef ScreenPipe8<2, 8, false, LD128> StnScreenPipe;
-
-template <int LAYER, bool POOL, bool RUN = false>
-__device__ __forceinline__ void stn_conv3_screened(const float* img, float* scratch, StnScreenPipe& g,
+typedef ScreenPipeF16<5, 2, 8, false, LD128> StnScreenPipeF16;
+template <bool F16>
+using StnPipeT = typename ScreenPipeSel<F16, StnScreenPipeF16, StnScreenPipe>::type;
+
+template <int LAYER, bool POOL, bool RUN = false, bool F16 = false>
+__device__ __forceinline__ void stn_conv3_screened(const float* img, float* scratch, StnPipeT<F16>& g,
                                                    const f32x4* __restrict__ wp3, const float* __restrict__ b3,
                                                    float* __restrict__ pm, int tile0, int valid2, const ScreenArgs& sc,
                                                    float* __restrict__ probe_rows, int wave, int tid, int lane,
@@ -679,13 +860,19 @@
 #pragma unroll
     for (int mb = 0; mb < 8; ++mb) acc[mb][0] = acc[mb][1] = zero16();
     const float* x = img + t * TP * LD128;
-    g.run(acc, x, ln);
+    int sa = 0;
+    if constexpr (F16) {
+      sa = screen_tile_scale(scratch + t * TP, ln);
+      g.run(acc, x, ln, sa);
+    } else {
+      g.run(acc, x, ln);
+    }
     asm volatile("v_mbcnt_lo_u32_b32 %0, -1, 0\n\tv_mbcnt_hi_u32_b32 %0, -1, %0" : "=v"(ln));
     const f32x4* wf = wp3 + ((size_t)mb0 * 16) * 64 + (ln & 31);
-    screen_select_store<8, 128, false, LAYER, POOL, RUN>(acc, wf, sc.nw, scratch + t * TP, x, sets,
-                                                         pm + (size_t)(tile0 + t) * PMW, b3, mb0 * 32, true,
-                                                         min(valid2 - t * TP, TP), tile0 + t, sc, ln, LD128, frun,
-                                                         first_pair && t == 0);
+    screen_select_store<8, 128, false, LAYER, POOL, RUN, F16>(acc, wf, sc.nw, scratch + t * TP, x, sets,
+                                                              pm + (size_t)(tile0 + t) * PMW, b3, mb0 * 32, true,
+                                                              min(valid2 - t * TP, TP), tile0 + t, sc, ln, LD128, frun,
+                                                              first_pair && t == 0, sa);
   };
   tile(0, lane);
   if (nt == 2) {
@@ -695,7 +882,7 @@
   }
 }
 
-template <bool POOL, bool RUN = false>
+template <bool POOL, bool RUN = false, bool F16 = false>
 __device__ __forceinline__ void stn3d_pair_s_body(catre_points P, const float* __restrict__ W1,
                                                   const float* __restrict__ b1, const f32x4* __restrict__ wp2,
                                                   const float* __restrict__ b2, const f32x4* __restrict__ wp3,
@@ -723,7 +910,7 @@
     conv3_relu_row<32>(x, y, z, W1, b1, (wave >> 1) * 32, a1 + p * LD64);
   }
   __syncthreads();
-  StnScreenPipe g3;
+  StnPipeT<F16> g3;
   g3.prefetch(sc.wps + ((size_t)wave * 8 * 8) * 64 + lane);
   {
     f32x16 acc[1][4] = {{zero16(), zero16(), zero16(), zero16()}};
@@ -731,21 +918,22 @@
     store_tile_lds_pre<1, 4, true, false>(acc, a2, LD128, wave * 32, bv2, lane);
   }
   __syncthreads();
-  stn_conv3_screened<1, POOL, RUN>(a2, a1, g3, wp3, b3, pm, tile0, ti.valid, sc, probe_rows, wave, tid, lane, frun, first_pair);
-}
-#define STN3D_PAIR_S_(NAME, POOL)                                                                                          \
+  stn_conv3_screened<1, POOL, RUN, F16>(a2, a1, g3, wp3, b3, pm, tile0, ti.valid, sc, probe_rows, wave, tid, lane, frun, first_pair);
+}
+#define STN3D_PAIR_S_(NAME, POOL, F16)                                                                                        \
   __global__ __launch_bounds__(256) void NAME(catre_points P, const float* __restrict__ W1, const float* __restrict__ b1, \
                                               const f32x4* __restrict__ wp2, const float* __restrict__ b2,                \
                                               const f32x4* __restrict__ wp3, const float* __restrict__ b3,                \
                                               float* __restrict__ pm, int B, int N, int M, ScreenArgs sc,                 \
                                               float* __restrict__ probe_rows) {                                           \
-    stn3d_pair_s_body<POOL>(P, W1, b1, wp2, b2, wp3, b3, pm, B, N, M, sc, probe_rows, blockIdx.x, threadIdx.x);          \
-  }
-STN3D_PAIR_S_(k_stn3d_pair_s, false)
-STN3D_PAIR_S_(k_stn3d_pair_sp, true)
+    stn3d_pair_s_body<POOL, false, F16>(P, W1, b1, wp2, b2, wp3, b3, pm, B, N, M, sc, probe_rows, blockIdx.x, threadIdx.x); \
+  }
+STN3D_PAIR_S_(k_stn3d_pair_s, false, false)
+STN3D_PAIR_S_(k_stn3d_pair_sp, true, false)
+STN3D_PAIR_S_(k_stn3d_pair_sp16, true, true)
 #undef STN3D_PAIR_S_
 
-template <bool POOL, bool RUN = false>
+template <bool POOL, bool RUN = false, bool F16 = false>
 __device__ __forceinline__ void stnkd_pair_s_body(catre_points P, const float* __restrict__ trans3,
                                                   const float* __restrict__ Wc1, const float* __restrict__ bc1,
                                                   const f32x4* __restrict__ wpf1, const float* __restrict__ bf1,
@@ -788,7 +976,7 @@
     store_tile_lds_pre<1, 2, true, false>(acc, f1 + half1 * TP * LD64, LD64, mblk1 * 32, bv1, lane);
   }
   __syncthreads();
-  StnScreenPipe g3;
+  StnPipeT<F16> g3;
   g3.prefetch(sc.wps + ((size_t)wave * 8 * 8) * 64 + lane);
   {
     f32x16 acc[1][4] = {{zero16(), zero16(), zero16(), zero16()}};
@@ -796,19 +984,20 @@
     store_tile_lds_pre<1, 4, true, false>(acc, f2, LD128, wave * 32, bv2, lane);
   }
   __syncthreads();
-  stn_conv3_screened<2, POOL, RUN>(f2, h1, g3, wpf3, bf3, pm, tile0, ti.valid, sc, probe_rows, wave, tid, lane, frun, first_pair);
-}
-#define STNKD_PAIR_S_(NAME, POOL)                                                                                      \
+  stn_conv3_screened<2, POOL, RUN, F16>(f2, h1, g3, wpf3, bf3, pm, tile0, ti.valid, sc, probe_rows, wave, tid, lane, frun, first_pair);
+}
+#define STNKD_PAIR_S_(NAME, POOL, F16)                                                                                    \
   __global__ __launch_bounds__(256) void NAME(                                                                        \
       catre_points P, const float* __restrict__ trans3, const float* __restrict__ Wc1, const float* __restrict__ bc1, \
       const f32x4* __restrict__ wpf1, const float* __restrict__ bf1, const f32x4* __restrict__ wpf2,                  \
       const float* __restrict__ bf2, const f32x4* __restrict__ wpf3, const float* __restrict__ bf3,                   \
       float* __restrict__ pm, int B, int N, int M, ScreenArgs sc, float* __restrict__ probe_rows) {                   \
-    stnkd_pair_s_body<POOL>(P, trans3, Wc1, bc1, wpf1, bf1, wpf2, bf2, wpf3, bf3, pm, B, N, M, sc, probe_rows,       \
+    stnkd_pair_s_body<POOL, false, F16>(P, trans3, Wc1, bc1, wpf1, bf1, wpf2, bf2, wpf3, bf3, pm, B, N, M, sc, probe_rows, \
                             blockIdx.x, threadIdx.x);                                                                  \
   }
-STNKD_PAIR_S_(k_stnkd_pair_s, false)
-STNKD_PAIR_S_(k_stnkd_pair_sp, true)
+STNKD_PAIR_S_(k_stnkd_pair_s, false, false)
+STNKD_PAIR_S_(k_stnkd_pair_sp, true, false)
+STNKD_PAIR_S_(k_stnkd_pair_sp16, true, true)
 #undef STNKD_PAIR_S_
 
 __device__ __forceinline__ void pair_run_info(int rid, int B, int N, int M, int SP, int& pair0, int& np) {
@@ -836,13 +1025,14 @@
   const u32x4* wps;
   const float* nw;
   int B, N, M, SP;
+  const float* uw;
 };
 
-__global__ __launch_bounds__(256) void k_stn3d_pair_sr(Stn3dRunArgs args) {
+template <bool F16>
+__device__ __forceinline__ void stn3d_pair_sr_body() {
   __shared__ __attribute__((aligned(16))) float frun[1024];
   typedef const __attribute__((address_space(4))) Stn3dRunArgs* ArgPtr;
   ArgPtr ap = (ArgPtr)__builtin_amdgcn_kernarg_segment_ptr();
-  (void)args;
   const int wave = __builtin_amdgcn_readfirstlane(threadIdx.x >> 6);
   int pair0, np;
   pair_run_info(blockIdx.x, ap->B, ap->N, ap->M, ap->SP, pair0, np);
@@ -854,10 +1044,19 @@
     asm volatile("v_mbcnt_lo_u32_b32 %0, -1, 0\n\tv_mbcnt_hi_u32_b32 %0, -1, %0" : "=v"(lane));
     asm volatile("" : "+s"(ap));
     const Stn3dRunArgs a = *(const Stn3dRunArgs*)ap;
-    stn3d_pair_s_body<true, true>(a.P, a.W1, a.b1, a.wp2, a.b2, a.wp3, a.b3, a.pm, a.B, a.N, a.M,
-                                  ScreenArgs{a.wps, a.nw, nullptr, nullptr}, nullptr, bid, wave * 64 + lane, frun, false);
+    stn3d_pair_s_body<true, true, F16>(a.P, a.W1, a.b1, a.wp2, a.b2, a.wp3, a.b3, a.pm, a.B, a.N, a.M,
+                                       ScreenArgs{a.wps, a.nw, nullptr, nullptr, a.uw}, nullptr, bid, wave * 64 + lane, frun,
+                                       false);
     __syncthreads();
   }
+}
+__global__ __launch_bounds__(256) void k_stn3d_pair_sr(Stn3dRunArgs args) {
+  (void)args;
+  stn3d_pair_sr_body<false>();
+}
+__global__ __launch_bounds__(256) void k_stn3d_pair_sr16(Stn3dRunArgs args) {
+  (void)args;
+  stn3d_pair_sr_body<true>();
 }
 
 struct StnkdRunArgs {
@@ -873,13 +1072,14 @@
   const u32x4* wps;
   const float* nw;
   int B, N, M, SP;
+  const float* uw;
 };
 
-__global__ __launch_bounds__(256) void k_stnkd_pair_sr(StnkdRunArgs args) {
+template <bool F16>
+__device__ __forceinline__ void stnkd_pair_sr_body() {
   __shared__ __attribute__((aligned(16))) float frun[1024];
   typedef const __attribute__((address_space(4))) StnkdRunArgs* ArgPtr;
   ArgPtr ap = (ArgPtr)__builtin_amdgcn_kernarg_segment_ptr();
-  (void)args;
   const int wave = __builtin_amdgcn_readfirstlane(threadIdx.x >> 6);
   int pair0, np;
   pair_run_info(blockIdx.x, ap->B, ap->N, ap->M, ap->SP, pair0, np);
@@ -891,8 +1091,17 @@
     asm volatile("v_mbcnt_lo_u32_b32 %0, -1, 0\n\tv_mbcnt_hi_u32_b32 %0, -1, %0" : "=v"(lane));
     asm volatile("" : "+s"(ap));
     const StnkdRunArgs a = *(const StnkdRunArgs*)ap;
-    stnkd_pair_s_body<true, true>(a.P, a.trans3, a.Wc1, a.bc1, a.wpf1, a.bf1, a.wpf2, a.bf2, a.wpf3, a.bf3, a.pm, a.B, a.N, a.M,
-                                  ScreenArgs{a.wps, a.nw, nullptr, nullptr}, nullptr, bid, wave * 64 + lane, frun, false);
+    stnkd_pair_s_body<true, true, F16>(a.P, a.trans3, a.Wc1, a.bc1, a.wpf1, a.bf1, a.wpf2, a.bf2, a.wpf3, a.bf3, a.pm, a.B, a.N,
+                                       a.M, ScreenArgs{a.wps, a.nw, nullptr, nullptr, a.uw}, nullptr, bid, wave * 64 + lane,
+                                       frun, false);
     __syncthreads();
   }
 }
+__global__ __launch_bounds__(256) void k_stnkd_pair_sr(StnkdRunArgs args) {
+  (void)args;
+  stnkd_pair_sr_body<false>();
+}
+__global__ __launch_bounds__(256) void k_stnkd_pair_sr16(StnkdRunArgs args) {
+  (void)args;
+  stnkd_pair_sr_body<true>();
+}
diff --git a/catre_amd/hip.py b/catre_amd/hip.py
--- a/catre_amd/hip.py
+++ b/catre_amd/hip.py
@@ -263,7 +263,7 @@
 
 
 FORM_IDS = {"trunk4": 0, "stn4": 1, "stn_pair": 2, "rotw": 3, "fc_tail": 4, "screen": 5, "screen_stn": 6, "screen_pool": 7,
-            "screen_run": 8}
+            "screen_run": 8, "screen_f16": 9}
 
 
 def form_switch(name, value=None):
diff --git a/profiles/screen_candidates.py b/profiles/screen_candidates.py
--- a/profiles/screen_candidates.py
+++ b/profiles/screen_candidates.py
@@ -29,9 +29,12 @@
 pool = hip.form_switch("screen_pool")
 run = pool and hip.form_switch("screen_run")
 run_stn = run and os.environ.get("CATRE_SCREEN_RUN_STN", "1") != "0"
+f16 = pool and hip.form_switch("screen_f16")
+f16_stn = f16 and os.environ.get("CATRE_SCREEN_F16_STN", "1") != "0"
 S = (hip.screen_run_len() or hip.screen_run_rule(B, N, M, torch.cuda.get_device_properties(0).multi_processor_count)) if run else 1
 lines = [f"B={B} N=M={N} K={K} refine, make_inputs(seed=1000), recipe weights; screen_pool {'on' if pool else 'off'}; "
          f"screen_run {'on, run length ' + str(S) + (' (STN kernels: ' + ('on' if run_stn else 'off') + ')') if run and S > 1 else 'off'}; "
+         f"screen_f16 {'on (STN kernels: ' + ('on' if f16_stn else 'off') + ')' if f16 else 'off'}; "
          "per-channel replay: chains a lane carries at once: 4"]
 for row, name in enumerate(("trunk conv4 (k_trunk4s)", "stn.conv3 (k_stn3d_pair_s)", "fstn.conv3 (k_stnkd_pair_s)")):
     c = list(cnt)[64 * row:64 * row + 64]
@@ -40,6 +43,8 @@
         name = name.replace("_s)", "_sp)").replace("k_trunk4s", "k_trunk4sp")
         if run and S > 1 and (row == 0 or run_stn):
             name = name.replace("sp)", "sr)")
+        if f16 and (row == 0 or f16_stn):
+            name = name.replace(")", "16)")
     lines.append(f"screened {name}")
     tot = sum(c[:32])
     mean = sum(i * v for i, v in enumerate(c[:32])) / max(tot, 1)
```

Result: faster. 52610 object-iterations/s, median of 6 (+11.3%).
